# autonomousvision/volsurfs

Measured on AMD Instinct MI355X. Metric: Mrays/s (fwd+bwd) at 800x800, K=5 shells, higher is better.
Workload: dtype f16 (hash features, MLP on MFMA, composite: as the reference), f32 accumulate and I/O

## Files before the change

### include/volsurfs_hip.h

```cpp
#ifndef VOLSURFS_HIP_H
#define VOLSURFS_HIP_H

#include <stdint.h>

#ifdef __cplusplus
extern "C" {
#endif

#define VSA_OK 0
#define VSA_ERR_ARG (-1)
#define VSA_ERR_UNSUPPORTED (-2)

#define VSA_MAX_SHELLS 16

int vsa_version(void);

int vsa_composite_dense_fwd(const float* surfs_rgb, const float* surfs_alpha,
                            const float* rgb_bg, int bg_is_broadcast, float* out_rgb,
                            float* out_rgb_fg, float* out_bg_transmittance, float* out_weights,
                            float* out_surfs_rgb_h, float* out_surfs_alpha_h, int nr_rays,
                            int nr_shells, int carry_f16, void* stream);

int vsa_composite_dense_bwd(const float* surfs_rgb, const float* surfs_alpha,
                            const float* rgb_bg, int bg_is_broadcast, const float* g_rgb,
                            float* g_surfs_rgb, float* g_surfs_alpha, float* g_rgb_bg,
                            int nr_rays, int nr_shells, int carry_f16, void* stream);

int vsa_composite_dense_bwd_l1(const float* surfs_rgb, const float* surfs_alpha,
                               const float* rgb_bg, int bg_is_broadcast, const float* pred_rgb,
                               const float* gt_rgb, float loss_scale, float* g_surfs_rgb,
                               float* g_surfs_alpha, int nr_rays, int nr_shells, int carry_f16,
                               void* stream);

int vsa_composite_dense_fwd_bwd_l1(const float* surfs_rgb, const float* surfs_alpha,
                                   const float* rgb_bg, int bg_is_broadcast, const float* gt_rgb,
                                   float loss_scale, float* out_rgb, float* g_surfs_rgb,
                                   float* g_surfs_alpha, int nr_rays, int nr_shells, int carry_f16,
                                   void* stream);

long long vsa_reduce_scratch_bytes(void);
int vsa_count_hits(const int32_t* hit_slot, long long n, void* scratch, int64_t* out, void* stream);
int vsa_l1_mean(const float* pred, const float* gt, long long n, void* scratch, float* out, void* stream);

typedef struct vsa_bvh vsa_bvh;
int vsa_bvh_build(const float* verts, const int32_t* faces, int nr_verts, int nr_faces,
                  int leaf_size, vsa_bvh** out_bvh);
int vsa_bvh_sizes(const vsa_bvh* bvh, int* nr_nodes, int* nr_tris, int* max_depth);
int vsa_bvh_export(const vsa_bvh* bvh, float* nodes_out, float* tris_out, int node_base,
                   int tri_base);
int vsa_bvh_export_q(const vsa_bvh* bvh, uint32_t* qnodes_out, float* tris_out, int node_base,
                     int tri_base, float* frame_out);
int vsa_bvh_refit(vsa_bvh* bvh, const float* verts, int nr_verts);
int vsa_bvh_destroy(vsa_bvh* bvh);

typedef struct vsa_bvh_dev vsa_bvh_dev;
int vsa_bvh_dev_build(const float* verts, const int32_t* faces, int nr_verts, int nr_faces, int leaf_size,
                      void* stream, vsa_bvh_dev** out_bvh);
int vsa_bvh_dev_sizes(const vsa_bvh_dev* bvh, int* nr_nodes, int* nr_tris, int* max_depth);
int vsa_bvh_dev_export(const vsa_bvh_dev* bvh, float* nodes_out, uint32_t* qnodes_out, float* tris_out,
                       int node_base, int tri_base, float* frame_out, void* stream);
int vsa_bvh_dev_refit(vsa_bvh_dev* bvh, const float* verts, int nr_verts, void* stream);
int vsa_bvh_dev_destroy(vsa_bvh_dev* bvh);
int vsa_bvh_dev_build_ploc(const float* verts, const int32_t* faces, int nr_verts, int nr_faces, int leaf_size,
                           int radius, void* stream, vsa_bvh_dev** out_bvh);

int vsa_trace(const float* nodes, const float* tris, const int32_t* mesh_roots, int nr_meshes,
              int max_depth, const float* rays_o, const float* rays_d, int nr_rays, float t_min,
              float* hit_t, int32_t* hit_slot, float* hit_uv, void* stream);

int vsa_trace_q(const uint32_t* qnodes, const float* tris, const int32_t* mesh_roots,
                const float* mesh_frames, int nr_meshes, int max_depth, const float* rays_o,
                const float* rays_d, int nr_rays, float t_min, float* hit_t, int32_t* hit_slot,
                float* hit_uv, void* stream);
int vsa_trace_q_narrow(const uint32_t* qnodes, const float* tris, const int32_t* mesh_roots,
                       const float* mesh_frames, int nr_meshes, int max_depth, const float* rays_o,
                       const float* rays_d, int nr_rays, float t_min, float* hit_t, int32_t* hit_slot,
                       float* hit_uv, int rays_per_wave, void* stream);
long long vsa_trace_feedback_bytes(int nr_rays, int nr_meshes);
int vsa_trace_q_fb(const uint32_t* qnodes, const float* tris, const int32_t* mesh_roots,
                   const float* mesh_frames, int nr_meshes, int max_depth, const float* rays_o,
                   const float* rays_d, int nr_rays, float t_min, float* hit_t, int32_t* hit_slot,
                   float* hit_uv, void* feedback, long long feedback_bytes, int phase, void* stream);
int vsa_trace_coop_config(int chunk, int lanes, long long max_waves);
int vsa_trace_q_stats(const uint32_t* qnodes, const float* tris, const int32_t* mesh_roots,
                      const float* mesh_frames, int nr_meshes, int max_depth, const float* rays_o,
                      const float* rays_d, int nr_rays, float t_min, uint64_t* stats, void* stream);
int vsa_hit_attributes(const float* tris, const float* rays_o, const float* rays_d,
                       const float* hit_t, const int32_t* hit_slot, const float* hit_uv,
                       int nr_rays, uint8_t* is_hit, int32_t* tri_id, float* positions,
                       float* normals, float* barycentric, void* stream);

#define VSA_NT_MAX_LEVELS 16
#define VSA_NT_MAX_DEG 4
#define VSA_NT_WEIGHTS_PER_TEX 8192
#define VSA_NT_ROW_QUADS(d) ((d) == 0 ? 2 : ((d) == 1 ? 4 : 8))
#define VSA_NT_ALPHA_QUAD(d) ((d) == 0 ? 1 : ((d) == 1 ? 3 : ((d) == 2 ? 4 : 6)))

typedef struct vsa_nt_plan {
  int32_t nr_shells;
  int32_t rgb_degrees;
  int32_t alpha_degrees;
  int32_t inner_solid;
  int32_t with_alpha_decay;
  int32_t n_levels;
  int32_t tex_res[VSA_NT_MAX_DEG];
  float sh_lo[VSA_NT_MAX_DEG];
  float sh_span[VSA_NT_MAX_DEG];
  float level_scale[VSA_NT_MAX_LEVELS];
  int32_t level_res[VSA_NT_MAX_LEVELS];
  int32_t level_size[VSA_NT_MAX_LEVELS];
  int32_t level_offset[VSA_NT_MAX_LEVELS + 1];
  int64_t dom_off[VSA_MAX_SHELLS * VSA_NT_MAX_DEG + 1];
  int64_t slot_capacity;
  int32_t max_rays;
  int32_t anchor;
  int64_t row_base[VSA_MAX_SHELLS * VSA_NT_MAX_DEG + 1];
  void* balance;
  int32_t row_format;
  int32_t grads_zeroed;
  int32_t shared_rgb;
  int32_t shared_alpha;
} vsa_nt_plan;

long long vsa_nt_balance_bytes(void);
int vsa_nt_rebalance(const vsa_nt_plan* plan, void* stream);

int vsa_nt_mark(const vsa_nt_plan* plan, const int32_t* hit_slot, const float* hit_uv,
                const float* face_uvs, int nr_rays, float* tex_uv, uint8_t* marks, void* stream);

int vsa_nt_compact_frame(const vsa_nt_plan* plan, uint8_t* marks, int32_t* slot_of,
                         int32_t* texel_of_slot, float* slot_xy, int32_t* seg_start,
                         int32_t* block_scratch, void* stream);

int vsa_nt_encode_fwd(const vsa_nt_plan* plan, const void* tables_h, const float* slot_xy,
                      const int32_t* seg_start, void* features, void* stream);

int vsa_nt_mlp_fwd(const vsa_nt_plan* plan, const void* weights_h, const void* features,
                   const int32_t* seg_start, uint8_t* texels, void* pre_out, void* stream);

int vsa_nt_encode_mlp_fwd(const vsa_nt_plan* plan, const void* tables_h, const void* weights_h,
                          const float* slot_xy, const int32_t* seg_start, void* features,
                          uint8_t* texels, void* pre_out, void* stream);

int vsa_nt_mlp_bwd(const vsa_nt_plan* plan, const void* weights_h, void* features,
                   const int32_t* seg_start, uint16_t* grad_rows, float* grad_weights,
                   float* dfeat_abs_sum, float weight_grad_scale, void* stream);

int vsa_nt_shade_fwd(const vsa_nt_plan* plan, const int32_t* hit_slot, const float* tex_uv,
                     const float* rays_d, const float* tris, const int32_t* slot_of,
                     const int32_t* seg_start, const uint8_t* texels, int nr_rays,
                     float* surfs_rgb, float* surfs_alpha,
                     float* surfs_normals, float* coeffs_out, float* act_out, void* stream);

int vsa_nt_shade_bwd(const vsa_nt_plan* plan, const int32_t* hit_slot, const float* tex_uv,
                     const float* rays_d, const float* tris, const int32_t* slot_of,
                     const int32_t* seg_start, const uint8_t* texels, int nr_rays,
                     const float* g_surfs_rgb,
                     const float* g_surfs_alpha, float grad_scale, uint16_t* grad_rows,
                     const float* act_in, void* stream);

long long vsa_nt_planes_bytes(const vsa_nt_plan* plan);
int vsa_nt_export_planes(const vsa_nt_plan* plan, const int32_t* slot_of, const int32_t* seg_start,
                         const uint8_t* texels, uint8_t* planes, long long planes_bytes, void* stream);
int vsa_nt_import_planes(const vsa_nt_plan* plan, const uint8_t* planes, long long planes_bytes,
                         const int32_t* slot_of, const int32_t* seg_start, uint8_t* texels, void* stream);

int vsa_nt_encode_bwd(const vsa_nt_plan* plan, const void* dfeatures, const float* dfeat_abs_sum,
                      float grad_scale, const float* slot_xy, const int32_t* seg_start,
                      float* grad_tables, void* stream);

int vsa_nt_encode_bwd_range(const vsa_nt_plan* plan, const void* dfeatures,
                            const float* dfeat_abs_sum, float grad_scale, const float* slot_xy,
                            const int32_t* seg_start, float* grad_tables, int shell_begin,
                            int shell_end, void* stream);

typedef struct vsa_dp_flags vsa_dp_flags;
int vsa_dp_flags_create(int n, vsa_dp_flags** out);
int vsa_dp_flags_destroy(vsa_dp_flags* flags);
int vsa_dp_flags_read(const vsa_dp_flags* flags, uint32_t* host_out);

int vsa_nt_encode_bwd_phased(const vsa_nt_plan* plan, const void* dfeatures,
                             const float* dfeat_abs_sum, float grad_scale, const float* slot_xy,
                             const int32_t* seg_start, float* grad_tables, int n_phases,
                             const int32_t* phase_shell_end, vsa_dp_flags* flags, uint32_t* counters,
                             const uint32_t* epoch, int reserve_cus, void* stream);

int vsa_dp_signal(vsa_dp_flags* flags, int index, uint32_t* epoch, int advance_epoch, void* stream);

int vsa_dp_stream_wait(vsa_dp_flags* flags, int index, uint32_t value, int mode, void* stream);

#define VSA_GRID_MAX_LEVELS 32
typedef struct vsa_grid_plan {
  int32_t n_dims;
  int32_t n_levels;
  int32_t n_features;
  int32_t reserved0;
  float level_scale[VSA_GRID_MAX_LEVELS];
  int32_t level_res[VSA_GRID_MAX_LEVELS];
  int32_t level_size[VSA_GRID_MAX_LEVELS];
  int32_t level_offset[VSA_GRID_MAX_LEVELS + 1];
} vsa_grid_plan;

int vsa_grid_encode_fwd(const vsa_grid_plan* plan, const float* tables, const float* x,
                        int nr_points, float* out, void* stream);
int vsa_grid_encode_bwd(const vsa_grid_plan* plan, const float* x, const float* g_out,
                        int nr_points, float* grad_tables, void* stream);
int vsa_grid_encode_bwd_sliced(const vsa_grid_plan* plan, const float* x, const float* g_out,
                               int nr_points, float* grad_tables, float* workspace, void* stream);
int vsa_grid_encode_bwd_binned_workspace(const vsa_grid_plan* plan, int nr_points,
                                         long long* workspace_floats);
int vsa_grid_encode_bwd_binned(const vsa_grid_plan* plan, const float* x, const float* g_out,
                               int nr_points, float* grad_tables, float* workspace, void* stream);
int vsa_grid_encode_fwd_ld(const vsa_grid_plan* plan, const float* tables, const float* x,
                           int nr_points, float* out, int out_stride, int append_x, void* stream);
int vsa_grid_encode_bwd_ld(const vsa_grid_plan* plan, const float* x, const float* g_out,
                           int g_stride, int nr_points, float* grad_tables, void* stream);
int vsa_grid_encode_bwd_sliced_ld(const vsa_grid_plan* plan, const float* x, const float* g_out,
                                  int g_stride, int nr_points, float* grad_tables, float* workspace,
                                  void* stream);
int vsa_grid_encode_bwd_binned_ld(const vsa_grid_plan* plan, const float* x, const float* g_out,
                                  int g_stride, int nr_points, float* grad_tables, float* workspace,
                                  void* stream);
int vsa_sh_encode(const float* dirs, int nr_dirs, int degree, float* out, void* stream);

int vsa_field_head_fwd(const float* y1, int y1_stride, const float* dirs_enc, long long nr_points, int nr_feat,
                       int nr_dir, float* x2, float* density, void* stream);
int vsa_field_head_bwd(const float* y1, int y1_stride, const float* dx2, const float* d_density, long long nr_points,
                       int nr_feat, int nr_dir, float* dy1, void* stream);

#define VSA_MLP_MAX_LAYERS 6
typedef struct vsa_mlp_plan {
  int32_t n_layers;
  int32_t dims[VSA_MLP_MAX_LAYERS + 1];
  const float* w[VSA_MLP_MAX_LAYERS];
  const float* b[VSA_MLP_MAX_LAYERS];
// ... 106 lines not shown
                           const float* rgb, const float* rgb_bg, int bg_per_ray, const float* weights_sum,
                           const float* g_rgb, const float* g_weights_sum, float* g_density,
                           float* g_rgb_samples, float* g_rgb_bg, float* scratch, int nr_rays,
                           int bug_compat, void* stream);
int vsa_nerf_coarse_cdf(const int32_t* start_end, const float* density, const float* dt, float* cdf,
                        int nr_rays, void* stream);
int vsa_neus_composite_fwd(const int32_t* start_end, const float* sdf, const float* sdf_grad,
                           const float* dirs, const float* dt, const float* samples_z,
                           const float* normals, const float* rgb, const float* rgb_bg, int bg_per_ray,
                           double cos_anneal_ratio, double logistic_beta, float* rgb_fg, float* rgb_out,
                           float* weights_sum, float* depth, float* normals_out, float* weights,
                           float* alpha, int nr_rays, void* stream);
int vsa_neus_composite_bwd(const int32_t* start_end, const float* sdf, const float* sdf_grad,
                           const float* dirs, const float* dt, const float* rgb, const float* rgb_bg,
                           int bg_per_ray, double cos_anneal_ratio, double logistic_beta,
                           const float* weights_sum, const float* g_rgb, const float* g_weights_sum,
                           float* g_sdf, float* g_sdf_grad, float* g_rgb_samples, float* g_rgb_bg,
                           float* scratch, int nr_rays, int bug_compat, void* stream);
int vsa_sdf_coarse_cdf(const int32_t* start_end, const float* sdf, const float* dt, float logistic_beta,
                       float* cdf, int nr_rays, void* stream);
int vsa_offsets_composite_fwd(const int32_t* start_end, int nr_surfs, const float* sdfs, const float* sdfs_grad,
                              const float* normals, const float* rgb, const float* transparency, const float* dirs,
                              const float* dt, const float* samples_z, const float* rgb_bg, int bg_per_ray,
                              double cos_anneal_ratio, double logistic_beta, int with_alpha_decay,
                              double alpha_decay_factor, float* surfs_rgb, float* surfs_normals, float* surfs_depths,
                              float* surfs_weight_sum, float* surfs_alpha, float* surfs_transmittance,
                              float* surfs_blending_weights, float* rgb_fg, float* bg_transmittance, float* rgb_out,
                              float* alpha, int nr_rays, void* stream);
int vsa_offsets_composite_bwd(const int32_t* start_end, int nr_surfs, const float* sdfs, const float* sdfs_grad,
                              const float* normals, const float* rgb, const float* transparency, const float* dirs,
                              const float* dt, const float* rgb_bg, int bg_per_ray, double cos_anneal_ratio,
                              double logistic_beta, int with_alpha_decay, double alpha_decay_factor,
                              const float* surfs_rgb, const float* surfs_alpha, const float* surfs_transmittance,
                              const float* bg_transmittance, const float* g_rgb, float* g_sdfs, float* g_sdfs_grad,
                              float* g_rgb_samples, float* g_transparency, float* g_rgb_bg, float* scratch,
                              int nr_rays, int bug_compat, void* stream);
int vsa_sdfs_coarse_cdf(const int32_t* start_end, int nr_surfs, const float* sdfs, const float* dt,
                        float logistic_beta, float* cdf, int nr_rays, void* stream);
int vsa_packed_median_depth(const int32_t* start_end, const float* samples_z,
                            const float* weights, float threshold, float* out, int nr_rays,
                            int fallback_compat, void* stream);
int vsa_packed_update_dt(const int32_t* start_end, const float* ray_max_dt, const float* ray_exit,
                         const float* samples_z, int is_background, float* samples_dt,
                         int nr_rays, void* stream);
int vsa_sample_bg(const float* rays_o, const float* rays_d, const float* ray_t_start,
                  float ray_t_far, int nr_samples_per_ray, int jitter, uint64_t rng_state,
                  uint64_t rng_inc, float* ray_max_dt, float* samples_3d, float* samples_dirs,
                  float* samples_z, int32_t* ray_start_end_idx, int nr_rays, void* stream);
int vsa_contract_samples(const float* ray_o, const int32_t* start_end, const float* samples_3d,
                         const float* samples_z, float* out_samples_3d, float* out_samples_z,
                         int nr_rays, void* stream);

int vsa_packed_sum_over_rays(const int32_t* start_end, const float* values, float* sum_per_ray,
                             float* sum_per_sample, int nr_rays, int dim, void* stream);
int vsa_packed_sum_over_rays_bwd(const int32_t* start_end, const float* g_sum_per_ray,
                                 const float* g_sum_per_sample, float* g_values, int nr_rays,
                                 int dim, void* stream);
int vsa_packed_sdf2alpha(const int32_t* start_end, const float* samples_dt, const float* samples_sdf,
                         const float* logistic_beta, float* alpha, int nr_rays, void* stream);
int vsa_packed_compute_cdf(const int32_t* start_end, const float* weights, float* cdf, int nr_rays,
                           void* stream);

int vsa_sample_fg(const float* rays_o, const float* rays_d, const float* ray_t_entry,
                  const float* ray_t_exit, float min_dist_between_samples,
                  int min_nr_samples_per_ray, int max_nr_samples_per_ray, int jitter,
                  uint64_t rng_state, uint64_t rng_inc, float* ray_max_dt, int32_t* samples_idx,
                  float* samples_3d, float* samples_dirs, float* samples_z,
                  int32_t* ray_start_end_idx, int nr_rays, void* stream);
int vsa_pack_compact(const int32_t* start_end, const int32_t* out_start, const int32_t* samples_idx,
                     const float* samples_3d, const float* samples_dirs, const float* samples_z,
                     const float* samples_dt, const float* samples_values, int values_dim,
                     int32_t* out_idx, float* out_3d, float* out_dirs, float* out_z, float* out_dt,
                     float* out_values, int32_t* out_start_end, int nr_rays, void* stream);
int vsa_importance_sample(const float* rays_o, const float* rays_d, const int32_t* start_end,
                          const float* samples_z, const float* samples_cdf,
                          int nr_importance_samples, int jitter, uint64_t rng_state,
                          uint64_t rng_inc, float* out_3d, float* out_dirs, float* out_z,
                          int32_t* out_start_end, int nr_rays, void* stream);

int vsa_uncontract_samples(const float* ray_o, const int32_t* start_end, const float* samples_3d,
                           const float* samples_z, float* out_samples_3d, float* out_samples_z,
                           int nr_rays, void* stream);

int vsa_combine_packs(const int32_t* start_end_1, const int32_t* idx_1, const float* s3d_1,
                      const float* dirs_1, const float* z_1, const float* values_1,
                      const int32_t* start_end_2, const int32_t* idx_2, const float* s3d_2,
                      const float* dirs_2, const float* z_2, const float* values_2,
                      const int32_t* out_start, float min_dist_between_samples, int values_dim,
                      int32_t* out_idx, float* out_3d, float* out_dirs, float* out_z,
                      float* out_values, int32_t* out_start_end, int nr_rays, void* stream);

int vsa_intersect_primitive(const float* rays_o, const float* rays_d, int nr_rays, int kind,
                            float size, uint8_t* is_hit, float* t_near, float* t_far,
                            float* points_near, float* points_far, void* stream);

int vsa_camera_rays(const float* c2w, const float* intrinsics_inv, int height, int width,
                    int nr_rays_per_pixel, int jitter_pixels, uint64_t rng_state, uint64_t rng_inc,
                    float* rays_o, float* rays_d, float* points_2d, void* stream);

int vsa_reel_next_rays_batch(const float* c2w_all, const float* intrinsics_inv_all,
                             const float* rgb_all, const float* mask_all, int nr_cameras, int height,
                             int width, int batch_size, int nr_rays_per_pixel, int jitter_pixels,
                             uint64_t rng_state, uint64_t rng_inc, int32_t* camera_idx,
                             float* rays_o, float* rays_d, float* gt_rgb, float* gt_mask,
                             float* points_2d, void* stream);

typedef struct vsa_train_ctl {
  int32_t iter;
  int32_t nr_rays;
  int32_t capacity;
  int32_t adam_step;
  float loss_scale;
  float adam_lr;
  float loss;
  int32_t clamped;
  uint64_t rng_state, rng_inc;
  int64_t nr_hits;
  int32_t target_hits;
  int32_t nr_warmup;
  int32_t nr_milestones;
  int32_t milestone[8];
  float lr_stage[9];
  int32_t adam_pending;
  double lr_base;
  double loss_weight;
  int64_t sum_rays, sum_hits;
} vsa_train_ctl;

int vsa_train_ctl_tick(vsa_train_ctl* ctl, void* stream);

int vsa_reel_next_rays_batch_ctl(const float* c2w_all, const float* intrinsics_inv_all, const float* rgb_all,
                                 const float* mask_all, int nr_cameras, int height, int width, int capacity,
                                 int nr_rays_per_pixel, int jitter_pixels, const vsa_train_ctl* ctl,
                                 const float* dummy_o, const float* dummy_d, const float* dummy_rgb,
                                 int32_t* camera_idx, float* rays_o, float* rays_d, float* gt_rgb,
                                 float* gt_mask, float* points_2d, void* stream);

int vsa_composite_dense_fwd_bwd_l1_ctl(const float* surfs_rgb, const float* surfs_alpha, const float* rgb_bg,
                                       int bg_is_broadcast, const float* gt_rgb, const vsa_train_ctl* ctl,
                                       float* out_rgb, float* g_surfs_rgb, float* g_surfs_alpha, int capacity,
                                       int nr_shells, int carry_f16, void* stream);

int vsa_l1_mean_ctl(const float* pred, const float* gt, int capacity, void* scratch, vsa_train_ctl* ctl, void* stream);

int vsa_adam_step_ctl(const vsa_adam_tensor* tensors_dev, const int32_t* chunks_dev, int nr_chunks, float beta1,
                      float beta2, float eps, float grad_scale, int zero_grads, int max_workgroups,
                      const vsa_train_ctl* ctl, void* stream);

int vsa_tile_order(const float* src, float* dst, int height, int width, int channels, int inverse,
                   void* stream);
int vsa_tile_order_rays(const float* rays_o, const float* rays_d, const float* gt_rgb,
                        float* rays_o_tiled, float* rays_d_tiled, float* gt_rgb_tiled, int height,
                        int width, void* stream);


int vsa_occ_grid_points(const int32_t* point_indices, int nr_points, int nr_voxels_per_dim,
                        float extent_x, float extent_y, float extent_z, int centre_of_voxel, int jitter,
                        uint64_t rng_state, uint64_t rng_inc, float* out_points, void* stream);
int vsa_occ_update_values(const int32_t* point_indices, const float* values, int nr_points, float decay,
                          float* grid_values, void* stream);
int vsa_occ_update_occupancy_density(const int32_t* point_indices, int nr_points, int nr_voxels_per_dim,
                                     float extent_x, float extent_y, float extent_z,
                                     float occupancy_thresh, int check_neighbours,
                                     const float* grid_values, uint8_t* grid_occupancy, void* stream);
int vsa_occ_update_occupancy_sdf(const int32_t* point_indices, const float* logistic_beta, int nr_points,
                                 int nr_voxels_per_dim, float extent_x, float extent_y, float extent_z,
                                 float occupancy_thresh, const float* grid_values,
                                 uint8_t* grid_occupancy, void* stream);
int vsa_occ_check(const float* points, int nr_points, int nr_voxels_per_dim, float extent_x,
                  float extent_y, float extent_z, const float* grid_values,
                  const uint8_t* grid_occupancy, const uint8_t* grid_roi, uint8_t* out_occupancy,
                  float* out_values, void* stream);
int vsa_occ_rays_t_near_t_far(const float* rays_o, const float* rays_d, const float* ray_t_entry,
                              const float* ray_t_exit, int nr_rays, int nr_voxels_per_dim,
                              float extent_x, float extent_y, float extent_z,
                              const uint8_t* grid_occupancy, const uint8_t* grid_roi, float* out_t_near,
                              float* out_t_far, void* stream);
int vsa_occ_first_sample(const float* rays_o, const float* rays_d, const float* ray_t_entry,
                         const float* ray_t_exit, int nr_rays, int nr_voxels_per_dim, float extent_x,
                         float extent_y, float extent_z, const uint8_t* grid_occupancy,
                         const uint8_t* grid_roi, float* samples_3d, float* samples_dirs,
                         float* samples_z, float* samples_dt, int32_t* ray_start_end_idx, void* stream);
int vsa_occ_advance_samples(const float* samples_dirs, const float* samples_3d, int nr_points,
                            int nr_voxels_per_dim, float extent_x, float extent_y, float extent_z,
                            const uint8_t* grid_occupancy, const uint8_t* grid_roi,
                            float* new_samples_3d, uint8_t* is_within_bounds, void* stream);
int vsa_sample_fg_occupied(const float* rays_o, const float* rays_d, const float* ray_t_entry,
                           const float* ray_t_exit, float min_dist_between_samples,
                           int min_nr_samples_per_ray, int max_nr_samples_per_ray, int jitter_samples,
                           uint64_t rng_state, uint64_t rng_inc, int nr_voxels_per_dim, float extent_x,
                           float extent_y, float extent_z, const uint8_t* grid_occupancy,
                           const uint8_t* grid_roi, float* ray_max_dt, int32_t* samples_idx,
                           float* samples_3d, float* samples_dirs, float* samples_z,
                           int32_t* ray_start_end_idx, int nr_rays, void* stream);

long long vsa_image_metrics_workspace_bytes(int B, int H, int W, int pool, int pred_u8, int gt_u8);
int vsa_image_metrics(const void* pred, int pred_u8, const void* gt, int gt_u8, int B, int H, int W, int pool,
                      int quantize_pred, void* workspace, long long workspace_bytes, double* psnr_out,
                      double* ssim_out, void* stream);

long long vsa_isosurface_workspace_bytes(long long nx, long long ny, long long nz, int nr_levels);
int vsa_isosurface_count(const float* grid, long long nx, long long ny, long long nz, const float* levels,
                         int nr_levels, int inside_above, void* workspace, long long workspace_bytes,
                         long long* totals, void* stream);
int vsa_isosurface_emit(const float* grid, long long nx, long long ny, long long nz, const float* levels,
                        int nr_levels, int inside_above, const float* origin, const float* spacing, void* workspace,
                        long long workspace_bytes, const long long* totals, float* const* verts,
                        int32_t* const* faces, void* stream);
int vsa_mc_table(int8_t* out);

long long vsa_simplify_workspace_bytes(long long nr_verts, long long nr_faces);
int vsa_simplify(const float* verts, long long nr_verts, const int32_t* faces, long long nr_faces,
                 long long target_faces, void* workspace, long long workspace_bytes, float* out_verts,
                 int32_t* out_faces, long long* stats, float* stage_ms, void* stream);

#define VSA_ERR_ATLAS_FULL (-3)
long long vsa_atlas_workspace_bytes(long long nr_verts, long long nr_faces, int resolution);
int vsa_atlas(const float* verts, long long nr_verts, const int32_t* faces, long long nr_faces, int resolution,
              int padding, void* workspace, long long workspace_bytes, float* out_faces_uvs, int32_t* out_chart,
              long long* stats, float* scale, float* stage_ms, void* stream);
long long vsa_atlas_rasterize_workspace_bytes(long long nr_faces);
int vsa_atlas_rasterize(const float* faces_uvs, long long nr_faces, int resolution, void* workspace,
                        long long workspace_bytes, int32_t* out_face_id, int32_t* out_count, void* stream);

int vsa_st_begin(const float* points_near, int nr_rays, int nr_slots, float* pts, uint8_t* flags, int32_t* live,
                 float* dense, int32_t* count, void* stream);
int vsa_st_step(const int32_t* live_in, const int32_t* count_in, const float* sdf, int nr_columns,
                const int32_t* slot_cols, int nr_rays, const float* rays_d, float sdf_multiplier, float thresh,
                int kind, float size, float* pts, uint8_t* flags, uint8_t* keep, int32_t* block_counts,
                const float* dense_in, int32_t* live_out, float* dense_out, int32_t* count_out, int bound,
                void* stream);
int vsa_st_finish(const float* pts, const float* rays_o, int nr_rays, int nr_slots, const uint8_t* flags,
                  int unconverged_are_hits, float* z, uint8_t* hit, uint8_t* keep, int32_t* block_counts,
                  int32_t* hit_list, int32_t* hit_count, void* stream);
int vsa_st_scatter(const int32_t* ids, long long nr_ids, const float* src, int nr_channels, int nr_rays,
                   int nr_slots, float* dst, void* stream);
int vsa_st_blend(const float* surfs_rgb, const float* surfs_alpha, int nr_rays, int nr_surfs,
                 float* surfs_transmittance, float* surfs_blending_weights, float* rgb_fg, float* bg_transmittance,
                 void* stream);

long long vsa_tb_workspace_bytes(long long nr_faces, int resolution);
long long vsa_tb_max_chunks(int resolution, int nr_samples, long long chunk_rows);
int vsa_tb_samples(const float* faces_uvs, long long nr_faces, int resolution, int nr_samples,
                   unsigned long long seed, long long chunk_rows, void* workspace, long long workspace_bytes,
                   int32_t* owner, int32_t* ctl, int ctl_len, void* stream);
int vsa_tb_emit(const float* verts, const int32_t* faces, const float* faces_uvs, long long nr_faces, int resolution,
                int nr_samples, unsigned long long seed, const void* workspace, long long workspace_bytes,
                const int32_t* owner, int32_t* row_start, float* points, float* normals, void* stream);
int vsa_tb_resolve(const float* vals, int nr_channels, const int32_t* row_start, int texel_begin, int texel_end,
                   int resolution, float* texture, void* stream);
int vsa_tb_dilate(float* img, int height, int width, int nr_channels, int nr_iterations, int32_t* stamp,
                  int32_t* filled, void* stream);

int vsa_tsdf_fuse_lattice(const float* proj, const float* depth, int nr_views, int height, int width,
                          const float* axis, int n, float sdf_trunc, int uncontract, float* out_tsdf, void* stream);
int vsa_tsdf_fuse_points(const float* proj, const float* depth, const float* rgb_maps, int nr_views, int height,
                         int width, const float* points, long long nr_points, float sdf_trunc, int uncontract,
                         float* out_tsdf, float* out_rgb, void* stream);
int vsa_tsdf_uncontract_points(const float* points, long long nr_points, float max_range, float* out, void* stream);

long long vsa_mesh_clusters_workspace_bytes(long long nr_verts, long long nr_faces);
int vsa_mesh_clusters(const float* verts, long long nr_verts, const int32_t* faces, long long nr_faces,
                      void* workspace, long long workspace_bytes, int32_t* out_triangle_clusters,
                      int32_t* out_cluster_n_triangles, double* out_cluster_area, long long* out_nr_clusters,
                      float* stage_ms, void* stream);
int vsa_mesh_filter(const float* verts, long long nr_verts, const int32_t* faces, long long nr_faces, int mode,
                    const uint8_t* keep_mask, long long cluster_to_keep, long long min_cluster_faces,
                    int drop_unreferenced, int drop_degenerate, void* workspace, long long workspace_bytes,
                    float* out_verts, int32_t* out_faces, int32_t* out_vertex_map, int32_t* out_face_map,
                    long long* stats, float* stage_ms, void* stream);
int vsa_mesh_compact_rows(const void* rows, long long nr_rows, int row_words, const int32_t* map, void* out,
                          void* stream);

int vsa_face_view_counts(const uint32_t* qnodes, const float* tris, const int32_t* mesh_roots,
                         const float* mesh_frames, int nr_meshes, int max_depth,
                         const float* c2w_all, const float* intrinsics_inv_all,
                         int nr_views, int height, int width, int supersample, float t_min,
                         const long long* face_base, uint32_t* counts,
                         void* stream);
int vsa_face_view_counts_tile(int tile);
int vsa_face_ring_dilate(const int32_t* faces, long long nr_faces, long long nr_verts, uint8_t* keep,
                         int rings, uint8_t* vert_scratch, void* stream);

int vsa_closest_point_q(const uint32_t* qnodes, const float* tris, const int32_t* mesh_roots,
                        const float* mesh_frames, int nr_meshes, int max_depth, const float* points,
                        long long nr_points, float* dist, int32_t* slot, float* bary, void* stream);
int vsa_closest_point_q_stats(const uint32_t* qnodes, const float* tris, const int32_t* mesh_roots,
                              const float* mesh_frames, int nr_meshes, int max_depth, const float* points,
                              long long nr_points, long long* counters, void* stream);
int vsa_closest_walk_config(int keep_bounds);
long long vsa_surface_area_prefix_workspace_bytes(long long nr_slots);
int vsa_surface_area_prefix(const float* tris, long long first_slot, long long nr_slots, void* workspace,
                            long long workspace_bytes, long long* area_prefix, void* stream);
int vsa_surface_sample(const float* tris, long long first_slot, long long nr_slots, const long long* area_prefix,
                       long long nr_samples, unsigned long long seed, float* points, int32_t* slot, float* bary,
                       void* stream);
int vsa_surface_distance(const float* src_tris, long long src_first_slot, long long src_nr_slots,
                         const long long* src_area_prefix, const uint32_t* dst_qnodes, const float* dst_tris,
                         int dst_root, const float* dst_frame, int dst_max_depth, long long nr_samples,
                         unsigned long long seed, const float* thresholds, int nr_thresholds,
                         unsigned long long* stats, double* partials, void* stream);

long long vsa_mesh_pseudonormals_workspace_bytes(long long nr_verts, long long nr_faces);
int vsa_mesh_pseudonormals(const float* vertices, long long nr_verts, const int32_t* faces, long long nr_faces,
                           void* workspace, long long workspace_bytes, float* table, void* stream);
int vsa_signed_distance_q(const uint32_t* qnodes, const float* tris, const int32_t* mesh_roots,
// ... 40 lines not shown
```

### volsurfs_amd/composite.py

```python
import torch

from . import _lib


class _CompositeDense(torch.autograd.Function):
    @staticmethod
    def forward(ctx, surfs_rgb, surfs_alpha, rgb_bg, carry_f16):
        N, K, _ = surfs_rgb.shape
        surfs_rgb = _lib.check_f32(surfs_rgb.contiguous(), N, K, 3)
        surfs_alpha = _lib.check_f32(surfs_alpha.contiguous().view(N, K), N, K)
        rgb_bg = rgb_bg.contiguous()
        bcast = rgb_bg.shape[0] == 1 and N != 1
        _lib.check_f32(rgb_bg, 1 if bcast else N, 3)
        dev = surfs_rgb.device
        out_rgb = torch.empty(N, 3, device=dev)
        out_fg = torch.empty(N, 3, device=dev)
        out_bgT = torch.empty(N, 1, device=dev)
        out_w = torch.empty(N, K, 1, device=dev)
        out_rgb_h = torch.empty(N, K, 3, device=dev)
        out_alpha_h = torch.empty(N, K, 1, device=dev)
        _lib.call("vsa_composite_dense_fwd", surfs_rgb, surfs_alpha, rgb_bg, bcast, out_rgb,
                  out_fg, out_bgT, out_w, out_rgb_h, out_alpha_h, N, K, int(carry_f16),
                  _lib.stream_ptr())
        ctx.save_for_backward(surfs_rgb, surfs_alpha, rgb_bg)
        ctx.bcast = bcast
        ctx.carry_f16 = int(carry_f16)
        ctx.mark_non_differentiable(out_fg, out_bgT, out_w, out_rgb_h, out_alpha_h)
        return out_rgb, out_fg, out_bgT, out_w, out_rgb_h, out_alpha_h

    @staticmethod
    def backward(ctx, g_rgb, *unused):
        surfs_rgb, surfs_alpha, rgb_bg = ctx.saved_tensors
        N, K, _ = surfs_rgb.shape
        g_rgb = _lib.check_f32(g_rgb.contiguous(), N, 3)
        g_c = torch.empty_like(surfs_rgb)
        g_a = torch.empty_like(surfs_alpha)
        need_bg = ctx.needs_input_grad[2]
        g_bg = torch.empty(N, 3, device=g_rgb.device) if need_bg else None
        _lib.call("vsa_composite_dense_bwd", surfs_rgb, surfs_alpha, rgb_bg, ctx.bcast, g_rgb,
                  g_c, g_a, g_bg, N, K, ctx.carry_f16, _lib.stream_ptr())
        if need_bg and ctx.bcast:
            g_bg = g_bg.sum(0, keepdim=True)
        return g_c, g_a, g_bg, None


def composite_dense(surfs_rgb, surfs_alpha, rgb_bg, carry_f16=False):
    N, K = surfs_rgb.shape[:2]
    alpha2d = surfs_alpha.reshape(N, K)
    rgb, fg, bgT, w, rgb_h, alpha_h = _CompositeDense.apply(surfs_rgb, alpha2d, rgb_bg, carry_f16)
    return {
        "rgb": rgb,
        "rgb_fg": fg,
        "rgb_bg": rgb_bg.expand(N, 3).half().float(),
        "surfs_alpha": alpha_h,
        "surfs_rgb": rgb_h,
        "surfs_blending_weights": w,
        "bg_transmittance": bgT,
    }


class _CompositeL1(torch.autograd.Function):

    @staticmethod
    def forward(ctx, surfs_rgb, surfs_alpha, rgb_bg, gt_rgb):
        N, K = surfs_rgb.shape[:2]
        rgb, g_c, g_a = composite_fwd_bwd_l1_raw(surfs_rgb.contiguous(), surfs_alpha.reshape(N, K).contiguous(),
                                                 rgb_bg.contiguous(), gt_rgb.contiguous(), 1.0 / (3.0 * N))
        ctx.save_for_backward(g_c, g_a)
        ctx.alpha_shape = surfs_alpha.shape
        loss = l1_mean(rgb, gt_rgb)
        ctx.mark_non_differentiable(rgb)
        return loss, rgb

    @staticmethod
    def backward(ctx, g_loss, _g_rgb):
        g_c, g_a = ctx.saved_tensors
        return g_c * g_loss, (g_a * g_loss).reshape(ctx.alpha_shape), None, None


def composite_l1(surfs_rgb, surfs_alpha, rgb_bg, gt_rgb):
    return _CompositeL1.apply(surfs_rgb, surfs_alpha, rgb_bg, gt_rgb)


def composite_fwd_raw(surfs_rgb, surfs_alpha, rgb_bg, carry_f16=False):
    N, K, _ = surfs_rgb.shape
    out = torch.empty(N, 3, device=surfs_rgb.device)
    bcast = rgb_bg.shape[0] == 1 and N != 1
    _lib.call("vsa_composite_dense_fwd", surfs_rgb, surfs_alpha, rgb_bg, bcast, out, None, None,
              None, None, None, N, K, int(carry_f16), _lib.stream_ptr())
    return out


def composite_bwd_raw(surfs_rgb, surfs_alpha, rgb_bg, g_rgb, carry_f16=False):
    N, K, _ = surfs_rgb.shape
    g_c = torch.empty_like(surfs_rgb)
    g_a = torch.empty_like(surfs_alpha)
    bcast = rgb_bg.shape[0] == 1 and N != 1
    _lib.call("vsa_composite_dense_bwd", surfs_rgb, surfs_alpha, rgb_bg, bcast, g_rgb, g_c, g_a,
              None, N, K, int(carry_f16), _lib.stream_ptr())
    return g_c, g_a


def composite_bwd_l1_raw(surfs_rgb, surfs_alpha, rgb_bg, pred_rgb, gt_rgb, loss_scale, carry_f16=False):
    N, K, _ = surfs_rgb.shape
    g_c = torch.empty_like(surfs_rgb)
    g_a = torch.empty_like(surfs_alpha)
    bcast = rgb_bg.shape[0] == 1 and N != 1
    _lib.call("vsa_composite_dense_bwd_l1", surfs_rgb, surfs_alpha, rgb_bg, bcast, pred_rgb, gt_rgb,
              float(loss_scale), g_c, g_a, N, K, int(carry_f16), _lib.stream_ptr())
    return g_c, g_a


def composite_fwd_bwd_l1_raw(surfs_rgb, surfs_alpha, rgb_bg, gt_rgb, loss_scale, carry_f16=False):
    N, K, _ = surfs_rgb.shape
    rgb = torch.empty(N, 3, device=surfs_rgb.device)
    g_c = torch.empty_like(surfs_rgb)
    g_a = torch.empty_like(surfs_alpha)
    bcast = rgb_bg.shape[0] == 1 and N != 1
    _lib.call("vsa_composite_dense_fwd_bwd_l1", surfs_rgb, surfs_alpha, rgb_bg, bcast, gt_rgb,
              float(loss_scale), rgb, g_c, g_a, N, K, int(carry_f16), _lib.stream_ptr())
    return rgb, g_c, g_a


_reduce_scratch = {}


def reduce_scratch(device):
    import ctypes
    dev = torch.device(device)
    dev = torch.device("cuda", torch.cuda.current_device()) if dev.index is None else dev
    key = (dev, torch.cuda.current_stream(dev).cuda_stream)
    sc = _reduce_scratch.get(key)
    if sc is None:
        fn = _lib.lib().vsa_reduce_scratch_bytes
        fn.restype = ctypes.c_longlong
        sc = _reduce_scratch[key] = torch.zeros(int(fn()), dtype=torch.uint8, device=dev)
    return sc


def l1_mean(pred, gt):
    import ctypes
    pred, gt = _lib.check_f32(pred.contiguous()), _lib.check_f32(gt.contiguous(), *pred.shape)
    pred, gt = (x if x.data_ptr() % 16 == 0 else x.clone() for x in (pred, gt))
    out = torch.empty((), device=pred.device)
    _lib.call("vsa_l1_mean", pred, gt, ctypes.c_longlong(pred.numel()), reduce_scratch(pred.device), out,
              _lib.stream_ptr())
    return out


def count_hits(hit_slot):
    import ctypes
    if hit_slot.dtype != torch.int32 or not hit_slot.is_contiguous() or not hit_slot.is_cuda:
        raise _lib.VolsurfsHipError("count_hits: contiguous CUDA int32 tensor expected")
    out = torch.empty((), dtype=torch.int64, device=hit_slot.device)
    _lib.call("vsa_count_hits", hit_slot, ctypes.c_longlong(hit_slot.numel()), reduce_scratch(hit_slot.device), out,
              _lib.stream_ptr())
    return out
```

### volsurfs_amd/csrc/composite_dense.hip

```cpp
#include "common.h"

namespace {

#ifndef VSA_COMP_TILE
#define VSA_COMP_TILE 256
#endif
constexpr int TILE = VSA_COMP_TILE;

template <int K>
struct Lds {
  static constexpr int SC = (3 * K) | 1;
  static constexpr int SA = K | 1;
};

template <int W, int S>
__device__ __forceinline__ void slab_load(const float* __restrict__ g, float* __restrict__ s,
                                          int rows_valid) {
  const int total = rows_valid * W;
  const int nvec = total >> 2;
  const float4* g4 = reinterpret_cast<const float4*>(g);
  if constexpr (W == S) {
    if (rows_valid == TILE && (TILE * W) % 4 == 0) {
      typedef __attribute__((address_space(3))) void* lds_vp;
      typedef __attribute__((address_space(1))) const void* glb_vp;
      const int wave = __builtin_amdgcn_readfirstlane(threadIdx.x >> 6), lane = threadIdx.x & 63;
      constexpr int NV = TILE * W / 4, NC = (NV + 63) / 64;
      for (int c = wave; c < NC; c += TILE / 64)
        if (c * 64 + lane < NV)
          __builtin_amdgcn_global_load_lds((glb_vp)(g4 + c * 64 + lane), (lds_vp)(s + c * 256), 16, 0, 0);
      return;
    }
    float4* s4 = reinterpret_cast<float4*>(s);
    for (int v = threadIdx.x; v < nvec; v += TILE) s4[v] = g4[v];
  } else {
    for (int v = threadIdx.x; v < nvec; v += TILE) {
      float4 x = g4[v];
      int e = v << 2;
      float xs[4] = {x.x, x.y, x.z, x.w};
#pragma unroll
      for (int i = 0; i < 4; ++i) {
        int r = (e + i) / W;
        int j = (e + i) - r * W;
        s[r * S + j] = xs[i];
      }
    }
  }
  for (int e = (nvec << 2) + threadIdx.x; e < total; e += TILE) {
    int r = e / W;
    s[r * S + (e - r * W)] = g[e];
  }
}
__device__ __forceinline__ void slab_load_fence() {
  asm volatile("s_waitcnt vmcnt(0)" ::: "memory");
}

template <int W, int S>
__device__ __forceinline__ void slab_store(float* __restrict__ g, const float* __restrict__ s,
                                           int rows_valid) {
  const int total = rows_valid * W;
  const int nvec = total >> 2;
  float4* g4 = reinterpret_cast<float4*>(g);
  if constexpr (W == S) {
    const float4* s4 = reinterpret_cast<const float4*>(s);
    for (int v = threadIdx.x; v < nvec; v += TILE) g4[v] = s4[v];
  } else {
    for (int v = threadIdx.x; v < nvec; v += TILE) {
      int e = v << 2;
      float xs[4];
#pragma unroll
      for (int i = 0; i < 4; ++i) {
        int r = (e + i) / W;
        int j = (e + i) - r * W;
        xs[i] = s[r * S + j];
      }
      g4[v] = make_float4(xs[0], xs[1], xs[2], xs[3]);
    }
  }
  for (int e = (nvec << 2) + threadIdx.x; e < total; e += TILE) {
    int r = e / W;
    g[e] = s[r * S + (e - r * W)];
  }
}

template <int K, bool CARRY_F16>
struct RayFwd {
  float a[K], c[K][3], T[K], w[K], om[K];
  float bgT, fg[3];
  __device__ __forceinline__ void run(const float* sc, const float* sa) {
#pragma unroll
    for (int k = 0; k < K; ++k) {
      a[k] = vsa_round_f16(sa[k]);
#pragma unroll
      for (int ch = 0; ch < 3; ++ch) c[k][ch] = vsa_round_f16(sc[3 * k + ch]);
      om[k] = vsa_round_f16(1.0f - a[k]);
    }
    float acc = 1.0f, Tp = 1.0f;
    fg[0] = fg[1] = fg[2] = 0.f;
#pragma unroll
    for (int k = K - 1; k >= 0; --k) {
      T[k] = Tp;
      if (CARRY_F16) {
        Tp = vsa_round_f16(Tp * om[k]);
      } else {
        acc = vsa_pin_f32(acc * om[k]);
        Tp = vsa_round_f16(acc);
      }
      w[k] = vsa_round_f16(T[k] * a[k]);
#pragma unroll
      for (int ch = 0; ch < 3; ++ch) fg[ch] += vsa_round_f16(c[k][ch] * w[k]);
    }
    bgT = Tp;
#pragma unroll
    for (int ch = 0; ch < 3; ++ch) fg[ch] = vsa_round_f16(vsa_pin_f32(fg[ch]));
  }
};

template <int K, bool CARRY_F16>
__global__ __launch_bounds__(TILE) void composite_dense_fwd_kernel(
    const float* __restrict__ surfs_rgb, const float* __restrict__ surfs_alpha,
    const float* __restrict__ rgb_bg, int bg_bcast, float* __restrict__ out_rgb,
    float* __restrict__ out_rgb_fg, float* __restrict__ out_bgT, float* __restrict__ out_w,
    float* __restrict__ out_rgb_h, float* __restrict__ out_alpha_h, int N) {
  using L = Lds<K>;
  __shared__ __attribute__((aligned(16))) float s_c[TILE * L::SC];
  __shared__ __attribute__((aligned(16))) float s_a[TILE * L::SA];
  __shared__ __attribute__((aligned(16))) float s_o[TILE * 3];
  const long long ray0 = (long long)blockIdx.x * TILE;
  const int rows = min(TILE, (int)(N - ray0));
  slab_load<3 * K, L::SC>(surfs_rgb + ray0 * 3 * K, s_c, rows);
  slab_load<K, L::SA>(surfs_alpha + ray0 * K, s_a, rows);
  if (!bg_bcast) slab_load<3, 3>(rgb_bg + ray0 * 3, s_o, rows);
  slab_load_fence();
  __syncthreads();
  const int r = threadIdx.x;
  if (r < rows) {
    RayFwd<K, CARRY_F16> f;
    f.run(s_c + r * L::SC, s_a + r * L::SA);
    float bg[3];
#pragma unroll
    for (int ch = 0; ch < 3; ++ch)
      bg[ch] = vsa_round_f16(bg_bcast ? rgb_bg[ch] : s_o[r * 3 + ch]);
#pragma unroll
    for (int ch = 0; ch < 3; ++ch)
      s_o[r * 3 + ch] = vsa_round_f16(f.fg[ch] + vsa_round_f16(f.bgT * bg[ch]));
    const long long n = ray0 + r;
    if (out_rgb_fg) {
#pragma unroll
      for (int ch = 0; ch < 3; ++ch) out_rgb_fg[n * 3 + ch] = f.fg[ch];
    }
    if (out_bgT) out_bgT[n] = f.bgT;
    if (out_w) {
#pragma unroll
      for (int k = 0; k < K; ++k) out_w[n * K + k] = f.w[k];
    }
    if (out_alpha_h) {
#pragma unroll
      for (int k = 0; k < K; ++k) out_alpha_h[n * K + k] = f.a[k];
    }
    if (out_rgb_h) {
#pragma unroll
      for (int k = 0; k < K; ++k)
#pragma unroll
        for (int ch = 0; ch < 3; ++ch) out_rgb_h[(n * K + k) * 3 + ch] = f.c[k][ch];
    }
  }
  __syncthreads();
  slab_store<3, 3>(out_rgb + ray0 * 3, s_o, rows);
}

template <int K, bool CARRY_F16>
__global__ __launch_bounds__(TILE) void composite_dense_bwd_kernel(
    const float* __restrict__ surfs_rgb, const float* __restrict__ surfs_alpha,
    const float* __restrict__ rgb_bg, int bg_bcast, const float* __restrict__ g_rgb,
    float* __restrict__ g_surfs_rgb, float* __restrict__ g_surfs_alpha,
    float* __restrict__ g_rgb_bg, int N, const float* __restrict__ l1_gt, float l1_scale,
    float* __restrict__ pred_out, const vsa_train_ctl* __restrict__ ctl) {
  using L = Lds<K>;
  int n_active = N;
  if (ctl) {
    l1_scale = ctl->loss_scale;
    n_active = ctl->nr_rays;
  }
  __shared__ __attribute__((aligned(16))) float s_c[TILE * L::SC];
  __shared__ __attribute__((aligned(16))) float s_a[TILE * L::SA];
  __shared__ __attribute__((aligned(16))) float s_g[TILE * 3];
  __shared__ __attribute__((aligned(16))) float s_b[TILE * 3];
  __shared__ __attribute__((aligned(16))) float s_t[TILE * 3];
  const long long ray0 = (long long)blockIdx.x * TILE;
  const int rows = min(TILE, (int)(N - ray0));
  slab_load<3 * K, L::SC>(surfs_rgb + ray0 * 3 * K, s_c, rows);
  slab_load<K, L::SA>(surfs_alpha + ray0 * K, s_a, rows);
  if (!pred_out) slab_load<3, 3>(g_rgb + ray0 * 3, s_g, rows);
  if (!bg_bcast) slab_load<3, 3>(rgb_bg + ray0 * 3, s_b, rows);
  if (l1_gt) slab_load<3, 3>(l1_gt + ray0 * 3, s_t, rows);
  slab_load_fence();
  __syncthreads();
  const int r = threadIdx.x;
  if (r < rows) {
    RayFwd<K, CARRY_F16> f;
    float* sc = s_c + r * L::SC;
    float* sa = s_a + r * L::SA;
    f.run(sc, sa);
    float g[3], bg[3];
#pragma unroll
    for (int ch = 0; ch < 3; ++ch) {
      bg[ch] = vsa_round_f16(bg_bcast ? rgb_bg[ch] : s_b[r * 3 + ch]);
      if (pred_out) {
        g[ch] = vsa_round_f16(f.fg[ch] + vsa_round_f16(f.bgT * bg[ch]));
        s_g[r * 3 + ch] = g[ch];
      } else {
        g[ch] = s_g[r * 3 + ch];
      }
      if (l1_gt) {
        const float d = g[ch] - s_t[r * 3 + ch];
        g[ch] = ray0 + r >= n_active ? 0.f : (d > 0.f ? l1_scale : (d < 0.f ? -l1_scale : 0.f));
      }
    }
    float S = g[0] * bg[0] + g[1] * bg[1] + g[2] * bg[2];
#pragma unroll
    for (int k = 0; k < K; ++k) {
      float rk = g[0] * f.c[k][0] + g[1] * f.c[k][1] + g[2] * f.c[k][2];
      sa[k] = f.T[k] * (rk - S);
      S = f.a[k] * rk + f.om[k] * S;
#pragma unroll
      for (int ch = 0; ch < 3; ++ch) sc[3 * k + ch] = g[ch] * f.w[k];
    }
    if (g_rgb_bg) {
#pragma unroll
      for (int ch = 0; ch < 3; ++ch) s_b[r * 3 + ch] = g[ch] * f.bgT;
    }
  }
  __syncthreads();
  slab_store<3 * K, L::SC>(g_surfs_rgb + ray0 * 3 * K, s_c, rows);
  slab_store<K, L::SA>(g_surfs_alpha + ray0 * K, s_a, rows);
  if (g_rgb_bg) slab_store<3, 3>(g_rgb_bg + ray0 * 3, s_b, rows);
  if (pred_out) slab_store<3, 3>(pred_out + ray0 * 3, s_g, rows);
}

}

#define VSA_K_DISPATCH(K_, BODY)              \
  switch (K_) {                               \
    case 1: { constexpr int KK = 1; BODY; } break;   \
    case 2: { constexpr int KK = 2; BODY; } break;   \
    case 3: { constexpr int KK = 3; BODY; } break;   \
    case 4: { constexpr int KK = 4; BODY; } break;   \
    case 5: { constexpr int KK = 5; BODY; } break;   \
    case 6: { constexpr int KK = 6; BODY; } break;   \
    case 7: { constexpr int KK = 7; BODY; } break;   \
    case 8: { constexpr int KK = 8; BODY; } break;   \
    case 9: { constexpr int KK = 9; BODY; } break;   \
    default: return VSA_ERR_UNSUPPORTED;      \
  }

extern "C" int vsa_composite_dense_fwd(const float* surfs_rgb, const float* surfs_alpha,
                                       const float* rgb_bg, int bg_is_broadcast, float* out_rgb,
                                       float* out_rgb_fg, float* out_bg_transmittance,
                                       float* out_weights, float* out_surfs_rgb_h,
                                       float* out_surfs_alpha_h, int nr_rays, int nr_shells,
                                       int carry_f16, void* stream) {
  if (nr_rays < 0 || !out_rgb) return VSA_ERR_ARG;
  if (nr_rays == 0) return VSA_OK;
  if (!surfs_rgb || !surfs_alpha || !rgb_bg) return VSA_ERR_ARG;
  dim3 grid(vsa_div_up(nr_rays, TILE)), block(TILE);
  hipStream_t st = (hipStream_t)stream;
  VSA_K_DISPATCH(nr_shells, {
    if (carry_f16)
      hipLaunchKernelGGL((composite_dense_fwd_kernel<KK, true>), grid, block, 0, st, surfs_rgb,
                         surfs_alpha, rgb_bg, bg_is_broadcast, out_rgb, out_rgb_fg,
                         out_bg_transmittance, out_weights, out_surfs_rgb_h, out_surfs_alpha_h,
                         nr_rays);
    else
      hipLaunchKernelGGL((composite_dense_fwd_kernel<KK, false>), grid, block, 0, st, surfs_rgb,
                         surfs_alpha, rgb_bg, bg_is_broadcast, out_rgb, out_rgb_fg,
                         out_bg_transmittance, out_weights, out_surfs_rgb_h, out_surfs_alpha_h,
                         nr_rays);
  });
  VSA_RETURN_LAUNCH_STATUS();
}

static int composite_bwd_launch(const float* surfs_rgb, const float* surfs_alpha,
                                const float* rgb_bg, int bg_is_broadcast, const float* g_rgb,
                                float* g_surfs_rgb, float* g_surfs_alpha, float* g_rgb_bg,
                                int nr_rays, int nr_shells, int carry_f16, const float* l1_gt,
                                float l1_scale, void* stream, float* pred_out = nullptr,
                                const vsa_train_ctl* ctl = nullptr) {
  if (nr_rays < 0) return VSA_ERR_ARG;
  if (nr_rays == 0) return VSA_OK;
  if (!surfs_rgb || !surfs_alpha || !rgb_bg || (!g_rgb && !pred_out) || !g_surfs_rgb || !g_surfs_alpha)
    return VSA_ERR_ARG;
  dim3 grid(vsa_div_up(nr_rays, TILE)), block(TILE);
  hipStream_t st = (hipStream_t)stream;
  VSA_K_DISPATCH(nr_shells, {
    if (carry_f16)
      hipLaunchKernelGGL((composite_dense_bwd_kernel<KK, true>), grid, block, 0, st, surfs_rgb,
                         surfs_alpha, rgb_bg, bg_is_broadcast, g_rgb, g_surfs_rgb, g_surfs_alpha,
                         g_rgb_bg, nr_rays, l1_gt, l1_scale, pred_out, ctl);
    else
      hipLaunchKernelGGL((composite_dense_bwd_kernel<KK, false>), grid, block, 0, st, surfs_rgb,
                         surfs_alpha, rgb_bg, bg_is_broadcast, g_rgb, g_surfs_rgb, g_surfs_alpha,
                         g_rgb_bg, nr_rays, l1_gt, l1_scale, pred_out, ctl);
  });
  VSA_RETURN_LAUNCH_STATUS();
}

extern "C" int vsa_composite_dense_bwd(const float* surfs_rgb, const float* surfs_alpha,
                                       const float* rgb_bg, int bg_is_broadcast,
                                       const float* g_rgb, float* g_surfs_rgb,
                                       float* g_surfs_alpha, float* g_rgb_bg, int nr_rays,
                                       int nr_shells, int carry_f16, void* stream) {
  return composite_bwd_launch(surfs_rgb, surfs_alpha, rgb_bg, bg_is_broadcast, g_rgb, g_surfs_rgb,
                              g_surfs_alpha, g_rgb_bg, nr_rays, nr_shells, carry_f16, nullptr, 0.f,
                              stream);
}

extern "C" int vsa_composite_dense_bwd_l1(const float* surfs_rgb, const float* surfs_alpha,
                                          const float* rgb_bg, int bg_is_broadcast,
                                          const float* pred_rgb, const float* gt_rgb,
                                          float loss_scale, float* g_surfs_rgb,
                                          float* g_surfs_alpha, int nr_rays, int nr_shells,
                                          int carry_f16, void* stream) {
  if (!gt_rgb) return VSA_ERR_ARG;
  return composite_bwd_launch(surfs_rgb, surfs_alpha, rgb_bg, bg_is_broadcast, pred_rgb,
                              g_surfs_rgb, g_surfs_alpha, nullptr, nr_rays, nr_shells, carry_f16,
                              gt_rgb, loss_scale, stream);
}

extern "C" int vsa_composite_dense_fwd_bwd_l1(const float* surfs_rgb, const float* surfs_alpha,
                                              const float* rgb_bg, int bg_is_broadcast,
                                              const float* gt_rgb, float loss_scale, float* out_rgb,
                                              float* g_surfs_rgb, float* g_surfs_alpha, int nr_rays,
                                              int nr_shells, int carry_f16, void* stream) {
  if (!gt_rgb || (nr_rays > 0 && !out_rgb)) return VSA_ERR_ARG;
  return composite_bwd_launch(surfs_rgb, surfs_alpha, rgb_bg, bg_is_broadcast, nullptr, g_surfs_rgb,
                              g_surfs_alpha, nullptr, nr_rays, nr_shells, carry_f16, gt_rgb,
                              loss_scale, stream, out_rgb);
}

extern "C" int vsa_composite_dense_fwd_bwd_l1_ctl(const float* surfs_rgb, const float* surfs_alpha,
                                                  const float* rgb_bg, int bg_is_broadcast, const float* gt_rgb,
                                                  const vsa_train_ctl* ctl, float* out_rgb, float* g_surfs_rgb,
                                                  float* g_surfs_alpha, int capacity, int nr_shells, int carry_f16,
                                                  void* stream) {
  if (!gt_rgb || !ctl || capacity < 1 || !out_rgb) return VSA_ERR_ARG;
  return composite_bwd_launch(surfs_rgb, surfs_alpha, rgb_bg, bg_is_broadcast, nullptr, g_surfs_rgb, g_surfs_alpha,
                              nullptr, capacity, nr_shells, carry_f16, gt_rgb, 0.f, stream, out_rgb, ctl);
}
```

### volsurfs_amd/csrc/nt_shade.hip

```cpp
#include "nt_common.h"

struct ShadeIdx {
  long long tile;
  int shell;
  bool valid;
};
__device__ __forceinline__ ShadeIdx shade_idx(int K, int tiles) {
  const unsigned id = blockIdx.x, x = id & 7u, q = id >> 3;
  const unsigned s = q % (unsigned)K, tg = q / (unsigned)K;
  const long long t = (long long)tg * 8 + x;
  return {t, (int)s, t < tiles};
}
static inline dim3 shade_grid(int tiles, int shells) {
  return dim3((unsigned)(((tiles + 7) / 8) * 8 * shells));
}

namespace {

constexpr int SH_BLOCK = 256;

constexpr float C0 = 0.28209479177387814f;
constexpr float C1 = 0.4886025119029199f;
constexpr float C2_0 = 1.0925484305920792f, C2_1 = -1.0925484305920792f,
                C2_2 = 0.31539156525252005f, C2_3 = -1.0925484305920792f,
                C2_4 = 0.5462742152960396f;
constexpr float C3_0 = -0.5900435899266435f, C3_1 = 2.890611442640554f,
                C3_2 = -0.4570457994644658f, C3_3 = 0.3731763325901154f,
                C3_4 = -0.4570457994644658f, C3_5 = 1.445305721320277f,
                C3_6 = -0.5900435899266435f;

__device__ __forceinline__ void sh_basis(float x, float y, float z, float b[16]) {
  b[0] = C0;
  b[1] = -(C1 * y);
  b[2] = C1 * z;
  b[3] = -(C1 * x);
  const float xx = x * x, yy = y * y, zz = z * z, xy = x * y, yz = y * z, xz = x * z;
  b[4] = C2_0 * xy;
  b[5] = C2_1 * yz;
  b[6] = C2_2 * ((2.0f * zz - xx) - yy);
  b[7] = C2_3 * xz;
  b[8] = C2_4 * (xx - yy);
  b[9] = (C3_0 * y) * (3.0f * xx - yy);
  b[10] = (C3_1 * xy) * z;
  b[11] = (C3_2 * y) * ((4.0f * zz - xx) - yy);
  b[12] = (C3_3 * z) * ((2.0f * zz - 3.0f * xx) - 3.0f * yy);
  b[13] = (C3_4 * x) * ((4.0f * zz - xx) - yy);
  b[14] = (C3_5 * z) * (xx - yy);
  b[15] = (C3_6 * x) * (xx - 3.0f * yy);
}

struct HitCtx {
  bool hit;
  float dir[3];
  float decay;
  int row[VSA_NT_MAX_DEG][4];
  float w[VSA_NT_MAX_DEG][4];
  float fx[VSA_NT_MAX_DEG], fy[VSA_NT_MAX_DEG];
};

__device__ __forceinline__ float sigmoidf_(float x) { return 1.0f / (1.0f + __expf(-x)); }

__device__ __forceinline__ float sh_raw(const float b[16], const float* sh, int degrees) {
  float r = vsa_round_f16(C0 * sh[0]);
  if (degrees > 1) {
    r = r + b[1] * sh[1];
    r = r + b[2] * sh[2];
    r = r + b[3] * sh[3];
    if (degrees > 2) {
#pragma unroll
      for (int m = 4; m < 9; ++m) r = r + b[m] * sh[m];
      if (degrees > 3) {
#pragma unroll
        for (int m = 9; m < 16; ++m) r = r + b[m] * sh[m];
      }
    }
  }
  return r;
}

__device__ __forceinline__ void build_lut(const vsa_nt_plan& plan, float* s_lut) {
  for (int i = threadIdx.x; i < VSA_NT_MAX_DEG * 256; i += blockDim.x) {
    const int d = i >> 8, q = i & 255;
    const float o = vsa_round_f16((float)q / 255.0f);
    const float t = vsa_round_f16(plan.sh_span[d] * o);
    s_lut[i] = vsa_round_f16(plan.sh_lo[d] + t);
  }
}

template <bool FULL4>
__device__ __forceinline__ int rgb_degs(const vsa_nt_plan& p) { return FULL4 ? VSA_NT_MAX_DEG : p.rgb_degrees; }
template <bool FULL4>
__device__ __forceinline__ int alpha_degs(const vsa_nt_plan& p) { return FULL4 ? VSA_NT_MAX_DEG : p.alpha_degrees; }

template <bool FULL4 = false>
__device__ __forceinline__ bool load_ctx(const vsa_nt_plan& plan, int s, long long n, int N,
                                         const int* hit_slot, const float* tex_uv,
                                         const float* rays_d, const float4* tris,
                                         const int* slot_of, const int* seg_start, HitCtx& c,
                                         float nrm[3]) {
  const long long o = (long long)s * N + n;
  const int tslot = hit_slot[o];
  c.hit = tslot >= 0;
  nrm[0] = nrm[1] = nrm[2] = 0.f;
  if (!c.hit) return false;
  c.dir[0] = rays_d[3 * n];
  c.dir[1] = rays_d[3 * n + 1];
  c.dir[2] = rays_d[3 * n + 2];
  const float4 e1 = tris[3 * (long long)tslot + 1], e2 = tris[3 * (long long)tslot + 2];
  const float cx = e1.y * e2.z - e1.z * e2.y, cy = e1.z * e2.x - e1.x * e2.z,
              cz = e1.x * e2.y - e1.y * e2.x;
  const float len = sqrtf((cx * cx + cy * cy) + cz * cz);
  const float inv = len > 0.f ? 1.0f / len : 0.f;
  nrm[0] = cx * inv;
  nrm[1] = cy * inv;
  nrm[2] = cz * inv;
  c.decay = 1.0f;
  if (plan.with_alpha_decay) {
    float dot = ((-c.dir[0]) * nrm[0] + (-c.dir[1]) * nrm[1]) + (-c.dir[2]) * nrm[2];
    dot = fminf(fmaxf(dot, 0.0f), 1.0f);
    c.decay = sigmoidf_(10.0f * dot) * 2.0f - 1.0f;
  }
  const float u = tex_uv[2 * o], v = tex_uv[2 * o + 1];
  const int D = max(rgb_degs<FULL4>(plan), alpha_degs<FULL4>(plan));
#pragma unroll
  for (int d = 0; d < VSA_NT_MAX_DEG; ++d) {
    if (d >= D) {
#pragma unroll
      for (int k = 0; k < 4; ++k) c.row[d][k] = 0, c.w[d][k] = 0.f;
      c.fx[d] = c.fy[d] = 0.f;
      continue;
    }
    const int R = plan.tex_res[d], W = R + 2;
    const bool anchor = plan.anchor != 0;
    const NtFootprint f = nt_footprint(u, v, R, anchor);
    const long long base = plan.dom_off[s * VSA_NT_MAX_DEG + d] + (long long)(f.j0 + 1) * W + (f.i0 + 1);
    const int sd = s * VSA_NT_MAX_DEG + d;
    const int rb = (int)plan.row_base[sd] - seg_start[sd] * nt_row_quads(d);
    c.row[d][0] = rb + slot_of[base] * nt_row_quads(d);
    c.row[d][1] = anchor ? c.row[d][0] : rb + slot_of[base + 1] * nt_row_quads(d);
    c.row[d][2] = anchor ? c.row[d][0] : rb + slot_of[base + W] * nt_row_quads(d);
    c.row[d][3] = anchor ? c.row[d][0] : rb + slot_of[base + W + 1] * nt_row_quads(d);
    c.fx[d] = f.fx;
    c.fy[d] = f.fy;
    c.w[d][0] = (1.0f - f.fx) * (1.0f - f.fy);
    c.w[d][1] = f.fx * (1.0f - f.fy);
    c.w[d][2] = (1.0f - f.fx) * f.fy;
    c.w[d][3] = f.fx * f.fy;
  }
  return true;
}

template <bool F16ROWS>
__device__ __forceinline__ void add_corner_row(const vsa_nt_plan& plan, int d, const unsigned* __restrict__ texels,
                                               int row, float wk, const float* s_lut, float acc[28]) {
  const int n = 2 * d + 1;
  if constexpr (!F16ROWS) {
    unsigned wds[8] = {0, 0, 0, 0, 0, 0, 0, 0};
    const unsigned* rp = texels + row;
    if (d == 0) {
      const uint2 v = *reinterpret_cast<const uint2*>(rp);
      wds[0] = v.x, wds[1] = v.y;
    } else {
      const uint4 lo = *reinterpret_cast<const uint4*>(rp);
      wds[0] = lo.x, wds[1] = lo.y, wds[2] = lo.z, wds[3] = lo.w;
      if (d >= 2) {
        const uint4 hi = *reinterpret_cast<const uint4*>(rp + 4);
        wds[4] = hi.x, wds[5] = hi.y, wds[6] = hi.z, wds[7] = hi.w;
      }
    }
#pragma unroll
    for (int i = 0; i < 3 * n; ++i) {
      const unsigned q = (wds[i >> 2] >> (8 * (i & 3))) & 255u;
      acc[i] = acc[i] + s_lut[d * 256 + q] * wk;
    }
#pragma unroll
    for (int i = 0; i < n; ++i) {
      const unsigned q = (wds[nt_alpha_quad(d) + (i >> 2)] >> (8 * (i & 3))) & 255u;
      acc[21 + i] = acc[21 + i] + s_lut[d * 256 + q] * wk;
    }
  } else {
    unsigned wds[16];
    const uint4* rp = reinterpret_cast<const uint4*>(texels + 2 * (long long)row);
    const int nv = d == 0 ? 1 : d == 1 ? 2 : 4;
#pragma unroll
    for (int v = 0; v < 4; ++v) {
      const uint4 x = v < nv ? rp[v] : make_uint4(0, 0, 0, 0);
      wds[4 * v] = x.x, wds[4 * v + 1] = x.y, wds[4 * v + 2] = x.z, wds[4 * v + 3] = x.w;
    }
    const float lo = plan.sh_lo[d], span = plan.sh_span[d];
    const bool raw = plan.row_format == 2;
    auto expand = [&](int elem) {
      const unsigned short hb = (unsigned short)(wds[elem >> 1] >> (16 * (elem & 1)));
      const float o = (float)__builtin_bit_cast(_Float16, hb);
      return raw ? o : vsa_round_f16(lo + vsa_round_f16(vsa_pin_f32(span * o)));
    };
#pragma unroll
    for (int i = 0; i < 3 * n; ++i) acc[i] = acc[i] + expand(i) * wk;
#pragma unroll
    for (int i = 0; i < n; ++i) acc[21 + i] = acc[21 + i] + expand(4 * nt_alpha_quad(d) + i) * wk;
  }
}

template <bool F16ROWS = false>
__device__ __forceinline__ void gather_coeffs(const vsa_nt_plan& plan, const HitCtx& c,
                                              const unsigned* __restrict__ texels,
                                              const float* s_lut, bool has_alpha,
                                              float sh_rgb[3][16], float sh_a[16]) {
#pragma unroll
  for (int d = 0; d < VSA_NT_MAX_DEG; ++d) {
    const int n = 2 * d + 1, m0 = d * d;
    const bool do_rgb = d < plan.rgb_degrees, do_a = has_alpha && d < plan.alpha_degrees;
    if (!do_rgb && !do_a) continue;
    float acc[28];
#pragma unroll
    for (int i = 0; i < 28; ++i) acc[i] = 0.f;
#pragma unroll
    for (int k = 0; k < 4; ++k) add_corner_row<F16ROWS>(plan, d, texels, c.row[d][k], c.w[d][k], s_lut, acc);
#pragma unroll
    for (int ch = 0; ch < 3; ++ch)
#pragma unroll
      for (int i = 0; i < n; ++i) sh_rgb[ch][m0 + i] = do_rgb ? vsa_round_f16(acc[ch * n + i]) : 0.f;
#pragma unroll
    for (int i = 0; i < n; ++i) sh_a[m0 + i] = do_a ? vsa_round_f16(acc[21 + i]) : 0.f;
  }
}

template <bool FULL4 = false, bool F16ROWS = false>
__device__ __forceinline__ void shade_hit(const vsa_nt_plan& plan, const HitCtx& c,
                                          const unsigned* __restrict__ texels, const float* s_lut,
                                          bool has_alpha, const float b[16], float raw[4],
                                          float* __restrict__ coeffs_out) {
  raw[0] = raw[1] = raw[2] = raw[3] = 0.f;
#pragma unroll
  for (int d = 0; d < VSA_NT_MAX_DEG; ++d) {
    const int n = 2 * d + 1, m0 = d * d;
    const bool do_rgb = d < rgb_degs<FULL4>(plan), do_a = has_alpha && d < alpha_degs<FULL4>(plan);
    if (!do_rgb && !do_a) {
      if (coeffs_out) {
#pragma unroll
        for (int i = 0; i < n; ++i)
          coeffs_out[m0 + i] = coeffs_out[16 + m0 + i] = coeffs_out[32 + m0 + i] = coeffs_out[48 + m0 + i] = 0.f;
      }
      continue;
    }
    float acc[28];
#pragma unroll
    for (int i = 0; i < 28; ++i) acc[i] = 0.f;
#pragma unroll
    for (int k = 0; k < 4; ++k) add_corner_row<F16ROWS>(plan, d, texels, c.row[d][k], c.w[d][k], s_lut, acc);
#pragma unroll
    for (int ch = 0; ch < 4; ++ch) {
      const bool on = ch < 3 ? do_rgb : do_a;
#pragma unroll
      for (int i = 0; i < n; ++i) {
        const int m = m0 + i;
        const float shv = on ? vsa_round_f16(ch < 3 ? acc[ch * n + i] : acc[21 + i]) : 0.f;
        if (coeffs_out) coeffs_out[ch * 16 + m] = shv;
        if (on) raw[ch] = m == 0 ? vsa_round_f16(C0 * shv) : raw[ch] + b[m] * shv;
      }
    }
  }
}

#ifndef NT_SHADE_FWD_OCC
#define NT_SHADE_FWD_OCC 3
#endif
template <bool FULL4, bool F16ROWS = false>
__global__ __launch_bounds__(SH_BLOCK, NT_SHADE_FWD_OCC) void nt_shade_fwd_kernel(
    vsa_nt_plan plan, const int* __restrict__ hit_slot, const float* __restrict__ tex_uv,
    const float* __restrict__ rays_d, const float4* __restrict__ tris,
    const int* __restrict__ slot_of, const int* __restrict__ seg_start,
    const unsigned* __restrict__ texels, int N, float* __restrict__ surfs_rgb, float* __restrict__ surfs_alpha,
    float* __restrict__ surfs_normals, float* __restrict__ coeffs_out,
    float4* __restrict__ act_out) {
  __shared__ float s_lut[VSA_NT_MAX_DEG * 256];
  build_lut(plan, s_lut);
  __syncthreads();
  const int K = plan.nr_shells;
  const ShadeIdx wi = shade_idx(K, (N + SH_BLOCK - 1) / SH_BLOCK);
  const long long n = wi.tile * SH_BLOCK + threadIdx.x;
  const int s = wi.shell;
  if (!wi.valid) return;
  if (n >= N) return;
  HitCtx c;
  float nrm[3];
  float rgb[3] = {0.f, 0.f, 0.f}, alpha = 0.f;
  float4 act = make_float4(0.f, 0.f, 0.f, 0.f);
  if (load_ctx<FULL4>(plan, s, n, N, hit_slot, tex_uv, rays_d, tris, slot_of, seg_start, c, nrm)) {
    const bool has_alpha = nt_shell_has_alpha(plan, s);
    float b[16], raw[4];
    sh_basis(c.dir[0], c.dir[1], c.dir[2], b);
    shade_hit<FULL4, F16ROWS>(plan, c, texels, s_lut, has_alpha, b, raw,
              coeffs_out ? coeffs_out + ((long long)s * N + n) * 64 : nullptr);
#pragma unroll
    for (int ch = 0; ch < 3; ++ch) {
      const float sg = sigmoidf_(raw[ch]);
      (ch == 0 ? act.x : ch == 1 ? act.y : act.z) = sg;
      rgb[ch] = rgb_degs<FULL4>(plan) > 1 ? sg : vsa_round_f16(sg);
    }
    if (has_alpha) {
      const float sg = sigmoidf_(raw[3]);
      act.w = sg;
      const float a = alpha_degs<FULL4>(plan) > 1 ? sg : vsa_round_f16(sg);
      alpha = a * c.decay;
    } else {
      alpha = 1.0f;
    }
    if (act_out) act_out[(long long)s * N + n] = act;
  } else if (coeffs_out) {
    float* co = coeffs_out + ((long long)s * N + n) * 64;
    for (int i = 0; i < 64; ++i) co[i] = 0.f;
  }
  const long long o = n * K + s;
  surfs_rgb[3 * o] = rgb[0];
  surfs_rgb[3 * o + 1] = rgb[1];
  surfs_rgb[3 * o + 2] = rgb[2];
  surfs_alpha[o] = alpha;
  if (surfs_normals) {
    surfs_normals[3 * o] = nrm[0];
    surfs_normals[3 * o + 1] = nrm[1];
    surfs_normals[3 * o + 2] = nrm[2];
  }
}

#ifdef SHADE_SPAN
static __device__ unsigned long long g_sspan[1 << 16][2];
__device__ __forceinline__ unsigned long long shade_now() {
  unsigned long long t;
  asm volatile("s_memrealtime %0\n\ts_waitcnt lgkmcnt(0)" : "=s"(t)::"memory");
  return t;
}
#endif
constexpr int SHB_BLOCK = 128;

__device__ __forceinline__ void atomic_pk_add_f16(const _Float16* base, unsigned byte_off, float a, float b) {
  const half2_t v = {(_Float16)a, (_Float16)b};
  asm volatile("global_atomic_pk_add_f16 %0, %1, %2" ::"v"(byte_off), "v"(__builtin_bit_cast(unsigned, v)), "s"(base) : "memory");
}

template <bool RECOMPUTE, bool FULL4, bool F16ROWS = false>
#ifndef NT_SHADE_BWD_OCC
#define NT_SHADE_BWD_OCC 4
#endif
__global__ __launch_bounds__(SHB_BLOCK, RECOMPUTE ? 2 : NT_SHADE_BWD_OCC) void nt_shade_bwd_kernel(
    vsa_nt_plan plan, const int* __restrict__ hit_slot, const float* __restrict__ tex_uv,
    const float* __restrict__ rays_d, const float4* __restrict__ tris,
    const int* __restrict__ slot_of, const int* __restrict__ seg_start,
    const unsigned* __restrict__ texels, int N, const float* __restrict__ g_surfs_rgb,
    const float* __restrict__ g_surfs_alpha, float grad_scale, _Float16* __restrict__ grad_rows,
    const float4* __restrict__ act_in) {
  __shared__ float s_lut[RECOMPUTE ? VSA_NT_MAX_DEG * 256 : 1];
  __shared__ float s_graw[SHB_BLOCK][4];
  __shared__ float s_basis[SHB_BLOCK][17];
  __shared__ int s_row[SHB_BLOCK][9];
  __shared__ float s_f[SHB_BLOCK][9];
#ifdef SHADE_SPAN
  const unsigned long long span_t0 = shade_now();
#endif
  if (RECOMPUTE) {
    build_lut(plan, s_lut);
    __syncthreads();
  }
  const int K = plan.nr_shells;
  const ShadeIdx wi = shade_idx(K, (N + SHB_BLOCK - 1) / SHB_BLOCK);
  const long long n = wi.valid ? wi.tile * SHB_BLOCK + threadIdx.x : (long long)N;
  const int s = wi.shell;
  const int t = threadIdx.x;
  HitCtx c;
  c.hit = false;
  float nrm[3];
  const bool has_alpha = nt_shell_has_alpha(plan, s);
  if (n < N && load_ctx<FULL4>(plan, s, n, N, hit_slot, tex_uv, rays_d, tris, slot_of, seg_start, c, nrm)) {
    float b[16];
    sh_basis(c.dir[0], c.dir[1], c.dir[2], b);
    const long long o = n * K + s;
    float sg4[4];
    if (!RECOMPUTE) {
      const float4 a = act_in[(long long)s * N + n];
      sg4[0] = a.x, sg4[1] = a.y, sg4[2] = a.z, sg4[3] = a.w;
    } else {
      float sh_rgb[3][16], sh_a[16];
      gather_coeffs<F16ROWS>(plan, c, texels, s_lut, has_alpha, sh_rgb, sh_a);
#pragma unroll
      for (int ch = 0; ch < 3; ++ch) sg4[ch] = sigmoidf_(sh_raw(b, sh_rgb[ch], plan.rgb_degrees));
      sg4[3] = has_alpha ? sigmoidf_(sh_raw(b, sh_a, plan.alpha_degrees)) : 0.f;
    }
#pragma unroll
    for (int ch = 0; ch < 3; ++ch) {
      const float sg = sg4[ch];
      s_graw[t][ch] = g_surfs_rgb[3 * o + ch] * sg * (1.0f - sg) * grad_scale;
    }
    float ga = 0.f;
    if (has_alpha) {
      const float sg = sg4[3];
      ga = g_surfs_alpha[o] * c.decay * sg * (1.0f - sg) * grad_scale;
    }
    s_graw[t][3] = ga;
#pragma unroll
    for (int m = 0; m < 16; ++m) s_basis[t][m] = b[m];
#pragma unroll
    for (int d = 0; d < VSA_NT_MAX_DEG; ++d) {
      s_row[t][2 * d] = c.row[d][0];
      s_row[t][2 * d + 1] = c.row[d][2];
      s_f[t][2 * d] = c.fx[d];
      s_f[t][2 * d + 1] = c.fy[d];
    }
  }
  const int lane = t & 63, wbase = t & ~63;
  const unsigned long long hits = __ballot(c.hit);
  const int d = lane < 12 ? 0 : (lane < 26 ? 1 : (lane < 37 ? 2 : 3));
  const int lb = lane - (d == 0 ? 0 : (d == 1 ? 12 : (d == 2 ? 26 : 37)));
  const int nn = 2 * d + 1, n_rgb_pairs = (3 * nn + 1) >> 1, row_pairs = n_rgb_pairs + ((nn + 1) >> 1);
  const unsigned magic3 = 0x55555556u, magic5 = 0x33333334u, magic7 = 0x24924925u;
  const unsigned magic_nn = d == 1 ? magic3 : (d == 2 ? magic5 : magic7);
  auto div_nn = [&](int x) { return d == 0 ? x : (int)__umulhi((unsigned)x, magic_nn); };
  const int q = d == 0 ? (int)__umulhi((unsigned)lb, magic3) : (d == 1 ? (int)__umulhi((unsigned)lb, magic7) : 0);
  const int jb = lb - q * row_pairs;
  const bool is_alpha = jb >= n_rgb_pairs;
  const int e0 = is_alpha ? 2 * (jb - n_rgb_pairs) : 2 * jb;
  const int part = is_alpha ? nn : 3 * nn;
  const int qd = nt_row_quads(d), qsh = d == 0 ? 1 : (d == 1 ? 2 : 3);
  const int lofs = 4 * (q * qd + (is_alpha ? nt_alpha_quad(d) : 0)) + e0;
  const bool band_on = lane < 52 && (is_alpha ? (has_alpha && d < alpha_degs<FULL4>(plan)) : d < rgb_degs<FULL4>(plan));
  const bool on1 = band_on && e0 + 1 < part;
  const int c0 = div_nn(e0), c1 = div_nn(e0 + 1);
  const int ch0 = is_alpha ? 3 : c0, ch1 = is_alpha ? 3 : c1;
  const int m0 = d * d + (is_alpha ? e0 : e0 - c0 * nn), m1 = on1 ? d * d + (is_alpha ? e0 + 1 : e0 + 1 - c1 * nn) : 0;
  float span = plan.row_format == 2 ? 1.0f : plan.sh_span[d];
  asm volatile("" : "+v"(span));
  typedef float float2_t __attribute__((ext_vector_type(2)));
  int cur[4] = {-1, -1, -1, -1};
  float2_t acc[4] = {float2_t(0.f), float2_t(0.f), float2_t(0.f), float2_t(0.f)};
  const unsigned lofs_b = 2u * (unsigned)lofs;
  unsigned long long rem = hits;
  struct HitIn { float g0, g1, b0, b1, fx, fy; int r0, r1; };
  auto fetch = [&](int ht) {
    HitIn r;
    r.g0 = s_graw[ht][ch0], r.g1 = s_graw[ht][ch1], r.b0 = s_basis[ht][m0], r.b1 = s_basis[ht][m1];
    r.fx = s_f[ht][2 * d], r.fy = s_f[ht][2 * d + 1];
    r.r0 = s_row[ht][2 * d], r.r1 = s_row[ht][2 * d + 1];
    return r;
  };
  HitIn nx = fetch(wbase + (rem ? __ffsll((long long)rem) - 1 : 0));
  while (rem) {
    const int hl = __ffsll((long long)rem) - 1;
    rem &= rem - 1;
    const HitIn cu = nx;
    nx = fetch(wbase + (rem ? __ffsll((long long)rem) - 1 : hl));
    if (band_on) {
      float2_t gg;
      gg.x = cu.g0 * cu.b0;
      gg.y = on1 ? cu.g1 * cu.b1 : 0.f;
      const float fx = cu.fx, fy = cu.fy;
      const float w[4] = {(1.0f - fx) * (1.0f - fy), fx * (1.0f - fy), (1.0f - fx) * fy, fx * fy};
      int sl[4];
      float wl[4];
#pragma unroll
      for (int y = 0; y < 2; ++y) {
        const int ra = y ? cu.r1 : cu.r0, rb = ra + qd;
        const int la = ra >> 3, lbn = rb >> 3;
        const bool ma = q == ((ra & 7) >> qsh), mb = q == ((rb & 7) >> qsh), one = la == lbn;
        sl[2 * y] = la;
        wl[2 * y] = ma ? w[2 * y] : ((one && mb) ? w[2 * y + 1] : 0.f);
        sl[2 * y + 1] = one ? -1 : lbn;
        wl[2 * y + 1] = (!one && mb) ? w[2 * y + 1] : 0.f;
      }
      const bool dup = sl[2] == sl[0] || sl[2] == sl[1] || ((sl[3] == sl[0] || sl[3] == sl[1]) && sl[3] >= 0);
      if (__builtin_expect(__ballot(dup) != 0ull, 0)) {
#pragma unroll
        for (int k = 2; k < 4; ++k)
#pragma unroll
          for (int i = 0; i < 2; ++i)
            if (sl[k] == sl[i] && sl[k] >= 0) {
              wl[i] += wl[k];
              wl[k] = 0.f;
              sl[k] = -1;
            }
      }
      float2_t v[4];
#pragma unroll
      for (int k = 0; k < 4; ++k) v[k] = float2_t(wl[k] * span) * gg;
#pragma unroll
      for (int j = 0; j < 4; ++j) {
        bool kept = false;
#pragma unroll
        for (int k = 0; k < 4; ++k) {
          const bool same = cur[j] == sl[k];
          v[k] = __builtin_elementwise_fma(acc[j], float2_t(same ? 1.0f : 0.0f), v[k]);
          kept |= same;
        }
        if (!kept && cur[j] >= 0) atomic_pk_add_f16(grad_rows, (unsigned)cur[j] * 64u + lofs_b, acc[j].x, acc[j].y);
      }
#pragma unroll
      for (int k = 0; k < 4; ++k) {
        cur[k] = sl[k];
        acc[k] = v[k];
      }
    }
  }
  if (band_on) {
#pragma unroll
    for (int k = 0; k < 4; ++k)
      if (cur[k] >= 0) atomic_pk_add_f16(grad_rows, (unsigned)cur[k] * 64u + lofs_b, acc[k].x, acc[k].y);
  }
#ifdef SHADE_SPAN
  {
    const int w = blockIdx.y * gridDim.x + blockIdx.x;
    if (threadIdx.x == 0 && w < (1 << 16)) g_sspan[w][0] = span_t0, g_sspan[w][1] = shade_now();
  }
#endif
}

}

extern "C" int vsa_nt_shade_fwd(const vsa_nt_plan* plan, const int32_t* hit_slot,
                                const float* tex_uv, const float* rays_d, const float* tris,
                                const int32_t* slot_of, const int32_t* seg_start,
                                const uint8_t* texels, int nr_rays, float* surfs_rgb,
                                float* surfs_alpha, float* surfs_normals, float* coeffs_out,
                                float* act_out, void* stream) {
  if (!plan || nr_rays < 0) return VSA_ERR_ARG;
  if (nr_rays == 0) return VSA_OK;
  if (!hit_slot || !tex_uv || !rays_d || !tris || !slot_of || !seg_start || !texels || !surfs_rgb ||
      !surfs_alpha)
    return VSA_ERR_ARG;
  if (plan->row_format < 0 || plan->row_format > 2) return VSA_ERR_UNSUPPORTED;
  dim3 grid = shade_grid(vsa_div_up(nr_rays, SH_BLOCK), plan->nr_shells);
  if (plan->row_format != 0)
    hipLaunchKernelGGL((nt_shade_fwd_kernel<false, true>), grid, dim3(SH_BLOCK), 0, (hipStream_t)stream, *plan,
                       hit_slot, tex_uv, rays_d, reinterpret_cast<const float4*>(tris), slot_of,
                       seg_start, reinterpret_cast<const unsigned*>(texels), nr_rays, surfs_rgb,
                       surfs_alpha, surfs_normals, coeffs_out, reinterpret_cast<float4*>(act_out));
  else if (plan->rgb_degrees == VSA_NT_MAX_DEG && plan->alpha_degrees == VSA_NT_MAX_DEG)
    hipLaunchKernelGGL(nt_shade_fwd_kernel<true>, grid, dim3(SH_BLOCK), 0, (hipStream_t)stream, *plan,
                       hit_slot, tex_uv, rays_d, reinterpret_cast<const float4*>(tris), slot_of,
                       seg_start, reinterpret_cast<const unsigned*>(texels), nr_rays, surfs_rgb,
                       surfs_alpha, surfs_normals, coeffs_out, reinterpret_cast<float4*>(act_out));
  else
    hipLaunchKernelGGL(nt_shade_fwd_kernel<false>, grid, dim3(SH_BLOCK), 0, (hipStream_t)stream, *plan,
                       hit_slot, tex_uv, rays_d, reinterpret_cast<const float4*>(tris), slot_of,
                       seg_start, reinterpret_cast<const unsigned*>(texels), nr_rays, surfs_rgb,
                       surfs_alpha, surfs_normals, coeffs_out, reinterpret_cast<float4*>(act_out));
  VSA_RETURN_LAUNCH_STATUS();
}

extern "C" int vsa_nt_shade_bwd(const vsa_nt_plan* plan, const int32_t* hit_slot,
                                const float* tex_uv, const float* rays_d, const float* tris,
                                const int32_t* slot_of, const int32_t* seg_start,
                                const uint8_t* texels, int nr_rays, const float* g_surfs_rgb,
                                const float* g_surfs_alpha, float grad_scale, uint16_t* grad_rows,
                                const float* act_in, void* stream) {
  if (!plan || nr_rays < 0) return VSA_ERR_ARG;
  if (nr_rays == 0) return VSA_OK;
  if (!hit_slot || !tex_uv || !rays_d || !tris || !slot_of || !seg_start || !texels || !g_surfs_rgb ||
      !g_surfs_alpha || !grad_rows)
    return VSA_ERR_ARG;
  if (plan->row_base[VSA_MAX_SHELLS * VSA_NT_MAX_DEG] * 8 >= (1ll << 32)) return VSA_ERR_UNSUPPORTED;
  if (plan->row_format < 0 || plan->row_format > 2) return VSA_ERR_UNSUPPORTED;
  dim3 grid = shade_grid(vsa_div_up(nr_rays, SHB_BLOCK), plan->nr_shells);
  const bool full4 = plan->rgb_degrees == VSA_NT_MAX_DEG && plan->alpha_degrees == VSA_NT_MAX_DEG;
  if (act_in && full4)
    hipLaunchKernelGGL((nt_shade_bwd_kernel<false, true>), grid, dim3(SHB_BLOCK), 0, (hipStream_t)stream, *plan,
                       hit_slot, tex_uv, rays_d, reinterpret_cast<const float4*>(tris), slot_of,
                       seg_start, reinterpret_cast<const unsigned*>(texels), nr_rays, g_surfs_rgb,
                       g_surfs_alpha, grad_scale, reinterpret_cast<_Float16*>(grad_rows),
                       reinterpret_cast<const float4*>(act_in));
  else if (act_in)
    hipLaunchKernelGGL((nt_shade_bwd_kernel<false, false>), grid, dim3(SHB_BLOCK), 0, (hipStream_t)stream, *plan,
                       hit_slot, tex_uv, rays_d, reinterpret_cast<const float4*>(tris), slot_of,
                       seg_start, reinterpret_cast<const unsigned*>(texels), nr_rays, g_surfs_rgb,
                       g_surfs_alpha, grad_scale, reinterpret_cast<_Float16*>(grad_rows),
                       reinterpret_cast<const float4*>(act_in));
  else if (plan->row_format != 0)
    hipLaunchKernelGGL((nt_shade_bwd_kernel<true, false, true>), grid, dim3(SHB_BLOCK), 0, (hipStream_t)stream, *plan,
                       hit_slot, tex_uv, rays_d, reinterpret_cast<const float4*>(tris), slot_of,
                       seg_start, reinterpret_cast<const unsigned*>(texels), nr_rays, g_surfs_rgb,
                       g_surfs_alpha, grad_scale, reinterpret_cast<_Float16*>(grad_rows), nullptr);
  else
    hipLaunchKernelGGL((nt_shade_bwd_kernel<true, false>), grid, dim3(SHB_BLOCK), 0, (hipStream_t)stream, *plan,
                       hit_slot, tex_uv, rays_d, reinterpret_cast<const float4*>(tris), slot_of,
                       seg_start, reinterpret_cast<const unsigned*>(texels), nr_rays, g_surfs_rgb,
                       g_surfs_alpha, grad_scale, reinterpret_cast<_Float16*>(grad_rows), nullptr);
  VSA_RETURN_LAUNCH_STATUS();
}

#ifdef SHADE_SPAN
extern "C" int vsa_span_read_shade(void* dst) {
  VSA_HIP_TRY(hipDeviceSynchronize());
  VSA_HIP_TRY(hipMemcpyFromSymbol(dst, HIP_SYMBOL(g_sspan), sizeof(g_sspan)));
  return 0;
}
#endif
```

### volsurfs_amd/csrc/raygen.hip

```cpp
#include "common.h"
#include "pcg32.h"
#include "pinhole.h"

namespace {

__device__ __forceinline__ void store_ray(const RayOut& r, float x, float y, long long i,
                                          float* __restrict__ rays_o, float* __restrict__ rays_d,
                                          float* __restrict__ points_2d) {
  rays_o[3 * i] = r.ox, rays_o[3 * i + 1] = r.oy, rays_o[3 * i + 2] = r.oz;
  rays_d[3 * i] = r.dx, rays_d[3 * i + 1] = r.dy, rays_d[3 * i + 2] = r.dz;
  if (points_2d) points_2d[2 * i] = x, points_2d[2 * i + 1] = y;
}

__global__ __launch_bounds__(256) void camera_rays_kernel(
    const float* __restrict__ c2w, const float* __restrict__ kinv, int W, int R, int jitter,
    unsigned long long rng_state, unsigned long long rng_inc, long long n_rays,
    float* __restrict__ rays_o, float* __restrict__ rays_d, float* __restrict__ points_2d) {
  const long long i = (long long)blockIdx.x * 256 + threadIdx.x;
  if (i >= n_rays) return;
  const long long pixel = i / R;
  const int row = (int)(pixel / W), col = (int)(pixel % W);
  float jx = 0.5f, jy = 0.5f;
  if (jitter) {
    Pcg32 rng{rng_state, rng_inc};
    rng.advance(2ull * (unsigned long long)i);
    jx = rng.next_float();
    jy = rng.next_float();
  }
  const float x = (float)col + jx, y = (float)row + jy;
  store_ray(pinhole_ray(c2w, kinv, x, y), x, y, i, rays_o, rays_d, points_2d);
}

struct ReelDummy {
  float o[3], d[3], rgb[3];
};

__global__ __launch_bounds__(256) void reel_rays_kernel(
    const float* __restrict__ c2w_all, const float* __restrict__ kinv_all,
    const float* __restrict__ rgb_all, const float* __restrict__ mask_all, int C, int H, int W,
    int B, int R, int jitter, unsigned long long rng_state, unsigned long long rng_inc,
    int* __restrict__ camera_idx, float* __restrict__ rays_o, float* __restrict__ rays_d,
    float* __restrict__ gt_rgb, float* __restrict__ gt_mask, float* __restrict__ points_2d,
    const vsa_train_ctl* __restrict__ ctl, ReelDummy dummy) {
  const long long b = (long long)blockIdx.x * 256 + threadIdx.x;
  if (ctl) {
    rng_state = ctl->rng_state;
    rng_inc = ctl->rng_inc;
    if (b >= ctl->capacity) return;
    if (b >= ctl->nr_rays) {
      camera_idx[b] = 0;
      if (gt_rgb) {
#pragma unroll
        for (int c = 0; c < 3; ++c) gt_rgb[3 * b + c] = dummy.rgb[c];
      }
      if (gt_mask) gt_mask[b] = 0.f;
      for (int s = 0; s < R; ++s) {
        const long long i = b * R + s;
#pragma unroll
        for (int c = 0; c < 3; ++c) rays_o[3 * i + c] = dummy.o[c], rays_d[3 * i + c] = dummy.d[c];
        if (points_2d) points_2d[2 * i] = points_2d[2 * i + 1] = 0.f;
      }
      return;
    }
  } else if (b >= B) {
    return;
  }
  Pcg32 rng{rng_state, rng_inc};
  rng.advance((unsigned long long)b * (unsigned long long)(3 + (jitter ? 2 * R : 0)));
  const int cam = min((int)(rng.next_float() * (float)C), C - 1);
  const int col = min((int)(rng.next_float() * (float)W), W - 1);
  const int row = min((int)(rng.next_float() * (float)H), H - 1);
  camera_idx[b] = cam;
  const long long px = ((long long)cam * H + row) * W + col;
  if (gt_rgb) {
#pragma unroll
    for (int c = 0; c < 3; ++c) gt_rgb[3 * b + c] = rgb_all[3 * px + c];
  }
  if (gt_mask) gt_mask[b] = mask_all[px];
  const float* c2w = c2w_all + 12ll * cam;
  const float* kinv = kinv_all + 9ll * cam;
  for (int s = 0; s < R; ++s) {
    float jx = 0.5f, jy = 0.5f;
    if (jitter) {
      jx = rng.next_float();
      jy = rng.next_float();
    }
    const float x = (float)col + jx, y = (float)row + jy;
    store_ray(pinhole_ray(c2w, kinv, x, y), x, y, b * R + s, rays_o, rays_d, points_2d);
  }
}

__device__ __forceinline__ int tile_x_of(int j) { return (j & 8) ? 7 - (j & 7) : (j & 7); }

struct __attribute__((packed, aligned(4))) F3 {
  float x, y, z;
};

template <int C>
__global__ __launch_bounds__(256) void tile_order_kernel(const float* __restrict__ src,
                                                         float* __restrict__ dst, int W, long long n,
                                                         int inverse) {
  const long long i = (long long)blockIdx.x * 256 + threadIdx.x;
  if (i >= n) return;
  const int tiles_x = W >> 3;
  const long long t = i >> 6;
  const int j = (int)(i & 63);
  const long long row = (t / tiles_x) * 8 + (j >> 3), col = (t % tiles_x) * 8 + tile_x_of(j);
  const long long px = row * W + col;
  const long long from = inverse ? i : px, to = inverse ? px : i;
  if constexpr (C == 3) {
    *reinterpret_cast<F3*>(dst + to * 3) = *reinterpret_cast<const F3*>(src + from * 3);
  } else {
#pragma unroll
    for (int c = 0; c < C; ++c) dst[to * C + c] = src[from * C + c];
  }
}

__global__ __launch_bounds__(256) void tile_order_rays_kernel(
    const float* __restrict__ o, const float* __restrict__ d, const float* __restrict__ gt,
    float* __restrict__ o_t, float* __restrict__ d_t, float* __restrict__ gt_t, int W, long long n) {
  const long long i = (long long)blockIdx.x * 256 + threadIdx.x;
  if (i >= n) return;
  const int tiles_x = W >> 3;
  const long long t = i >> 6;
  const int j = (int)(i & 63);
  const long long px = ((t / tiles_x) * 8 + (j >> 3)) * W + (t % tiles_x) * 8 + tile_x_of(j);
  const F3 vo = *reinterpret_cast<const F3*>(o + 3 * px), vd = *reinterpret_cast<const F3*>(d + 3 * px);
  F3 vg = {0.f, 0.f, 0.f};
  if (gt) vg = *reinterpret_cast<const F3*>(gt + 3 * px);
  *reinterpret_cast<F3*>(o_t + 3 * i) = vo;
  *reinterpret_cast<F3*>(d_t + 3 * i) = vd;
  if (gt) *reinterpret_cast<F3*>(gt_t + 3 * i) = vg;
}

}

extern "C" int vsa_tile_order_rays(const float* rays_o, const float* rays_d, const float* gt_rgb,
                                   float* rays_o_tiled, float* rays_d_tiled, float* gt_rgb_tiled,
                                   int height, int width, void* stream) {
  if (height < 0 || width < 0 || (height & 7) || (width & 7)) return VSA_ERR_ARG;
  const long long n = (long long)height * width;
  if (n == 0) return VSA_OK;
  if (!rays_o || !rays_d || !rays_o_tiled || !rays_d_tiled || (gt_rgb && !gt_rgb_tiled)) return VSA_ERR_ARG;
  hipLaunchKernelGGL(tile_order_rays_kernel, dim3(vsa_div_up(n, 256)), dim3(256), 0, (hipStream_t)stream,
                     rays_o, rays_d, gt_rgb, rays_o_tiled, rays_d_tiled, gt_rgb_tiled, width, n);
  VSA_RETURN_LAUNCH_STATUS();
}

extern "C" int vsa_tile_order(const float* src, float* dst, int height, int width, int channels,
                              int inverse, void* stream) {
  if (height < 0 || width < 0 || (height & 7) || (width & 7)) return VSA_ERR_ARG;
  const long long n = (long long)height * width;
  if (n == 0) return VSA_OK;
  if (!src || !dst || src == dst) return VSA_ERR_ARG;
  const dim3 grid(vsa_div_up(n, 256)), block(256);
  switch (channels) {
    case 1: hipLaunchKernelGGL(tile_order_kernel<1>, grid, block, 0, (hipStream_t)stream, src, dst, width, n, inverse); break;
    case 2: hipLaunchKernelGGL(tile_order_kernel<2>, grid, block, 0, (hipStream_t)stream, src, dst, width, n, inverse); break;
    case 3: hipLaunchKernelGGL(tile_order_kernel<3>, grid, block, 0, (hipStream_t)stream, src, dst, width, n, inverse); break;
    case 4: hipLaunchKernelGGL(tile_order_kernel<4>, grid, block, 0, (hipStream_t)stream, src, dst, width, n, inverse); break;
    default: return VSA_ERR_UNSUPPORTED;
  }
  VSA_RETURN_LAUNCH_STATUS();
}

extern "C" int vsa_camera_rays(const float* c2w, const float* intrinsics_inv, int height, int width,
                               int nr_rays_per_pixel, int jitter_pixels, uint64_t rng_state,
                               uint64_t rng_inc, float* rays_o, float* rays_d, float* points_2d,
                               void* stream) {
  if (height < 0 || width < 0 || nr_rays_per_pixel < 1) return VSA_ERR_ARG;
  const long long n = (long long)height * width * nr_rays_per_pixel;
  if (n == 0) return VSA_OK;
  if (!c2w || !intrinsics_inv || !rays_o || !rays_d) return VSA_ERR_ARG;
  if (n > 0x7fffffffll * 256) return VSA_ERR_UNSUPPORTED;
  hipLaunchKernelGGL(camera_rays_kernel, dim3(vsa_div_up(n, 256)), dim3(256), 0, (hipStream_t)stream,
                     c2w, intrinsics_inv, width, nr_rays_per_pixel, jitter_pixels,
                     (unsigned long long)rng_state, (unsigned long long)rng_inc, n, rays_o, rays_d,
                     points_2d);
  VSA_RETURN_LAUNCH_STATUS();
}

extern "C" int vsa_reel_next_rays_batch(const float* c2w_all, const float* intrinsics_inv_all,
                                        const float* rgb_all, const float* mask_all, int nr_cameras,
                                        int height, int width, int batch_size, int nr_rays_per_pixel,
                                        int jitter_pixels, uint64_t rng_state, uint64_t rng_inc,
                                        int32_t* camera_idx, float* rays_o, float* rays_d,
                                        float* gt_rgb, float* gt_mask, float* points_2d,
                                        void* stream) {
  if (batch_size < 0 || nr_rays_per_pixel < 1) return VSA_ERR_ARG;
  if (batch_size == 0) return VSA_OK;
  if (nr_cameras < 1 || height < 1 || width < 1) return VSA_ERR_ARG;
  if (!c2w_all || !intrinsics_inv_all || !camera_idx || !rays_o || !rays_d) return VSA_ERR_ARG;
  if ((gt_rgb && !rgb_all) || (gt_mask && !mask_all)) return VSA_ERR_ARG;
  hipLaunchKernelGGL(reel_rays_kernel, dim3(vsa_div_up(batch_size, 256)), dim3(256), 0,
                     (hipStream_t)stream, c2w_all, intrinsics_inv_all, rgb_all, mask_all, nr_cameras,
                     height, width, batch_size, nr_rays_per_pixel, jitter_pixels,
                     (unsigned long long)rng_state, (unsigned long long)rng_inc, camera_idx, rays_o,
                     rays_d, gt_rgb, gt_mask, points_2d, (const vsa_train_ctl*)nullptr, ReelDummy{});
  VSA_RETURN_LAUNCH_STATUS();
}

extern "C" int vsa_reel_next_rays_batch_ctl(const float* c2w_all, const float* intrinsics_inv_all,
                                            const float* rgb_all, const float* mask_all, int nr_cameras, int height,
                                            int width, int capacity, int nr_rays_per_pixel, int jitter_pixels,
                                            const vsa_train_ctl* ctl, const float* dummy_o, const float* dummy_d,
                                            const float* dummy_rgb, int32_t* camera_idx, float* rays_o,
                                            float* rays_d, float* gt_rgb, float* gt_mask, float* points_2d,
                                            void* stream) {
  if (capacity < 1 || nr_rays_per_pixel < 1 || nr_cameras < 1 || height < 1 || width < 1) return VSA_ERR_ARG;
  if (!ctl || !dummy_o || !dummy_d || !dummy_rgb || !c2w_all || !intrinsics_inv_all || !camera_idx || !rays_o || !rays_d)
    return VSA_ERR_ARG;
  if ((gt_rgb && !rgb_all) || (gt_mask && !mask_all)) return VSA_ERR_ARG;
  ReelDummy dm;
  for (int c = 0; c < 3; ++c) dm.o[c] = dummy_o[c], dm.d[c] = dummy_d[c], dm.rgb[c] = dummy_rgb[c];
  hipLaunchKernelGGL(reel_rays_kernel, dim3(vsa_div_up(capacity, 256)), dim3(256), 0, (hipStream_t)stream, c2w_all,
                     intrinsics_inv_all, rgb_all, mask_all, nr_cameras, height, width, capacity, nr_rays_per_pixel,
                     jitter_pixels, 0ull, 0ull, camera_idx, rays_o, rays_d, gt_rgb, gt_mask, points_2d, ctl, dm);
  VSA_RETURN_LAUNCH_STATUS();
}

namespace {
__global__ void intersect_primitive_kernel(const float* __restrict__ rays_o,
                                           const float* __restrict__ rays_d, int N, int kind,
                                           float size, unsigned char* __restrict__ is_hit,
                                           float* __restrict__ t_near, float* __restrict__ t_far,
                                           float* __restrict__ p_near, float* __restrict__ p_far) {
  const long long n = (long long)blockIdx.x * blockDim.x + threadIdx.x;
  if (n >= N) return;
  const float o[3] = {rays_o[3 * n], rays_o[3 * n + 1], rays_o[3 * n + 2]};
  const float d[3] = {rays_d[3 * n], rays_d[3 * n + 1], rays_d[3 * n + 2]};
  float tn, tf;
  bool hit;
  if (kind == 0) {
    tn = -INFINITY;
    tf = INFINITY;
#pragma unroll
    for (int i = 0; i < 3; ++i) {
      const float inv = 1.0f / d[i];
      const float a = (-size - o[i]) * inv, b = (size - o[i]) * inv;
      tn = fmaxf(tn, fminf(a, b));
      tf = fminf(tf, fmaxf(a, b));
    }
    hit = tn <= tf && tf > 0.0f;
  } else {
    const float a = (d[0] * d[0] + d[1] * d[1]) + d[2] * d[2];
    const float b = 2.0f * ((o[0] * d[0] + o[1] * d[1]) + o[2] * d[2]);
    const float c = ((o[0] * o[0] + o[1] * o[1]) + o[2] * o[2]) - size * size;
    const float disc = b * b - (4.0f * a) * c;
    const float sq = sqrtf(fmaxf(disc, 0.0f));
    tn = (-b - sq) / (2.0f * a);
    tf = (-b + sq) / (2.0f * a);
    hit = disc >= 0.0f && tf > 0.0f;
  }
  tn = hit ? fmaxf(tn, 0.0f) : 0.0f;
  tf = hit ? tf : 0.0f;
  is_hit[n] = hit ? 1 : 0;
  t_near[n] = tn;
  t_far[n] = tf;
#pragma unroll
  for (int i = 0; i < 3; ++i) {
    if (p_near) p_near[3 * n + i] = o[i] + tn * d[i];
    if (p_far) p_far[3 * n + i] = o[i] + tf * d[i];
  }
}
}

extern "C" int vsa_intersect_primitive(const float* rays_o, const float* rays_d, int nr_rays,
                                       int kind, float size, uint8_t* is_hit, float* t_near,
                                       float* t_far, float* points_near, float* points_far,
                                       void* stream) {
  if (nr_rays < 0 || (kind != 0 && kind != 1) || !(size > 0.0f)) return VSA_ERR_ARG;
  if (nr_rays == 0) return VSA_OK;
  if (!rays_o || !rays_d || !is_hit || !t_near || !t_far) return VSA_ERR_ARG;
  hipLaunchKernelGGL(intersect_primitive_kernel, dim3(vsa_div_up(nr_rays, 256)), dim3(256), 0,
                     (hipStream_t)stream, rays_o, rays_d, nr_rays, kind, size, is_hit, t_near, t_far,
                     points_near, points_far);
  VSA_RETURN_LAUNCH_STATUS();
}
```

### volsurfs_amd/csrc/trace.hip

```cpp
#include "common.h"
#include "trace_walk.h"
#include <algorithm>
#include <cstdio>
#include <cstdlib>

namespace {

__device__ __forceinline__ bool box_test(float lx, float ly, float lz, float hx, float hy,
                                         float hz, float ox, float oy, float oz, float ix,
                                         float iy, float iz, float t_min, float t_max,
                                         float& t_near) {
  float a = (lx - ox) * ix, b = (hx - ox) * ix;
  float tn = fminf(a, b), tf = fmaxf(a, b);
  a = (ly - oy) * iy;
  b = (hy - oy) * iy;
  tn = fmaxf(tn, fminf(a, b));
  tf = fminf(tf, fmaxf(a, b));
  a = (lz - oz) * iz;
  b = (hz - oz) * iz;
  tn = fmaxf(tn, fminf(a, b));
  tf = fminf(tf, fmaxf(a, b));
  t_near = tn;
  return tn <= tf * 1.0000004f + 1e-30f && tf >= t_min && tn <= t_max;
}

#ifdef TRACE_SPAN
constexpr int TRACE_SPAN_WAVES = 1 << 17;
static __device__ unsigned long long g_tspan[TRACE_SPAN_WAVES][3];
static __device__ int g_torder[TRACE_SPAN_WAVES];
static __device__ int g_torder_on;
__device__ __forceinline__ unsigned long long trace_now() {
  unsigned long long t;
  asm volatile("s_memrealtime %0\n\ts_waitcnt lgkmcnt(0)" : "=s"(t)::"memory");
  return t;
}
enum { SP_ROUNDS, SP_VISITS, SP_OUTER };
#define SPAN_ADD(k, v)                                                                        \
  do {                                                                                        \
    const unsigned v__ = (unsigned)(v);                                                       \
    if ((int)threadIdx.x == __builtin_ctzll(__builtin_amdgcn_read_exec())) s_span[k] += v__;  \
  } while (0)
#endif

template <int STACK>
__global__ __launch_bounds__(TRACE_BLOCK) void trace_ww_kernel(
    const float4* __restrict__ nodes, const float4* __restrict__ tris, Roots roots,
    const float* __restrict__ rays_o, const float* __restrict__ rays_d, int N, float t_min,
    float* __restrict__ hit_t, int* __restrict__ hit_slot, float* __restrict__ hit_uv) {
  __shared__ int s_stack[STACK][TRACE_BLOCK];
  const int lane = threadIdx.x;
  const long long n = (long long)blockIdx.x * TRACE_BLOCK + lane;
  const int mesh = blockIdx.y;
  if (n >= N) return;
  const float ox = rays_o[3 * n], oy = rays_o[3 * n + 1], oz = rays_o[3 * n + 2];
  const float dx = rays_d[3 * n], dy = rays_d[3 * n + 1], dz = rays_d[3 * n + 2];
  const float ix = 1.0f / dx, iy = 1.0f / dy, iz = 1.0f / dz;

  Hit best = no_hit();
  int cur = roots.root[mesh];
  int sp = 0;
  while (cur != TRACE_EMPTY) {
    while ((unsigned)cur < (unsigned)TRACE_EMPTY) {
      const float4 q0 = nodes[4 * (long long)cur + 0];
      const float4 q1 = nodes[4 * (long long)cur + 1];
      const float4 q2 = nodes[4 * (long long)cur + 2];
      const float4 q3 = nodes[4 * (long long)cur + 3];
      const int ref0 = __float_as_int(q3.x), ref1 = __float_as_int(q3.y);
      const int cnt0 = __float_as_int(q3.z), cnt1 = __float_as_int(q3.w);
      float tn0, tn1;
      bool h0 = box_test(q0.x, q0.y, q0.z, q0.w, q1.x, q1.y, ox, oy, oz, ix, iy, iz, t_min, best.t, tn0);
      bool h1 = box_test(q1.z, q1.w, q2.x, q2.y, q2.z, q2.w, ox, oy, oz, ix, iy, iz, t_min, best.t, tn1);
      const int c0 = ref0 < 0 ? ~(((~ref0) << 4) | cnt0) : ref0;
      const int c1 = ref1 < 0 ? ~(((~ref1) << 4) | cnt1) : ref1;
      h0 = h0 && !(ref0 < 0 && cnt0 == 0);
      h1 = h1 && !(ref1 < 0 && cnt1 == 0);
      if (h0 && h1) {
        const bool swap = tn1 < tn0;
        s_stack[sp++][lane] = swap ? c0 : c1;
        cur = swap ? c1 : c0;
      } else if (h0) {
        cur = c0;
      } else if (h1) {
        cur = c1;
      } else {
        cur = sp ? s_stack[--sp][lane] : TRACE_EMPTY;
      }
    }
    if (cur != TRACE_EMPTY) {
      leaf_test(tris, cur, ox, oy, oz, dx, dy, dz, t_min, best);
      cur = sp ? s_stack[--sp][lane] : TRACE_EMPTY;
    }
  }
  write_hit(best, (long long)mesh * N + n, hit_t, hit_slot, hit_uv);
}

template <int STACK>
__global__ __launch_bounds__(TRACE_BLOCK) void trace_q_kernel(
    const uint4* __restrict__ qnodes, const float4* __restrict__ tris, Roots roots, Frames frames,
    const float* __restrict__ rays_o, const float* __restrict__ rays_d, int N, float t_min,
    float* __restrict__ hit_t, int* __restrict__ hit_slot, float* __restrict__ hit_uv, int rpw) {
  __shared__ int s_stack[STACK][TRACE_BLOCK];
  const int lane = threadIdx.x;
#ifndef TRACE_SPAN
  if (lane >= rpw) return;
  const long long n = (long long)blockIdx.x * rpw + lane;
  const int mesh = blockIdx.y;
#else
  int item = blockIdx.y * gridDim.x + blockIdx.x;
  if (g_torder_on) item = g_torder[item];
  const int mesh = item / (int)gridDim.x;
  const long long n = (long long)(item - mesh * (int)gridDim.x) * TRACE_BLOCK + lane;
  const unsigned long long span_t0 = trace_now();
  __shared__ unsigned s_span[8];
  if (threadIdx.x < 8) s_span[threadIdx.x] = 0;
#endif
  if (n >= N) return;
  const float ox = rays_o[3 * n], oy = rays_o[3 * n + 1], oz = rays_o[3 * n + 2];
  const float dx = rays_d[3 * n], dy = rays_d[3 * n + 1], dz = rays_d[3 * n + 2];
  const QRay qr = make_qray(frames.f[mesh], ox, oy, oz, dx, dy, dz);
  Hit best = no_hit();
  int cur = roots.root[mesh];
  int sp = 0;
  while (cur != TRACE_EMPTY) {
#ifdef TRACE_SPAN
    SPAN_ADD(SP_OUTER, 1);
#endif
    while ((unsigned)cur < (unsigned)TRACE_EMPTY) {
#ifdef TRACE_SPAN
      SPAN_ADD(SP_ROUNDS, 1);
      SPAN_ADD(SP_VISITS, __builtin_popcountll(__builtin_amdgcn_read_exec()));
#endif
      const uint4 a = qnodes[2 * (long long)cur], b = qnodes[2 * (long long)cur + 1];
      float tn0, tn1;
      const bool h0 = qbox_test(a.x, a.y, a.z, qr, t_min, best.t, tn0);
      const bool h1 = qbox_test(a.w, b.x, b.y, qr, t_min, best.t, tn1);
      const int c0 = (int)b.z, c1 = (int)b.w;
      if (h0 && h1) {
        const bool swap = tn1 < tn0;
        s_stack[sp++][lane] = swap ? c0 : c1;
        cur = swap ? c1 : c0;
      } else if (h0) {
        cur = c0;
      } else if (h1) {
        cur = c1;
      } else {
        cur = sp ? s_stack[--sp][lane] : TRACE_EMPTY;
      }
    }
    if (cur != TRACE_EMPTY) {
      leaf_test(tris, cur, ox, oy, oz, dx, dy, dz, t_min, best);
      cur = sp ? s_stack[--sp][lane] : TRACE_EMPTY;
    }
  }
// ... 26 lines not shown
  const unsigned b = __float_as_uint(t);
  const unsigned o = b ^ ((b >> 31) ? 0xffffffffu : 0x80000000u);
  return ((unsigned long long)o << 32) | (unsigned)id;
}
__device__ __forceinline__ float coop_key_t(unsigned long long k) {
  const unsigned o = (unsigned)(k >> 32);
  return __uint_as_float(o ^ ((o >> 31) ? 0x80000000u : 0xffffffffu));
}

template <int STACK>
__device__ __forceinline__ int q_finish_coop(const uint4* __restrict__ qnodes, const float4* __restrict__ tris,
                                          const QRay& qr, float ox, float oy, float oz, float dx, float dy,
                                          float dz, float t_min, int& cur, int& sp, Hit& best,
                                          int (*s_stack)[TRACE_BLOCK], TraceCoop& L, int lane) {
  constexpr int QCAP = STACK * TRACE_BLOCK < TRACE_COOP_Q ? STACK * TRACE_BLOCK : TRACE_COOP_Q;
  int* const qn = &s_stack[0][0];
  const bool strag = cur != TRACE_EMPTY;
  const int mine = strag ? sp + 1 : 0;
  int incl = mine, top = strag ? sp : 0;
#pragma unroll
  for (int off = 1; off < 64; off <<= 1) {
    const int o = __shfl_up(incl, off, 64);
    if (lane >= off) incl += o;
    top = max(top, __shfl_xor(top, off, 64));
  }
  int count = __shfl(incl, 63, 64);
  const int F = top * TRACE_BLOCK;
  if (count > QCAP / 2 || F + count > STACK * TRACE_BLOCK) return -1;
  if (strag) {
    const int base = incl - mine;
    L.key[lane] = coop_key(best.t, best.id);
    L.slot[lane] = best.slot;
    qn[F + base] = cur;
    L.qr[base] = (unsigned char)lane;
    for (int k = 0; k < sp; ++k) {
      qn[F + base + 1 + k] = s_stack[k][lane];
      L.qr[base + 1 + k] = (unsigned char)lane;
    }
  }
  if (F)
    for (int i = lane; i < count; i += TRACE_BLOCK) {
      const int e = qn[F + i];
      qn[i] = e;
    }
  const unsigned long long lt = lane ? (~0ull >> (64 - lane)) : 0ull;
  int rounds = 0;
  while (count > 0) {
    ++rounds;
    const int P = count > QCAP - 128 - STACK ? 1 : min(64, count);
    const int start = count - P;
    const bool have = lane < P;
    const int e = have ? qn[start + lane] : TRACE_EMPTY;
    const int r = have ? (int)L.qr[start + lane] : lane;
    count = start;
    const unsigned long long k0 = L.key[r];
    bool h0 = false, h1 = false;
    int c0 = 0, c1 = 0;
    {
      QRay q;
      const float ix = __shfl(qr.ix.x, r, 64), iy = __shfl(qr.iy.x, r, 64), iz = __shfl(qr.iz.x, r, 64);
      const float cx = __shfl(qr.cx.x, r, 64), cy = __shfl(qr.cy.x, r, 64), cz = __shfl(qr.cz.x, r, 64);
      q.ix = f32x2_t{ix, ix}, q.iy = f32x2_t{iy, iy}, q.iz = f32x2_t{iz, iz};
      q.cx = f32x2_t{cx, cx}, q.cy = f32x2_t{cy, cy}, q.cz = f32x2_t{cz, cz};
      if (have && e >= 0) {
        const uint4 a = qnodes[2 * (long long)e], b = qnodes[2 * (long long)e + 1];
        float tn0, tn1;
        const float tb = coop_key_t(k0);
        h0 = qbox_test(a.x, a.y, a.z, q, t_min, tb, tn0);
        h1 = qbox_test(a.w, b.x, b.y, q, t_min, tb, tn1);
        c0 = (int)b.z, c1 = (int)b.w;
      }
    }
    __builtin_amdgcn_sched_barrier(0);
    Hit hb;
    hb.t = coop_key_t(k0), hb.id = (int)(unsigned)k0, hb.u = hb.v = 0.f, hb.slot = -1;
    {
      const float rox = __shfl(ox, r, 64), roy = __shfl(oy, r, 64), roz = __shfl(oz, r, 64);
      const float rdx = __shfl(dx, r, 64), rdy = __shfl(dy, r, 64), rdz = __shfl(dz, r, 64);
      if (have && e < 0) {
        const int code = ~e;
        const int first = code >> 4, cnt = code & 15;
#pragma nounroll
        for (int i = 0; i < cnt; ++i) {
          const long long s = first + i;
          tri_test(tris[3 * s], tris[3 * s + 1], tris[3 * s + 2], rox, roy, roz, rdx, rdy, rdz, t_min, first + i, hb);
        }
      }
    }
    __builtin_amdgcn_sched_barrier(0);
    const bool better = hb.slot >= 0;
    const unsigned long long mykey = coop_key(hb.t, hb.id);
    if (better) atomicMin(&L.key[r], mykey);
    const unsigned long long m0 = __builtin_amdgcn_ballot_w64(h0), m1 = __builtin_amdgcn_ballot_w64(h1);
    const int n0 = __builtin_popcountll(m0);
    if (h0) {
      const int p = count + __builtin_popcountll(m0 & lt);
      qn[p] = c0;
      L.qr[p] = (unsigned char)r;
    }
    if (h1) {
      const int p = count + n0 + __builtin_popcountll(m1 & lt);
      qn[p] = c1;
      L.qr[p] = (unsigned char)r;
    }
    count += n0 + __builtin_popcountll(m1);
    if (better && L.key[r] == mykey) L.slot[r] = hb.slot;
  }
  if (strag) {
    const unsigned long long k = L.key[lane];
    const int slot = L.slot[lane];
    if (slot != best.slot) {
      Hit w = no_hit();
      tri_test(tris[3 * (long long)slot], tris[3 * (long long)slot + 1], tris[3 * (long long)slot + 2], ox, oy, oz, dx, dy,
               dz, t_min, slot, w);
      best = w;
    }
    (void)k;
  }
  cur = TRACE_EMPTY;
  sp = 0;
  return rounds;
}

struct TraceFeedback {
  const int* prev;
  const unsigned char* prev_flag;
  const int* prev_lists;
  int* next;
  unsigned char* next_flag;
  int* next_lists;
  int cap;
};
struct TraceFeedbackBuf {
  char* half[2];
  long long flags_bytes;
  const int* phase_word;
  int phase, cap;
};
__device__ __forceinline__ TraceFeedback trace_fb_select(const TraceFeedbackBuf& b) {
  const int ph = (b.phase_word ? __builtin_amdgcn_readfirstlane(*b.phase_word) : b.phase) & 1;
  char* prev = b.half[ph];
  char* next = b.half[ph ^ 1];
  TraceFeedback fb;
  fb.prev = reinterpret_cast<const int*>(prev);
  fb.prev_flag = reinterpret_cast<const unsigned char*>(prev + 16);
  fb.prev_lists = reinterpret_cast<const int*>(prev + 16 + b.flags_bytes);
  fb.next = reinterpret_cast<int*>(next);
  fb.next_flag = reinterpret_cast<unsigned char*>(next + 16);
  fb.next_lists = reinterpret_cast<int*>(next + 16 + b.flags_bytes);
  fb.cap = b.cap;
  return fb;
}
__global__ void trace_fb_flip_kernel(int* phase_word, char* half0, char* half1) {
  const int ph = (*phase_word ^ 1) & 1;
  if (threadIdx.x == 0) *phase_word = ph;
  if (threadIdx.x < 4) reinterpret_cast<int*>(ph ? half0 : half1)[threadIdx.x] = 0;
}
#ifndef TRACE_FB_T
#define TRACE_FB_T 160, 128, 64
#endif
constexpr int TRACE_FB_TS[3] = {TRACE_FB_T};
constexpr int TRACE_FB_T0 = TRACE_FB_TS[0], TRACE_FB_T1 = TRACE_FB_TS[1], TRACE_FB_T2 = TRACE_FB_TS[2];

template <int STACK, bool COOP>
__global__ __launch_bounds__(TRACE_BLOCK) void trace_qf_kernel(
    const uint4* __restrict__ qnodes, const float4* __restrict__ tris, Roots roots, Frames frames,
    const float* __restrict__ rays_o, const float* __restrict__ rays_d, int N, int G, int nr_items, float t_min,
    TraceFeedbackBuf fbb, float* __restrict__ hit_t, int* __restrict__ hit_slot, float* __restrict__ hit_uv,
    int coop_chunk, int coop_lanes) {
  __shared__ int s_stack[STACK][TRACE_BLOCK];
  const int lane = threadIdx.x;
  const TraceFeedback fb = trace_fb_select(fbb);
  int item = blockIdx.x;
  {
    int n0 = 0, n1 = 0, n2 = 0;
    if (fb.prev[0] == nr_items) n0 = min(fb.prev[1], fb.cap), n1 = min(fb.prev[2], fb.cap), n2 = min(fb.prev[3], fb.cap);
    const int heavy = n0 + n1 + n2;
    if (item < heavy) {
      const int l = item < n0 ? 0 : item < n0 + n1 ? 1 : 2;
      item = fb.prev_lists[l * fb.cap + (item - (l == 0 ? 0 : l == 1 ? n0 : n0 + n1))];
    } else {
      item -= heavy;
      if (item >= nr_items) return;
      if (heavy && fb.prev_flag[item]) return;
    }
  }
  const int mesh = item / G;
  const long long n_raw = (long long)(item - mesh * G) * TRACE_BLOCK + lane;
  const bool alive = n_raw < N;
  const long long n = alive ? n_raw : N - 1;
  const float ox = rays_o[3 * n], oy = rays_o[3 * n + 1], oz = rays_o[3 * n + 2];
  const float dx = rays_d[3 * n], dy = rays_d[3 * n + 1], dz = rays_d[3 * n + 2];
  const QRay qr = make_qray(frames.f[mesh], ox, oy, oz, dx, dy, dz);
  Hit best = no_hit();
  int cur = alive ? roots.root[mesh] : TRACE_EMPTY;
  int sp = 0;
  int trips = 0;
  if constexpr (COOP) {
    __shared__ TraceCoop s_coop;
    for (int chunk = coop_chunk;;) {
      trips += q_walk<STACK, true>(qnodes, tris, qr, ox, oy, oz, dx, dy, dz, t_min, cur, sp, best, s_stack, lane, chunk);
      const unsigned long long left = __builtin_amdgcn_ballot_w64(cur != TRACE_EMPTY);
      if (left == 0) break;
      if (__builtin_popcountll(left) > coop_lanes) continue;
      const int rounds = q_finish_coop<STACK>(qnodes, tris, qr, ox, oy, oz, dx, dy, dz, t_min, cur, sp, best, s_stack,
                                              s_coop, lane);
      if (rounds >= 0) {
        trips += rounds;
        break;
      }
    }
  } else {
    trips = q_walk<STACK, true>(qnodes, tris, qr, ox, oy, oz, dx, dy, dz, t_min, cur, sp, best, s_stack, lane, 0x7fffffff);
  }
  if (alive) write_hit(best, (long long)mesh * N + n, hit_t, hit_slot, hit_uv);
  if (lane == 0) {
    const int l = trips >= TRACE_FB_T0 ? 0 : trips >= TRACE_FB_T1 ? 1 : trips >= TRACE_FB_T2 ? 2 : 3;
    bool listed = false;
    if (l < 3) {
      const int idx = atomicAdd(&fb.next[1 + l], 1);
      listed = idx < fb.cap;
      if (listed) fb.next_lists[l * fb.cap + idx] = item;
    }
    fb.next_flag[item] = listed ? 1 : 0;
    if (item == 0) fb.next[0] = nr_items;
  }
}

template <int STACK>
__global__ __launch_bounds__(TRACE_BLOCK) void trace_q_count_kernel(
    const uint4* __restrict__ qnodes, const float4* __restrict__ tris, Roots roots, Frames frames,
    const float* __restrict__ rays_o, const float* __restrict__ rays_d, int N, float t_min,
    unsigned long long* __restrict__ stats) {
  __shared__ int s_stack[STACK][TRACE_BLOCK];
  const int lane = threadIdx.x;
  const long long n = (long long)blockIdx.x * TRACE_BLOCK + lane;
  const int mesh = blockIdx.y;
  WalkCounts wc = {};
  int trips = 0, max_trips = 0;
  if (n < N) {
    const float ox = rays_o[3 * n], oy = rays_o[3 * n + 1], oz = rays_o[3 * n + 2];
    const float dx = rays_d[3 * n], dy = rays_d[3 * n + 1], dz = rays_d[3 * n + 2];
    const QRay qr = make_qray(frames.f[mesh], ox, oy, oz, dx, dy, dz);
    Hit best = no_hit();
    int cur = roots.root[mesh], sp = 0;
    trips = q_walk<STACK, false, true>(qnodes, tris, qr, ox, oy, oz, dx, dy, dz, t_min, cur, sp, best, s_stack, lane, 0,
                                       &wc);
  }
  int visits = wc.visits, tests = wc.tests;
  for (int o = 32; o > 0; o >>= 1) {
    visits += __shfl_down(visits, o);
    tests += __shfl_down(tests, o);
  }
  max_trips = trips;
  if (lane == 0) {
    atomicAdd(&stats[0], (unsigned long long)visits);
    atomicAdd(&stats[1], (unsigned long long)tests);
    atomicAdd(&stats[2], (unsigned long long)trips);
    atomicAdd(&stats[3], 1ull);
    atomicMax(&stats[4], (unsigned long long)max_trips);
  }
}

extern "C" int vsa_trace_q_stats(const uint32_t* qnodes, const float* tris, const int32_t* mesh_roots,
                                 const float* mesh_frames, int nr_meshes, int max_depth,
                                 const float* rays_o, const float* rays_d, int nr_rays, float t_min,
                                 uint64_t* stats, void* stream) {
  if (nr_rays < 1) return VSA_ERR_ARG;
  if (const int rc = check_qtree(qnodes, tris, mesh_roots, mesh_frames, nr_meshes, max_depth, VSA_ERR_UNSUPPORTED)) return rc;
  if (!rays_o || !rays_d || !stats) return VSA_ERR_ARG;
  const QTree t = make_qtree(qnodes, tris, mesh_roots, mesh_frames, nr_meshes);
  VSA_HIP_TRY(hipMemsetAsync(stats, 0, 5 * sizeof(uint64_t), (hipStream_t)stream));
  dim3 grid(vsa_div_up(nr_rays, TRACE_BLOCK), nr_meshes), block(TRACE_BLOCK);
  with_stack(max_depth, [&](auto st) {
    hipLaunchKernelGGL(trace_q_count_kernel<decltype(st)::value>, grid, block, 0, (hipStream_t)stream, t.qnodes, t.tris,
                       t.roots, t.frames, rays_o, rays_d, nr_rays, t_min, reinterpret_cast<unsigned long long*>(stats));
  });
  VSA_RETURN_LAUNCH_STATUS();
}

__global__ void hit_attributes_kernel(const float4* __restrict__ tris,
                                      const float* __restrict__ rays_o,
                                      const float* __restrict__ rays_d,
                                      const float* __restrict__ hit_t,
                                      const int* __restrict__ hit_slot,
                                      const float* __restrict__ hit_uv, int N,
                                      unsigned char* __restrict__ is_hit,
                                      int* __restrict__ tri_id, float* __restrict__ positions,
                                      float* __restrict__ normals, float* __restrict__ bary) {
  const long long n = (long long)blockIdx.x * blockDim.x + threadIdx.x;
  if (n >= N) return;
  const int slot = hit_slot[n];
  float p[3] = {0, 0, 0}, nn[3] = {0, 0, 0}, b[3] = {0, 0, 0};
  int id = -1;
  if (slot >= 0) {
    const float t = hit_t[n];
    for (int c = 0; c < 3; ++c) p[c] = rays_o[3 * n + c] + t * rays_d[3 * n + c];
    const float4 v0 = tris[3 * (long long)slot], e1 = tris[3 * (long long)slot + 1],
                 e2 = tris[3 * (long long)slot + 2];
    id = __float_as_int(v0.w);
    float cx = e1.y * e2.z - e1.z * e2.y, cy = e1.z * e2.x - e1.x * e2.z,
          cz = e1.x * e2.y - e1.y * e2.x;
    float len = sqrtf(dot3(cx, cy, cz, cx, cy, cz));
    float inv = len > 0.f ? 1.0f / len : 0.f;
    nn[0] = cx * inv; nn[1] = cy * inv; nn[2] = cz * inv;
    const float u = hit_uv[2 * n], v = hit_uv[2 * n + 1];
    b[0] = (1.0f - u) - v; b[1] = u; b[2] = v;
  }
  if (is_hit) is_hit[n] = slot >= 0;
  if (tri_id) tri_id[n] = id;
  for (int c = 0; c < 3; ++c) {
    if (positions) positions[3 * n + c] = p[c];
    if (normals) normals[3 * n + c] = nn[c];
    if (bary) bary[3 * n + c] = b[c];
  }
}

}

extern "C" int vsa_trace(const float* nodes, const float* tris, const int32_t* mesh_roots,
                         int nr_meshes, int max_depth, const float* rays_o, const float* rays_d,
                         int nr_rays, float t_min, float* hit_t, int32_t* hit_slot, float* hit_uv,
                         void* stream) {
  if (nr_meshes < 1 || nr_meshes > VSA_MAX_SHELLS || nr_rays < 0 || !mesh_roots) return VSA_ERR_ARG;
  if (max_depth >= TRACE_STACK) return VSA_ERR_UNSUPPORTED;
  if (nr_rays == 0) return VSA_OK;
  if (!nodes || !tris || !rays_o || !rays_d || !hit_t || !hit_slot || !hit_uv) return VSA_ERR_ARG;
  const Roots r = make_roots(mesh_roots, nr_meshes);
  dim3 grid(vsa_div_up(nr_rays, TRACE_BLOCK), nr_meshes), block(TRACE_BLOCK);
  with_stack(max_depth, [&](auto st) {
    hipLaunchKernelGGL(trace_ww_kernel<decltype(st)::value>, grid, block, 0, (hipStream_t)stream,
                       reinterpret_cast<const float4*>(nodes), reinterpret_cast<const float4*>(tris), r, rays_o, rays_d,
                       nr_rays, t_min, hit_t, hit_slot, hit_uv);
  });
  VSA_RETURN_LAUNCH_STATUS();
}

extern "C" int vsa_trace_q_narrow(const uint32_t* qnodes, const float* tris, const int32_t* mesh_roots,
                                  const float* mesh_frames, int nr_meshes, int max_depth,
                                  const float* rays_o, const float* rays_d, int nr_rays, float t_min,
                                  float* hit_t, int32_t* hit_slot, float* hit_uv, int rays_per_wave,
                                  void* stream) {
  if (nr_rays < 0 || rays_per_wave < 1 || rays_per_wave > TRACE_BLOCK) return VSA_ERR_ARG;
  if (const int rc = check_qtree(qnodes, tris, mesh_roots, mesh_frames, nr_meshes, max_depth, VSA_ERR_UNSUPPORTED, nr_rays > 0))
    return rc;
  if (nr_rays == 0) return VSA_OK;
  if (!rays_o || !rays_d || !hit_t || !hit_slot || !hit_uv) return VSA_ERR_ARG;
  const QTree t = make_qtree(qnodes, tris, mesh_roots, mesh_frames, nr_meshes);
  dim3 grid(vsa_div_up(nr_rays, rays_per_wave), nr_meshes), block(TRACE_BLOCK);
  with_stack(max_depth, [&](auto st) {
    hipLaunchKernelGGL(trace_q_kernel<decltype(st)::value>, grid, block, 0, (hipStream_t)stream, t.qnodes, t.tris, t.roots,
                       t.frames, rays_o, rays_d, nr_rays, t_min, hit_t, hit_slot, hit_uv, rays_per_wave);
  });
  VSA_RETURN_LAUNCH_STATUS();
}

extern "C" int vsa_trace_q(const uint32_t* qnodes, const float* tris, const int32_t* mesh_roots,
                           const float* mesh_frames, int nr_meshes, int max_depth,
                           const float* rays_o, const float* rays_d, int nr_rays, float t_min,
                           float* hit_t, int32_t* hit_slot, float* hit_uv, void* stream) {
  return vsa_trace_q_narrow(qnodes, tris, mesh_roots, mesh_frames, nr_meshes, max_depth, rays_o, rays_d, nr_rays, t_min,
                            hit_t, hit_slot, hit_uv, TRACE_BLOCK, stream);
}

static long long trace_fb_half_bytes(long long items, int* cap_out) {
  const int cap = (int)std::min<long long>(items / 8 + 64, 1 << 27);
  if (cap_out) *cap_out = cap;
  return (16 + (items + 15) / 16 * 16 + 12ll * cap + 255) / 256 * 256;
}

extern "C" long long vsa_trace_feedback_bytes(int nr_rays, int nr_meshes) {
  if (nr_rays < 0 || nr_meshes < 1) return -1;
  return 2 * trace_fb_half_bytes((long long)vsa_div_up(nr_rays, TRACE_BLOCK) * nr_meshes, nullptr) + 256;
}

struct TraceCoopConfig {
  int chunk, lanes;
  long long max_waves;
};
static TraceCoopConfig& trace_coop_config() {
  static TraceCoopConfig cfg{TRACE_COOP_CHUNK, TRACE_COOP_LANES, TRACE_COOP_WAVES};
  return cfg;
}
extern "C" int vsa_trace_coop_config(int chunk, int lanes, long long max_waves) {
  if (chunk < 1 || lanes < 0 || lanes > TRACE_BLOCK || max_waves < 0) return VSA_ERR_ARG;
  trace_coop_config() = TraceCoopConfig{chunk, lanes, max_waves};
  return VSA_OK;
}

extern "C" int vsa_trace_q_fb(const uint32_t* qnodes, const float* tris, const int32_t* mesh_roots,
                              const float* mesh_frames, int nr_meshes, int max_depth, const float* rays_o,
                              const float* rays_d, int nr_rays, float t_min, float* hit_t, int32_t* hit_slot,
                              float* hit_uv, void* feedback, long long feedback_bytes, int phase, void* stream) {
  if (nr_rays < 0 || phase < 0 || phase > 2) return VSA_ERR_ARG;
  if (const int rc = check_qtree(qnodes, tris, mesh_roots, mesh_frames, nr_meshes, max_depth, VSA_ERR_UNSUPPORTED, nr_rays > 0))
    return rc;
  if (nr_rays == 0) return VSA_OK;
  if (!rays_o || !rays_d || !hit_t || !hit_slot || !hit_uv || !feedback) return VSA_ERR_ARG;
  const int G = vsa_div_up(nr_rays, TRACE_BLOCK);
  const long long items = (long long)G * nr_meshes;
  int cap = 0;
  if (items > 0x7fffffff / 2 || feedback_bytes < 2 * trace_fb_half_bytes(items, &cap) + 256 || ((uintptr_t)feedback & 15))
    return VSA_ERR_ARG;
  const long long half = ((feedback_bytes - 256) / 2) & ~255ll;
  const QTree t = make_qtree(qnodes, tris, mesh_roots, mesh_frames, nr_meshes);
  char* b = static_cast<char*>(feedback);
  TraceFeedbackBuf fb;
  fb.half[0] = b, fb.half[1] = b + half;
  fb.flags_bytes = (items + 15) / 16 * 16;
  fb.phase_word = phase == 2 ? reinterpret_cast<const int*>(b + 2 * half) : nullptr;
  fb.phase = phase & 1;
  fb.cap = cap;
  hipStream_t s = (hipStream_t)stream;
  if (phase == 2)
    hipLaunchKernelGGL(trace_fb_flip_kernel, dim3(1), dim3(64), 0, s, reinterpret_cast<int*>(b + 2 * half),
                       fb.half[0], fb.half[1]);
  else
    VSA_HIP_TRY(hipMemsetAsync(fb.half[phase ^ 1], 0, 16, s));
  dim3 grid((unsigned)(items + 3ll * cap)), block(TRACE_BLOCK);
  const TraceCoopConfig& cfg = trace_coop_config();
  const int coop_chunk = cfg.chunk, coop_lanes = cfg.lanes;
  const bool coop = coop_lanes > 0 && items <= cfg.max_waves;
  with_stack(max_depth, [&](auto st) {
    with_flag(coop, [&](auto co) {
      hipLaunchKernelGGL((trace_qf_kernel<decltype(st)::value, decltype(co)::value>), grid, block, 0, s, t.qnodes, t.tris,
                         t.roots, t.frames, rays_o, rays_d, nr_rays, G, (int)items, t_min, fb, hit_t, hit_slot, hit_uv,
                         coop_chunk, coop_lanes);
    });
  });
  VSA_RETURN_LAUNCH_STATUS();
}

extern "C" int vsa_hit_attributes(const float* tris, const float* rays_o, const float* rays_d,
                                  const float* hit_t, const int32_t* hit_slot,
                                  const float* hit_uv, int nr_rays, uint8_t* is_hit,
                                  int32_t* tri_id, float* positions, float* normals,
                                  float* barycentric, void* stream) {
  if (nr_rays < 0) return VSA_ERR_ARG;
  if (nr_rays == 0) return VSA_OK;
  if (!tris || !rays_o || !rays_d || !hit_t || !hit_slot || !hit_uv) return VSA_ERR_ARG;
  hipLaunchKernelGGL(hit_attributes_kernel, dim3(vsa_div_up(nr_rays, 256)), dim3(256), 0,
                     (hipStream_t)stream, reinterpret_cast<const float4*>(tris), rays_o, rays_d,
                     hit_t, hit_slot, hit_uv, nr_rays, is_hit, tri_id, positions, normals,
                     barycentric);
  VSA_RETURN_LAUNCH_STATUS();
}

#ifdef TRACE_SPAN
extern "C" int vsa_span_set_order(const void* order, int n) {
  VSA_HIP_TRY(hipDeviceSynchronize());
  const int on = order != nullptr;
  if (on) VSA_HIP_TRY(hipMemcpyToSymbol(HIP_SYMBOL(g_torder), order, sizeof(int) * n));
  VSA_HIP_TRY(hipMemcpyToSymbol(HIP_SYMBOL(g_torder_on), &on, sizeof(int)));
  return 0;
}
extern "C" int vsa_span_read_trace(void* dst) {
  VSA_HIP_TRY(hipDeviceSynchronize());
  VSA_HIP_TRY(hipMemcpyFromSymbol(dst, HIP_SYMBOL(g_tspan), sizeof(g_tspan)));
  return 0;
}
#endif
```

### volsurfs_amd/pipeline.py

```python
import torch

from . import _lib
from .camera import pinhole_rays
from .mesh import nested_shells, stress_shells
from .raytrace import RayTracer


GRAD_CHAIN_GAIN = 16.0

_CAPTURE_MODE = "thread_local"


class _no_gc:

    def __enter__(self):
        import gc
        gc.collect()
        self.was = gc.isenabled()
        gc.disable()

    def __exit__(self, *exc):
        import gc
        if self.was:
            gc.enable()
# ... 90 lines not shown
            rows = rows.to(device)
            o, d, gt = (x.view(H, W, 3)[rows].reshape(-1, 3).contiguous() for x in (o, d, gt))
            h_local = int(rows.numel())
        p = cls(meshes, o, d, gt, seed=seed, image_hw=(h_local, W), **kw)
        p.loss_rays = n_frame
        p.grad_scale = GRAD_CHAIN_GAIN * float(n_frame)
        p.res = res
        p.subdiv = subdiv
        p.scene_desc = ("stress shells: 4 lobes of depth 0.3 r across the view axis (non-convex, up to 6 crossings per "
                        "ray), triangle areas spread 12x, 256 randomly packed uv charts per shell, noise 0.05, "
                        f"parameters {kw.get('init', 'tcnn')}-initialised") if stress else \
            (f"noise {noise}, {atlas_charts}x{atlas_charts} randomly packed uv charts per shell, "
             f"parameters {kw.get('init', 'tcnn')}-initialised") if (noise or atlas_charts) else \
            "perfect spheres, one continuous octahedral uv chart, tcnn-initialised parameters"
        return p

    def reset_stage_timers(self):
        self.timer = StageTimer()

    def stage_report(self):
        return self.timer.report()

    @staticmethod
    def stage_roofline(st, hbm_peak, mfma_peak):
        sec = st["ms"] * 1e-3
        out = {}
        if st.get("bytes"):
            out["GB/s"] = round(st["bytes"] / sec / 1e9, 1)
            out["hbm_frac"] = round(st["bytes"] / sec / 1e9 / hbm_peak, 4)
        if st.get("flops"):
            out["TFLOP/s"] = round(st["flops"] / sec / 1e12, 2)
            out["mfma_frac"] = round(st["flops"] / sec / 1e12 / mfma_peak, 4)
        return out

    def config_desc(self, world):
        return {
            "workload": f"synthetic kitten-like: {self.res if isinstance(self.res, int) else self.res[1]}x"
                        f"{self.res if isinstance(self.res, int) else self.res[0]} rays, K={self.K} nested "
                        f"icospheres subdiv {self.subdiv} ({self.tracer.mesh_nr_tris[0]} tris each), "
                        "SH-degree-3 neural textures (rgb + alpha per shell, res 2048/1024/512/256, "
                        "16-level 2-D hash grid + 32-64-64-C MLP, 8-bit quantised, lerp), alpha decay, "
                        "white bg, L1 loss, gradients to all hash tables and MLP weights",
            "rays_per_gpu": self.nr_rays,
            "global_rays": self.loss_rays if self.loss_rays != self.nr_rays else self.nr_rays * world,
            "parallelism": f"tile-parallel x{world}",
            "hits_per_frame": getattr(self, "last_hits", None),
            "unique_texels_per_frame": getattr(self, "last_slots", None),
            "trace_launch_order": "cost feedback from the previous frame (static camera: the previous frame has "
                                  "the same rays; value_cold is the figure without any inter-frame feedback)"
                                  if self.tracer.cost_feedback and
                                  self.tracer.node_format == "q16" else "natural",
        }

    def stats(self):
        from .neural_textures import stage_accounting
        bank, N, K = self.bank, self.nr_rays, self.K
        self.last_hits = M = int((self._hit_slot >= 0).sum().item())
        nodes_b = self.tracer.nodes.numel() * 4 + self.tracer.tris.numel() * 4
        self.acct, self.mlp_flops_fwd, self.last_slots = stage_accounting(bank, N, M, nodes_b)
        return self.last_hits, self.last_slots

    def capture_graph_split(self, **step_kw):
        self._static_rgb = None
        self._graph_dp = dp = step_kw.get("dp")
        s = torch.cuda.Stream()
        s.wait_stream(torch.cuda.current_stream())
        hook, _ = (dp.on_weights_final, setattr(dp, "on_weights_final", None)) if dp is not None else (None, None)
        with torch.cuda.stream(s):
            for _ in range(2):
                self.step(**step_kw)
        if dp is not None:
            dp.on_weights_final = hook
        torch.cuda.current_stream().wait_stream(s)
        self._graph_prefix, self._graph_mid, self._graph_tail = (torch.cuda.CUDAGraph() for _ in range(3))
        with _no_gc():
            with torch.cuda.graph(self._graph_prefix, capture_error_mode=_CAPTURE_MODE):
                self.step(part="prefix", **step_kw)
            with torch.cuda.graph(self._graph_mid, pool=self._graph_prefix.pool(), capture_error_mode=_CAPTURE_MODE):
                self.step(part="mid", **step_kw)
            with torch.cuda.graph(self._graph_tail, pool=self._graph_prefix.pool(), capture_error_mode=_CAPTURE_MODE):
                self._static_rgb = self.step(part="tail", **step_kw)

    def replay_prefix(self):
        self._graph_prefix.replay()

    def _count_replay(self):
        dp = getattr(self, "_graph_dp", None)
        if dp is not None:
            dp.epoch_host += 1

    def replay_mid(self):
        self._graph_mid.replay()
        self._count_replay()

    def replay_tail(self):
        self._graph_tail.replay()
        return self._static_rgb

    def replay_rest(self):
        self._graph_mid.replay()
        self._count_replay()
        self._graph_tail.replay()
        return self._static_rgb

    def capture_graph(self, **step_kw):
        self._static_rgb = None
        self._graph_dp = dp = step_kw.get("dp")
        s = torch.cuda.Stream()
        s.wait_stream(torch.cuda.current_stream())
        hook, _ = (dp.on_weights_final, setattr(dp, "on_weights_final", None)) if dp is not None else (None, None)
        with torch.cuda.stream(s):
            for _ in range(2):
                self.step(**step_kw)
        if dp is not None:
            dp.on_weights_final = hook
        torch.cuda.current_stream().wait_stream(s)
        self._graph = torch.cuda.CUDAGraph()
        with _no_gc(), torch.cuda.graph(self._graph, capture_error_mode=_CAPTURE_MODE):
            self._static_rgb = self.step(**step_kw)
        return self._graph

    def replay(self):
        self._graph.replay()
        self._count_replay()
        return self._static_rgb

    def step(self, record=False, grad_ready=None, dp=None, part=None):
        from .composite import composite_fwd_raw, composite_bwd_raw
        N, K = self.nr_rays, self.K
        T, bank = self.timer, self.bank
        acct = getattr(self, "acct", None) or {}

        if part == "tail":
            return self._step_tail(record, acct, grad_ready, dp, self._mid_out)
        if part in ("rest", "mid"):
            rays_d, gt, hit_slot, tex_uv = self._prefix_out
        else:
            rays_d, gt, hit_slot, tex_uv = self._step_prefix(record, acct)
            if part == "prefix":
                self._prefix_out = (rays_d, gt, hit_slot, tex_uv)
                return None
        T.run("zero_grad", bank.zero_grads, record, bytes=(bank.tables.numel() + bank.weights.numel()) * 4)
        rgb = self._step_rest(record, acct, dp, rays_d, gt, hit_slot, tex_uv)
        if part == "mid":
            self._mid_out = rgb
            return None
        if dp is not None and dp.on_weights_final is not None and not torch.cuda.is_current_stream_capturing():
            dp.on_weights_final()
        return self._step_tail(record, acct, grad_ready, dp, rgb)

    def _step_prefix(self, record, acct):
        N, T, bank = self.nr_rays, self.timer, self.bank
        rays_o, rays_d, gt = self.rays_o, self.rays_d, self.gt
        if self.image_hw is not None:
            H, W = self.image_hw

            T.run("ray_tile_order",
                  lambda: _lib.call("vsa_tile_order_rays", self.rays_o, self.rays_d, self.gt, self._o_t,
                                    self._d_t, self._gt_t, H, W, _lib.stream_ptr()),
                  record, bytes=N * 72)
            rays_o, rays_d, gt = self._o_t, self._d_t, self._gt_t
        hit_t, hit_slot, hit_uv = T.run(
            "trace", lambda: self.tracer.trace_all(rays_o, rays_d), record,
            bytes=acct.get("trace", 0))
        self._hit_slot = hit_slot
        tex_uv = T.run("nt_mark_compact",
                       lambda: bank.mark_and_compact(hit_slot, hit_uv, self.face_uvs), record,
                       bytes=acct.get("nt_mark_compact", 0))
        return rays_d, gt, hit_slot, tex_uv

    def _step_rest(self, record, acct, dp, rays_d, gt, hit_slot, tex_uv):
        N, K = self.nr_rays, self.K
        T, bank = self.timer, self.bank
        mlp_flops = getattr(self, "mlp_flops_fwd", 0)
        from . import neural_textures as _nt
        if _nt.FUSED_FORWARD is True:
            T.run("nt_encode_mlp_fwd", bank.encode_mlp, record, bytes=acct.get("nt_encode_mlp_fwd", 0),
                  flops=mlp_flops, bound="mfma")
        else:
            T.run("nt_encode_fwd", bank.encode, record, bytes=acct.get("nt_encode_fwd", 0))
            T.run("nt_mlp_fwd", bank.mlp, record, bytes=acct.get("nt_mlp_fwd", 0), flops=mlp_flops,
                  bound="mfma")
        rgb_k, alpha_k, _, _ = T.run(
            "nt_shade_fwd", lambda: bank.shade(hit_slot, tex_uv, rays_d, self.tracer.tris,
                                               act_out=self._act),
            record, bytes=acct.get("nt_shade_fwd", 0))
        self.surfs_rgb, self.surfs_alpha = rgb_k, alpha_k
        from .composite import composite_fwd_bwd_l1_raw
        rgb, g_c, g_a = T.run("composite_fwd_bwd",
                              lambda: composite_fwd_bwd_l1_raw(rgb_k, alpha_k, self.bg, gt,
                                                               1.0 / (3.0 * self.loss_rays)),
                              record, bytes=N * (12 + 12 + 32 * K))
        if self.image_hw is not None:
            T.run("rgb_row_order", lambda: _lib.call("vsa_tile_order", rgb, self._rgb_out, self.image_hw[0],
                                                     self.image_hw[1], 3, 1, _lib.stream_ptr()),
                  record, bytes=N * 24)
            rgb = self._rgb_out
        tris = self.tracer.tris
        T.run("nt_shade_bwd", lambda: bank.backward_shade(hit_slot, tex_uv, rays_d, tris, g_c, g_a,
                                                           self.grad_scale, self._act), record,
              bytes=acct.get("nt_shade_bwd", 0), bound="atomic")
        T.run("nt_mlp_bwd", lambda: bank.backward_mlp(self.grad_scale), record,
              bytes=acct.get("nt_mlp_bwd", 0), flops=2 * mlp_flops, bound="mfma")
        if dp is not None:
            dp.signal_weights()
        return rgb

    def _step_tail(self, record, acct, grad_ready, dp, rgb):
        K, T, bank = self.K, self.timer, self.bank
        enc_bytes = acct.get("nt_encode_bwd", 0)
        if dp is not None:
            T.run("nt_encode_bwd", lambda: bank.backward_encode_phased(self.grad_scale, dp), record,
                  bytes=enc_bytes)
        elif grad_ready is None:
            T.run("nt_encode_bwd", lambda: bank.backward_encode(self.grad_scale), record,
                  bytes=enc_bytes)
        else:
            grad_ready(bank.weights.grad)

            def by_shell():
                for s in range(K):
                    bank.backward_encode(self.grad_scale, shells=(s, s + 1))
                    grad_ready(bank.tables.grad[s * 8:(s + 1) * 8])
            T.run("nt_encode_bwd", by_shell, record, bytes=enc_bytes)
        return rgb
```

### volsurfs_amd/raytrace.py

```python
import ctypes
import os

import numpy as np
import torch

from . import _lib


def _rays(rays_o, rays_d):
    N = rays_o.shape[0]
    return N, _lib.check_f32(rays_o.contiguous(), N, 3), _lib.check_f32(rays_d.contiguous(), N, 3)


class RayTracer:
    BUILDERS = ("host", "device", "ploc")
    DEVICE_BUILDERS = ("device", "ploc")
    PLOC_RADIUS = 8

    def __init__(self, tensor_meshes, leaf_size=4, node_format=None, builder="host", ploc_radius=None):
        if builder not in self.BUILDERS:
            raise _lib.VolsurfsHipError(f"unknown builder {builder!r} (expected one of {self.BUILDERS})")
        self.builder = builder
        self.node_format = node_format or os.environ.get("VSA_TRACE_NODES", "q16")
        if self.node_format not in ("q16", "f32"):
# ... 31 lines not shown
        else:
            built = [build_one(vf) for vf in arrays]
        for rc, h in built:
            if rc != 0:
                raise _lib.VolsurfsHipError(f"vsa_bvh_build failed with status {rc}")
        sizes = []
        for _, h in built:
            self._bvh.append(h)
            nn, nt, md = ctypes.c_int(), ctypes.c_int(), ctypes.c_int()
            L.vsa_bvh_sizes(h, ctypes.byref(nn), ctypes.byref(nt), ctypes.byref(md))
            sizes.append((nn.value, nt.value, md.value))
        self._record_shells(sizes)
        dev = tensor_meshes[0].vertices.device
        self.device = dev
        nodes, qnodes, tris, frames = self._export()
        self.nodes = torch.from_numpy(nodes).to(dev)
        self.qnodes = torch.from_numpy(qnodes.view(np.int32)).to(dev)
        self._frames = (ctypes.c_float * (6 * self.nr_meshes))(*frames.tolist())
        self.tris = torch.from_numpy(tris).to(dev)
        self.slot_face_id = torch.from_numpy(tris[:, 3].copy().view(np.int32)).to(dev)

    def _record_shells(self, sizes):
        node_base = tri_base = 0
        for nn, nt, md in sizes:
            self._layout.append((node_base, nn, tri_base, nt))
            self.mesh_tri_offset.append(tri_base)
            self.mesh_nr_tris.append(nt)
            self.max_depth = max(self.max_depth, md)
            node_base += nn
            tri_base += nt
        self.roots = [lay[0] for lay in self._layout]
        self._roots = (ctypes.c_int32 * self.nr_meshes)(*self.roots)
        return node_base, tri_base

    def _build_on_device(self, tensor_meshes, leaf_size, radius):
        L = _lib.lib()
        dev = tensor_meshes[0].vertices.device
        if dev.type != "cuda":
            raise _lib.VolsurfsHipError(f'builder="{self.builder}" needs the meshes on the GPU')
        st = _lib.stream_ptr()
        inputs = []
        try:
            for m in tensor_meshes:
                v = m.vertices.detach().to(dev, torch.float32).contiguous()
                f = m.faces.detach().to(dev, torch.int32).contiguous()
                inputs.append((v, f))
                h = ctypes.c_void_p()
                if self.builder == "ploc":
                    name = "vsa_bvh_dev_build_ploc"
                    rc = L.vsa_bvh_dev_build_ploc(v.data_ptr(), f.data_ptr(), v.shape[0], f.shape[0], leaf_size, radius,
                                                  st, ctypes.byref(h))
                else:
                    name = "vsa_bvh_dev_build"
                    rc = L.vsa_bvh_dev_build(v.data_ptr(), f.data_ptr(), v.shape[0], f.shape[0], leaf_size, st,
                                             ctypes.byref(h))
                if rc != 0:
                    raise _lib.VolsurfsHipError(f"{name} failed with status {rc}")
                self._bvh.append(h)
            sizes = []
            for h in self._bvh:
                nn, nt, md = ctypes.c_int(), ctypes.c_int(), ctypes.c_int()
                rc = L.vsa_bvh_dev_sizes(h, ctypes.byref(nn), ctypes.byref(nt), ctypes.byref(md))
                if rc == -2 and md.value >= 48:
                    raise _lib.VolsurfsHipError(
                        f'builder="{self.builder}": tree depth {md.value} >= 48, deeper than the traversal stack; '
                        'build this mesh with builder="host"')
                if rc != 0:
                    raise _lib.VolsurfsHipError(f"vsa_bvh_dev_sizes failed with status {rc}")
                sizes.append((nn.value, nt.value, md.value))
        except Exception:
            self._destroy()
            raise
        node_base, tri_base = self._record_shells(sizes)
        self.device = dev
        self.nodes = torch.empty(node_base, 16, dtype=torch.float32, device=dev)
        self.qnodes = torch.empty(node_base, 8, dtype=torch.int32, device=dev)
        self.tris = torch.empty(tri_base, 12, dtype=torch.float32, device=dev)
        self._export_device()
        self.slot_face_id = self.tris[:, 3].contiguous().view(torch.int32)

    def _export_device(self):
        L = _lib.lib()
        frames = (ctypes.c_float * (6 * self.nr_meshes))()
        st = _lib.stream_ptr()
        for i, (h, (nb, nn, tb, nt)) in enumerate(zip(self._bvh, self._layout)):
            rc = L.vsa_bvh_dev_export(h, self.nodes[nb].data_ptr(), self.qnodes[nb].data_ptr(), self.tris[tb].data_ptr(),
                                      nb, tb, ctypes.addressof(frames) + 24 * i, st)
            if rc != 0:
                raise _lib.VolsurfsHipError(f"vsa_bvh_dev_export failed with status {rc}")
        self._frames = frames

    def _destroy(self):
        L = _lib.lib()
        for h in self._bvh:
            (L.vsa_bvh_dev_destroy if self.builder in self.DEVICE_BUILDERS else L.vsa_bvh_destroy)(h)
        self._bvh = []

    def _export(self):
        L = _lib.lib()
        n_nodes = sum(lay[1] for lay in self._layout)
        n_tris = sum(lay[3] for lay in self._layout)
        nodes = np.empty((n_nodes, 16), np.float32)
        qnodes = np.empty((n_nodes, 8), np.uint32)
        tris = np.empty((n_tris, 12), np.float32)
        frames = np.empty(6 * self.nr_meshes, np.float32)
        for i, (h, (nb, nn, tb, nt)) in enumerate(zip(self._bvh, self._layout)):
            rc = L.vsa_bvh_export(h, nodes[nb:nb + nn].ctypes.data_as(ctypes.c_void_p),
                                  tris[tb:tb + nt].ctypes.data_as(ctypes.c_void_p), ctypes.c_int(nb),
                                  ctypes.c_int(tb))
            rc2 = L.vsa_bvh_export_q(h, qnodes[nb:nb + nn].ctypes.data_as(ctypes.c_void_p),
                                     tris[tb:tb + nt].ctypes.data_as(ctypes.c_void_p), ctypes.c_int(nb),
                                     ctypes.c_int(tb), frames[6 * i:6 * i + 6].ctypes.data_as(ctypes.c_void_p))
            if rc != 0 or rc2 != 0:
                raise _lib.VolsurfsHipError(f"vsa_bvh_export failed with status {rc} / {rc2}")
        return nodes, qnodes, tris, frames

    def refit(self, tensor_meshes):
        if len(tensor_meshes) != self.nr_meshes:
            raise _lib.VolsurfsHipError("refit needs the meshes the tracer was built on")
        L = _lib.lib()
        self._meshes, self._pn = list(tensor_meshes), None
        self._wm = self._census = None
        if self.builder in self.DEVICE_BUILDERS:
            st = _lib.stream_ptr()
            for h, m in zip(self._bvh, tensor_meshes):
                v = m.vertices.detach().to(self.device, torch.float32).contiguous()
                rc = L.vsa_bvh_dev_refit(h, v.data_ptr(), v.shape[0], st)
                if rc != 0:
                    raise _lib.VolsurfsHipError(f"vsa_bvh_dev_refit failed with status {rc} (vertex count changed?)")
            self._export_device()
            self._fb = None
            return self
        for h, m in zip(self._bvh, tensor_meshes):
            v = np.ascontiguousarray(m.vertices.detach().cpu().numpy(), np.float32)
            rc = L.vsa_bvh_refit(h, v.ctypes.data_as(ctypes.c_void_p), ctypes.c_int(v.shape[0]))
            if rc != 0:
                raise _lib.VolsurfsHipError(f"vsa_bvh_refit failed with status {rc} (vertex count changed?)")
        nodes, qnodes, tris, frames = self._export()
        self.nodes.copy_(torch.from_numpy(nodes))
        self.qnodes.copy_(torch.from_numpy(qnodes.view(np.int32)))
        self.tris.copy_(torch.from_numpy(tris))
        self._frames = (ctypes.c_float * (6 * self.nr_meshes))(*frames.tolist())
        self._fb = None
        return self

    def __del__(self):
        try:
            if getattr(self, "_bvh", None):
                self._destroy()
        except Exception:
            pass
        self._bvh = []

    def trace_all(self, rays_o, rays_d, t_min=0.0, out=None):
        N, rays_o, rays_d = _rays(rays_o, rays_d)
        K = self.nr_meshes
        if out is not None:
            hit_t, hit_slot, hit_uv = out
            _lib.check_f32(hit_t, K, N)
            _lib.check_f32(hit_uv, K, N, 2)
            if hit_slot.dtype != torch.int32 or tuple(hit_slot.shape) != (K, N) or not hit_slot.is_contiguous():
                raise _lib.VolsurfsHipError("trace_all: out[1] must be a contiguous int32 [K, N] tensor")
        else:
            hit_t = torch.empty(K, N, device=rays_o.device)
            hit_slot = torch.empty(K, N, dtype=torch.int32, device=rays_o.device)
            hit_uv = torch.empty(K, N, 2, device=rays_o.device)
        rpw = self.narrow_rays_per_wave(N, K) if self.node_format == "q16" else 64
        if rpw < 64:
            _lib.call("vsa_trace_q_narrow", *self.q16_tree_args(), rays_o, rays_d, N, float(t_min), hit_t, hit_slot,
                      hit_uv, int(rpw), _lib.stream_ptr())
        elif self.node_format == "q16" and self.cost_feedback and self.max_depth < 48:
            if self._fb is None or self._fb[1] < N or self._fb[0].device != rays_o.device:
                fn = _lib.lib().vsa_trace_feedback_bytes
                fn.restype = ctypes.c_longlong
                nbytes = int(fn(ctypes.c_int(N), ctypes.c_int(K)))
                if nbytes < 0:
                    raise _lib.VolsurfsHipError("vsa_trace_feedback_bytes failed")
                self._fb = [torch.zeros(nbytes, dtype=torch.uint8, device=rays_o.device), N, nbytes]
            _lib.call("vsa_trace_q_fb", *self.q16_tree_args(), rays_o, rays_d, N, float(t_min), hit_t, hit_slot, hit_uv,
                      self._fb[0], ctypes.c_longlong(self._fb[2]), 2, _lib.stream_ptr())
        elif self.node_format == "q16":
            _lib.call("vsa_trace_q", *self.q16_tree_args(), rays_o, rays_d, N, float(t_min), hit_t, hit_slot, hit_uv,
                      _lib.stream_ptr())
        else:
            _lib.call("vsa_trace", self.nodes, self.tris, self._roots, K, self.max_depth, rays_o,
                      rays_d, N, float(t_min), hit_t, hit_slot, hit_uv, _lib.stream_ptr())
        return hit_t, hit_slot, hit_uv

    NARROW_BELOW = int(os.environ.get("VSA_TRACE_NARROW_BELOW", "0"))
    NARROW_RPW = 16

    @staticmethod
    def coop_config(chunk=16, lanes=24, max_waves=4096):
        _lib.call("vsa_trace_coop_config", int(chunk), int(lanes), ctypes.c_longlong(int(max_waves)))

    def narrow_rays_per_wave(self, N, K):
        return self.NARROW_RPW if N * K < self.NARROW_BELOW else 64

    def walk_stats(self, rays_o, rays_d, t_min=0.0):
        N, rays_o, rays_d = _rays(rays_o, rays_d)
        st = torch.zeros(5, dtype=torch.int64, device=rays_o.device)
        _lib.call("vsa_trace_q_stats", *self.q16_tree_args(), rays_o, rays_d, N, float(t_min), st, _lib.stream_ptr())
        v = st.cpu().tolist()
        return dict(zip(("lane_visits", "tri_tests", "wave_trips", "waves", "max_wave_trips"), v))

    def face_view_counts(self, cameras, supersample=1, t_min=0.0):
        from .visibility import tracer_face_view_counts
        return tracer_face_view_counts(self, cameras, supersample, t_min)

    def q16_tree_args(self, mesh_id=None):
        if mesh_id is None:
            return self.qnodes, self.tris, self._roots, self._frames, self.nr_meshes, self.max_depth
        return (self.qnodes, self.tris, (ctypes.c_int32 * 1)(self.roots[mesh_id]), self._frame_ptr(mesh_id), 1,
                self.max_depth)

    def require_q16(self, what, walk=True):
        if self.node_format != "q16":
            raise _lib.VolsurfsHipError(
                f'{what} walks the quantised nodes: the tracer was built with node_format="{self.node_format}", '
                'build it with node_format="q16"')
        if walk and self.max_depth >= 48:
            raise _lib.VolsurfsHipError(f"tree depth {self.max_depth} >= 48, deeper than the traversal stack")

    def _closest_args(self, points, what):
        self.require_q16(what)
        if not isinstance(points, torch.Tensor) or points.dim() != 2 or points.shape[1] != 3 or points.shape[0] < 1:
            raise _lib.VolsurfsHipError(f"{what}: expected points [N, 3] with N >= 1, got "
                                        f"{tuple(points.shape) if isinstance(points, torch.Tensor) else type(points)}")
        return _lib.check_f32(points.contiguous(), points.shape[0], 3)

    def closest_all(self, points):
        points = self._closest_args(points, "closest_all")
        K, N = self.nr_meshes, points.shape[0]
        dist = torch.empty(K, N, device=points.device)
        slot = torch.empty(K, N, dtype=torch.int32, device=points.device)
        bary = torch.empty(K, N, 2, device=points.device)
        _lib.call("vsa_closest_point_q", *self.q16_tree_args(), points, N, dist, slot, bary, _lib.stream_ptr())
        return {"dist": dist, "face": self._slot_faces(slot), "slot": slot, "bary": bary}

    def closest(self, points, mesh_id=0):
        points = self._closest_args(points, "closest")
        if not 0 <= int(mesh_id) < self.nr_meshes:
            raise _lib.VolsurfsHipError(f"closest: mesh_id {mesh_id} outside 0..{self.nr_meshes - 1}")
        N = points.shape[0]
        dist = torch.empty(N, device=points.device)
        slot = torch.empty(N, dtype=torch.int32, device=points.device)
        bary = torch.empty(N, 2, device=points.device)
        _lib.call("vsa_closest_point_q", *self.q16_tree_args(mesh_id), points, N, dist, slot, bary, _lib.stream_ptr())
        return {"dist": dist, "face": self._slot_faces(slot), "slot": slot, "bary": bary}

    def pseudonormal_tables(self):
        if self._pn is None:
            from .mesh_sdf import pseudonormals
            tables = [pseudonormals(m, device=self.device) for m in self._meshes]
            base = np.cumsum([0] + [t.shape[0] for t in tables[:-1]])
            self._pn = (torch.cat(tables) if len(tables) > 1 else tables[0],
                        (ctypes.c_longlong * self.nr_meshes)(*[int(b) for b in base]))
        return self._pn

    SIGNS = ("pseudonormal", "winding", "auto")

    def winding_moments(self):
        if self._wm is None:
            self.require_q16("winding_moments")
            nn, nt, K = self.qnodes.shape[0], self.tris.shape[0], self.nr_meshes
            nbytes = _lib.workspace_bytes("vsa_mesh_winding_moments_workspace_bytes", nn, K)
            ws = torch.empty(nbytes, dtype=torch.uint8, device=self.device)
            table = torch.empty(2 * nn + K, 8, device=self.device)
            _lib.call("vsa_mesh_winding_moments", self.qnodes, self.tris, self._roots, K, nn, nt, ws, nbytes, table,
                      _lib.stream_ptr())
            self._wm = (table, (ctypes.c_longlong * K)(*[2 * nn + k for k in range(K)]))
        return self._wm

    def edge_census(self, mesh_id=0):
        if self._census is None:
            self._census = [None] * self.nr_meshes
        if self._census[mesh_id] is None:
            from .mesh_winding import edge_census
            self._census[mesh_id] = edge_census(self._meshes[mesh_id], device=self.device)
        return self._census[mesh_id]

    def sign_rule(self, sign, mesh_ids=None):
        if sign not in self.SIGNS:
            raise ValueError(f"sign must be one of {self.SIGNS}, got {sign!r}")
        if sign != "auto":
            return sign
        ids = range(self.nr_meshes) if mesh_ids is None else mesh_ids
        return "winding" if any(any(self.edge_census(k).values()) for k in ids) else "pseudonormal"

    @staticmethod
    def _check_beta(beta):
        beta = float(beta)
        if not beta > 1.0:
            raise ValueError(f"beta must be > 1 (math.inf: every leaf is summed exactly), got {beta}")
        return beta

    def _winding_roots(self, mesh_id):
        table, entries = self.winding_moments()
        if mesh_id is None:
            return table, self._roots, entries, self.nr_meshes
        return table, (ctypes.c_int32 * 1)(self.roots[mesh_id]), (ctypes.c_longlong * 1)(entries[mesh_id]), 1

    def _winding(self, points, mesh_id, beta, what):
        points = self._closest_args(points, what)
        beta = self._check_beta(beta)
        if mesh_id is not None and not 0 <= int(mesh_id) < self.nr_meshes:
            raise _lib.VolsurfsHipError(f"{what}: mesh_id {mesh_id} outside 0..{self.nr_meshes - 1}")
        table, roots, entries, K = self._winding_roots(mesh_id)
        N = points.shape[0]
        w = torch.empty((K, N) if mesh_id is None else (N,), device=points.device)
        _lib.call("vsa_winding_number_q", self.qnodes, self.tris, roots, K, self.max_depth, table, entries, beta, points,
                  N, w, _lib.stream_ptr())
        return w

    def winding_number_all(self, points, beta=2.0):
        return self._winding(points, None, beta, "winding_number_all")

    def winding_number(self, points, mesh_id=0, beta=2.0):
        return self._winding(points, int(mesh_id), beta, "winding_number")

    def winding_stats(self, points, beta=2.0):
        points = self._closest_args(points, "winding_stats")
        table, roots, entries, K = self._winding_roots(None)
        st = torch.zeros(3, dtype=torch.int64, device=points.device)
        _lib.call("vsa_winding_number_q_stats", self.qnodes, self.tris, roots, K, self.max_depth, table, entries,
                  self._check_beta(beta), points, points.shape[0], st, _lib.stream_ptr())
        v = st.cpu().tolist()
        return {"node_visits": v[0], "tri_terms": v[1], "queries": v[2]}

    def _signed_w(self, points, mesh_id, beta):
        beta = self._check_beta(beta)
        table, _, entries, K = self._winding_roots(mesh_id)
        N = points.shape[0]
# ... 103 lines not shown
```

Measured before the change: 266.1.

## Fuse step prologue with feedback flip, scatter composite output, pair texel corner loads

Several changes land at once. A new step prologue kernel does the feedback-buffer phase flip together with ray tile reordering, and the trace then runs in a flipped mode. The composite forward/backward writes predicted RGB straight to row order, which removes the separate inverse tile-order pass. Neural-texture shading now loads horizontally adjacent texel rows as one pair with wider loads, storing two row indices per degree instead of four. Together these aim to cut kernel launches and memory passes, at the cost of more code paths and new alignment assumptions on the paired loads.

```diff
diff --git a/include/volsurfs_hip.h b/include/volsurfs_hip.h
--- a/include/volsurfs_hip.h
+++ b/include/volsurfs_hip.h
@@ -37,6 +37,10 @@
                                    float loss_scale, float* out_rgb, float* g_surfs_rgb,
                                    float* g_surfs_alpha, int nr_rays, int nr_shells, int carry_f16,
                                    void* stream);
+int vsa_composite_dense_fwd_bwd_l1_rows(const float* surfs_rgb, const float* surfs_alpha, const float* rgb_bg,
+                                        int bg_is_broadcast, const float* gt_rgb, float loss_scale, float* out_rgb,
+                                        float* g_surfs_rgb, float* g_surfs_alpha, int height, int width,
+                                        int nr_shells, int carry_f16, void* stream);
 
 long long vsa_reduce_scratch_bytes(void);
 int vsa_count_hits(const int32_t* hit_slot, long long n, void* scratch, int64_t* out, void* stream);
@@ -81,6 +85,10 @@
                    const float* mesh_frames, int nr_meshes, int max_depth, const float* rays_o,
                    const float* rays_d, int nr_rays, float t_min, float* hit_t, int32_t* hit_slot,
                    float* hit_uv, void* feedback, long long feedback_bytes, int phase, void* stream);
+int vsa_trace_q_fb_flipped(const uint32_t* qnodes, const float* tris, const int32_t* mesh_roots,
+                           const float* mesh_frames, int nr_meshes, int max_depth, const float* rays_o,
+                           const float* rays_d, int nr_rays, float t_min, float* hit_t, int32_t* hit_slot,
+                           float* hit_uv, void* feedback, long long feedback_bytes, void* stream);
 int vsa_trace_coop_config(int chunk, int lanes, long long max_waves);
 int vsa_trace_q_stats(const uint32_t* qnodes, const float* tris, const int32_t* mesh_roots,
                       const float* mesh_frames, int nr_meshes, int max_depth, const float* rays_o,
@@ -493,6 +501,10 @@
 int vsa_tile_order_rays(const float* rays_o, const float* rays_d, const float* gt_rgb,
                         float* rays_o_tiled, float* rays_d_tiled, float* gt_rgb_tiled, int height,
                         int width, void* stream);
+int vsa_step_prologue(void* feedback, long long feedback_bytes, int nr_meshes, const float* rays_o,
+                      const float* rays_d, const float* gt_rgb, float* rays_o_tiled, float* rays_d_tiled,
+                      float* gt_rgb_tiled, int height, int width, float* clear, long long clear_floats,
+                      void* stream);
 
 
 int vsa_occ_grid_points(const int32_t* point_indices, int nr_points, int nr_voxels_per_dim,
diff --git a/volsurfs_amd/composite.py b/volsurfs_amd/composite.py
--- a/volsurfs_amd/composite.py
+++ b/volsurfs_amd/composite.py
@@ -111,14 +111,22 @@
     return g_c, g_a
 
 
-def composite_fwd_bwd_l1_raw(surfs_rgb, surfs_alpha, rgb_bg, gt_rgb, loss_scale, carry_f16=False):
+def composite_fwd_bwd_l1_raw(surfs_rgb, surfs_alpha, rgb_bg, gt_rgb, loss_scale, carry_f16=False, image_hw=None,
+                             rgb_out=None):
     N, K, _ = surfs_rgb.shape
-    rgb = torch.empty(N, 3, device=surfs_rgb.device)
+    rgb = torch.empty(N, 3, device=surfs_rgb.device) if rgb_out is None else _lib.check_f32(rgb_out, N, 3)
     g_c = torch.empty_like(surfs_rgb)
     g_a = torch.empty_like(surfs_alpha)
     bcast = rgb_bg.shape[0] == 1 and N != 1
-    _lib.call("vsa_composite_dense_fwd_bwd_l1", surfs_rgb, surfs_alpha, rgb_bg, bcast, gt_rgb,
-              float(loss_scale), rgb, g_c, g_a, N, K, int(carry_f16), _lib.stream_ptr())
+    if image_hw is not None:
+        H, W = image_hw
+        if H * W != N:
+            raise _lib.VolsurfsHipError(f"image_hw {image_hw} does not hold {N} rays")
+        _lib.call("vsa_composite_dense_fwd_bwd_l1_rows", surfs_rgb, surfs_alpha, rgb_bg, bcast, gt_rgb,
+                  float(loss_scale), rgb, g_c, g_a, int(H), int(W), K, int(carry_f16), _lib.stream_ptr())
+    else:
+        _lib.call("vsa_composite_dense_fwd_bwd_l1", surfs_rgb, surfs_alpha, rgb_bg, bcast, gt_rgb,
+                  float(loss_scale), rgb, g_c, g_a, N, K, int(carry_f16), _lib.stream_ptr())
     return rgb, g_c, g_a
 
 
diff --git a/volsurfs_amd/csrc/composite_dense.hip b/volsurfs_amd/csrc/composite_dense.hip
--- a/volsurfs_amd/csrc/composite_dense.hip
+++ b/volsurfs_amd/csrc/composite_dense.hip
@@ -1,4 +1,5 @@
 #include "common.h"
+#include "tile_order.h"
 
 namespace {
 
@@ -174,7 +175,7 @@
     const float* __restrict__ rgb_bg, int bg_bcast, const float* __restrict__ g_rgb,
     float* __restrict__ g_surfs_rgb, float* __restrict__ g_surfs_alpha,
     float* __restrict__ g_rgb_bg, int N, const float* __restrict__ l1_gt, float l1_scale,
-    float* __restrict__ pred_out, const vsa_train_ctl* __restrict__ ctl) {
+    float* __restrict__ pred_out, const vsa_train_ctl* __restrict__ ctl, int pred_img_w) {
   using L = Lds<K>;
   int n_active = N;
   if (ctl) {
@@ -234,7 +235,14 @@
   slab_store<3 * K, L::SC>(g_surfs_rgb + ray0 * 3 * K, s_c, rows);
   slab_store<K, L::SA>(g_surfs_alpha + ray0 * K, s_a, rows);
   if (g_rgb_bg) slab_store<3, 3>(g_rgb_bg + ray0 * 3, s_b, rows);
-  if (pred_out) slab_store<3, 3>(pred_out + ray0 * 3, s_g, rows);
+  if (pred_out) {
+    if (pred_img_w) {
+      if (r < rows)
+        *reinterpret_cast<F3*>(pred_out + 3 * tile_pixel_of(ray0 + r, pred_img_w)) = *reinterpret_cast<const F3*>(s_g + 3 * r);
+    } else {
+      slab_store<3, 3>(pred_out + ray0 * 3, s_g, rows);
+    }
+  }
 }
 
 }
@@ -284,7 +292,7 @@
                                 float* g_surfs_rgb, float* g_surfs_alpha, float* g_rgb_bg,
                                 int nr_rays, int nr_shells, int carry_f16, const float* l1_gt,
                                 float l1_scale, void* stream, float* pred_out = nullptr,
-                                const vsa_train_ctl* ctl = nullptr) {
+                                const vsa_train_ctl* ctl = nullptr, int pred_img_w = 0) {
   if (nr_rays < 0) return VSA_ERR_ARG;
   if (nr_rays == 0) return VSA_OK;
   if (!surfs_rgb || !surfs_alpha || !rgb_bg || (!g_rgb && !pred_out) || !g_surfs_rgb || !g_surfs_alpha)
@@ -295,11 +303,11 @@
     if (carry_f16)
       hipLaunchKernelGGL((composite_dense_bwd_kernel<KK, true>), grid, block, 0, st, surfs_rgb,
                          surfs_alpha, rgb_bg, bg_is_broadcast, g_rgb, g_surfs_rgb, g_surfs_alpha,
-                         g_rgb_bg, nr_rays, l1_gt, l1_scale, pred_out, ctl);
+                         g_rgb_bg, nr_rays, l1_gt, l1_scale, pred_out, ctl, pred_img_w);
     else
       hipLaunchKernelGGL((composite_dense_bwd_kernel<KK, false>), grid, block, 0, st, surfs_rgb,
                          surfs_alpha, rgb_bg, bg_is_broadcast, g_rgb, g_surfs_rgb, g_surfs_alpha,
-                         g_rgb_bg, nr_rays, l1_gt, l1_scale, pred_out, ctl);
+                         g_rgb_bg, nr_rays, l1_gt, l1_scale, pred_out, ctl, pred_img_w);
   });
   VSA_RETURN_LAUNCH_STATUS();
 }
@@ -337,6 +345,20 @@
                               loss_scale, stream, out_rgb);
 }
 
+extern "C" int vsa_composite_dense_fwd_bwd_l1_rows(const float* surfs_rgb, const float* surfs_alpha,
+                                                   const float* rgb_bg, int bg_is_broadcast, const float* gt_rgb,
+                                                   float loss_scale, float* out_rgb, float* g_surfs_rgb,
+                                                   float* g_surfs_alpha, int height, int width, int nr_shells,
+                                                   int carry_f16, void* stream) {
+  if (height < 0 || width < 0 || (height & 7) || (width & 7)) return VSA_ERR_ARG;
+  const long long n = (long long)height * width;
+  if (n > 0x7fffffff) return VSA_ERR_UNSUPPORTED;
+  if (!gt_rgb || (n > 0 && !out_rgb)) return VSA_ERR_ARG;
+  return composite_bwd_launch(surfs_rgb, surfs_alpha, rgb_bg, bg_is_broadcast, nullptr, g_surfs_rgb,
+                              g_surfs_alpha, nullptr, (int)n, nr_shells, carry_f16, gt_rgb, loss_scale, stream,
+                              out_rgb, nullptr, width);
+}
+
 extern "C" int vsa_composite_dense_fwd_bwd_l1_ctl(const float* surfs_rgb, const float* surfs_alpha,
                                                   const float* rgb_bg, int bg_is_broadcast, const float* gt_rgb,
                                                   const vsa_train_ctl* ctl, float* out_rgb, float* g_surfs_rgb,
diff --git a/volsurfs_amd/csrc/nt_shade.hip b/volsurfs_amd/csrc/nt_shade.hip
--- a/volsurfs_amd/csrc/nt_shade.hip
+++ b/volsurfs_amd/csrc/nt_shade.hip
@@ -53,7 +53,7 @@
   bool hit;
   float dir[3];
   float decay;
-  int row[VSA_NT_MAX_DEG][4];
+  int row[VSA_NT_MAX_DEG][2];
   float w[VSA_NT_MAX_DEG][4];
   float fx[VSA_NT_MAX_DEG], fy[VSA_NT_MAX_DEG];
 };
@@ -126,7 +126,8 @@
   for (int d = 0; d < VSA_NT_MAX_DEG; ++d) {
     if (d >= D) {
 #pragma unroll
-      for (int k = 0; k < 4; ++k) c.row[d][k] = 0, c.w[d][k] = 0.f;
+      for (int k = 0; k < 4; ++k) c.w[d][k] = 0.f;
+      c.row[d][0] = c.row[d][1] = 0;
       c.fx[d] = c.fy[d] = 0.f;
       continue;
     }
@@ -137,9 +138,7 @@
     const int sd = s * VSA_NT_MAX_DEG + d;
     const int rb = (int)plan.row_base[sd] - seg_start[sd] * nt_row_quads(d);
     c.row[d][0] = rb + slot_of[base] * nt_row_quads(d);
-    c.row[d][1] = anchor ? c.row[d][0] : rb + slot_of[base + 1] * nt_row_quads(d);
-    c.row[d][2] = anchor ? c.row[d][0] : rb + slot_of[base + W] * nt_row_quads(d);
-    c.row[d][3] = anchor ? c.row[d][0] : rb + slot_of[base + W + 1] * nt_row_quads(d);
+    c.row[d][1] = anchor ? c.row[d][0] : rb + slot_of[base + W] * nt_row_quads(d);
     c.fx[d] = f.fx;
     c.fy[d] = f.fy;
     c.w[d][0] = (1.0f - f.fx) * (1.0f - f.fy);
@@ -151,53 +150,73 @@
 }
 
 template <bool F16ROWS>
-__device__ __forceinline__ void add_corner_row(const vsa_nt_plan& plan, int d, const unsigned* __restrict__ texels,
-                                               int row, float wk, const float* s_lut, float acc[28]) {
+__device__ __forceinline__ void add_corner_pair(const vsa_nt_plan& plan, int d, const unsigned* __restrict__ texels,
+                                                int row, bool pair, float w0, float w1, const float* s_lut,
+                                                float acc[28]) {
   const int n = 2 * d + 1;
+  const int xq = pair ? nt_row_quads(d) : 0;
   if constexpr (!F16ROWS) {
-    unsigned wds[8] = {0, 0, 0, 0, 0, 0, 0, 0};
+    unsigned wds[2][8] = {{0, 0, 0, 0, 0, 0, 0, 0}, {0, 0, 0, 0, 0, 0, 0, 0}};
     const unsigned* rp = texels + row;
     if (d == 0) {
-      const uint2 v = *reinterpret_cast<const uint2*>(rp);
-      wds[0] = v.x, wds[1] = v.y;
+      if (pair) {
+        uint4 v;
+        __builtin_memcpy(&v, __builtin_assume_aligned(rp, 8), 16);
+        wds[0][0] = v.x, wds[0][1] = v.y, wds[1][0] = v.z, wds[1][1] = v.w;
+      } else {
+        const uint2 v = *reinterpret_cast<const uint2*>(rp);
+        wds[0][0] = wds[1][0] = v.x, wds[0][1] = wds[1][1] = v.y;
+      }
     } else {
-      const uint4 lo = *reinterpret_cast<const uint4*>(rp);
-      wds[0] = lo.x, wds[1] = lo.y, wds[2] = lo.z, wds[3] = lo.w;
-      if (d >= 2) {
-        const uint4 hi = *reinterpret_cast<const uint4*>(rp + 4);
-        wds[4] = hi.x, wds[5] = hi.y, wds[6] = hi.z, wds[7] = hi.w;
-      }
-    }
-#pragma unroll
-    for (int i = 0; i < 3 * n; ++i) {
-      const unsigned q = (wds[i >> 2] >> (8 * (i & 3))) & 255u;
-      acc[i] = acc[i] + s_lut[d * 256 + q] * wk;
-    }
-#pragma unroll
-    for (int i = 0; i < n; ++i) {
-      const unsigned q = (wds[nt_alpha_quad(d) + (i >> 2)] >> (8 * (i & 3))) & 255u;
-      acc[21 + i] = acc[21 + i] + s_lut[d * 256 + q] * wk;
+#pragma unroll
+      for (int x = 0; x < 2; ++x) {
+        const unsigned* rx = rp + x * xq;
+        const uint4 lo = *reinterpret_cast<const uint4*>(rx);
+        wds[x][0] = lo.x, wds[x][1] = lo.y, wds[x][2] = lo.z, wds[x][3] = lo.w;
+        if (d >= 2) {
+          const uint4 hi = *reinterpret_cast<const uint4*>(rx + 4);
+          wds[x][4] = hi.x, wds[x][5] = hi.y, wds[x][6] = hi.z, wds[x][7] = hi.w;
+        }
+      }
+    }
+#pragma unroll
+    for (int x = 0; x < 2; ++x) {
+      const float wk = x ? w1 : w0;
+#pragma unroll
+      for (int i = 0; i < 3 * n; ++i) {
+        const unsigned q = (wds[x][i >> 2] >> (8 * (i & 3))) & 255u;
+        acc[i] = acc[i] + s_lut[d * 256 + q] * wk;
+      }
+#pragma unroll
+      for (int i = 0; i < n; ++i) {
+        const unsigned q = (wds[x][nt_alpha_quad(d) + (i >> 2)] >> (8 * (i & 3))) & 255u;
+        acc[21 + i] = acc[21 + i] + s_lut[d * 256 + q] * wk;
+      }
     }
   } else {
-    unsigned wds[16];
-    const uint4* rp = reinterpret_cast<const uint4*>(texels + 2 * (long long)row);
-    const int nv = d == 0 ? 1 : d == 1 ? 2 : 4;
-#pragma unroll
-    for (int v = 0; v < 4; ++v) {
-      const uint4 x = v < nv ? rp[v] : make_uint4(0, 0, 0, 0);
-      wds[4 * v] = x.x, wds[4 * v + 1] = x.y, wds[4 * v + 2] = x.z, wds[4 * v + 3] = x.w;
-    }
     const float lo = plan.sh_lo[d], span = plan.sh_span[d];
     const bool raw = plan.row_format == 2;
-    auto expand = [&](int elem) {
-      const unsigned short hb = (unsigned short)(wds[elem >> 1] >> (16 * (elem & 1)));
-      const float o = (float)__builtin_bit_cast(_Float16, hb);
-      return raw ? o : vsa_round_f16(lo + vsa_round_f16(vsa_pin_f32(span * o)));
-    };
-#pragma unroll
-    for (int i = 0; i < 3 * n; ++i) acc[i] = acc[i] + expand(i) * wk;
-#pragma unroll
-    for (int i = 0; i < n; ++i) acc[21 + i] = acc[21 + i] + expand(4 * nt_alpha_quad(d) + i) * wk;
+#pragma unroll
+    for (int x = 0; x < 2; ++x) {
+      unsigned wds[16];
+      const uint4* rp = reinterpret_cast<const uint4*>(texels + 2 * (long long)(row + x * xq));
+      const int nv = d == 0 ? 1 : d == 1 ? 2 : 4;
+#pragma unroll
+      for (int v = 0; v < 4; ++v) {
+        const uint4 t = v < nv ? rp[v] : make_uint4(0, 0, 0, 0);
+        wds[4 * v] = t.x, wds[4 * v + 1] = t.y, wds[4 * v + 2] = t.z, wds[4 * v + 3] = t.w;
+      }
+      const float wk = x ? w1 : w0;
+      auto expand = [&](int elem) {
+        const unsigned short hb = (unsigned short)(wds[elem >> 1] >> (16 * (elem & 1)));
+        const float o = (float)__builtin_bit_cast(_Float16, hb);
+        return raw ? o : vsa_round_f16(lo + vsa_round_f16(vsa_pin_f32(span * o)));
+      };
+#pragma unroll
+      for (int i = 0; i < 3 * n; ++i) acc[i] = acc[i] + expand(i) * wk;
+#pragma unroll
+      for (int i = 0; i < n; ++i) acc[21 + i] = acc[21 + i] + expand(4 * nt_alpha_quad(d) + i) * wk;
+    }
   }
 }
 
@@ -215,7 +234,8 @@
 #pragma unroll
     for (int i = 0; i < 28; ++i) acc[i] = 0.f;
 #pragma unroll
-    for (int k = 0; k < 4; ++k) add_corner_row<F16ROWS>(plan, d, texels, c.row[d][k], c.w[d][k], s_lut, acc);
+    for (int y = 0; y < 2; ++y)
+      add_corner_pair<F16ROWS>(plan, d, texels, c.row[d][y], plan.anchor == 0, c.w[d][2 * y], c.w[d][2 * y + 1], s_lut, acc);
 #pragma unroll
     for (int ch = 0; ch < 3; ++ch)
 #pragma unroll
@@ -225,7 +245,7 @@
   }
 }
 
-template <bool FULL4 = false, bool F16ROWS = false>
+template <bool FULL4 = false, bool F16ROWS = false, bool PAIR = true>
 __device__ __forceinline__ void shade_hit(const vsa_nt_plan& plan, const HitCtx& c,
                                           const unsigned* __restrict__ texels, const float* s_lut,
                                           bool has_alpha, const float b[16], float raw[4],
@@ -247,7 +267,8 @@
 #pragma unroll
     for (int i = 0; i < 28; ++i) acc[i] = 0.f;
 #pragma unroll
-    for (int k = 0; k < 4; ++k) add_corner_row<F16ROWS>(plan, d, texels, c.row[d][k], c.w[d][k], s_lut, acc);
+    for (int y = 0; y < 2; ++y)
+      add_corner_pair<F16ROWS>(plan, d, texels, c.row[d][y], PAIR, c.w[d][2 * y], c.w[d][2 * y + 1], s_lut, acc);
 #pragma unroll
     for (int ch = 0; ch < 4; ++ch) {
       const bool on = ch < 3 ? do_rgb : do_a;
@@ -265,7 +286,7 @@
 #ifndef NT_SHADE_FWD_OCC
 #define NT_SHADE_FWD_OCC 3
 #endif
-template <bool FULL4, bool F16ROWS = false>
+template <bool FULL4, bool F16ROWS = false, bool ANCHOR = false>
 __global__ __launch_bounds__(SH_BLOCK, NT_SHADE_FWD_OCC) void nt_shade_fwd_kernel(
     vsa_nt_plan plan, const int* __restrict__ hit_slot, const float* __restrict__ tex_uv,
     const float* __restrict__ rays_d, const float4* __restrict__ tris,
@@ -290,7 +311,7 @@
     const bool has_alpha = nt_shell_has_alpha(plan, s);
     float b[16], raw[4];
     sh_basis(c.dir[0], c.dir[1], c.dir[2], b);
-    shade_hit<FULL4, F16ROWS>(plan, c, texels, s_lut, has_alpha, b, raw,
+    shade_hit<FULL4, F16ROWS, !ANCHOR>(plan, c, texels, s_lut, has_alpha, b, raw,
               coeffs_out ? coeffs_out + ((long long)s * N + n) * 64 : nullptr);
 #pragma unroll
     for (int ch = 0; ch < 3; ++ch) {
@@ -401,7 +422,7 @@
 #pragma unroll
     for (int d = 0; d < VSA_NT_MAX_DEG; ++d) {
       s_row[t][2 * d] = c.row[d][0];
-      s_row[t][2 * d + 1] = c.row[d][2];
+      s_row[t][2 * d + 1] = c.row[d][1];
       s_f[t][2 * d] = c.fx[d];
       s_f[t][2 * d + 1] = c.fy[d];
     }
@@ -526,21 +547,22 @@
     return VSA_ERR_ARG;
   if (plan->row_format < 0 || plan->row_format > 2) return VSA_ERR_UNSUPPORTED;
   dim3 grid = shade_grid(vsa_div_up(nr_rays, SH_BLOCK), plan->nr_shells);
-  if (plan->row_format != 0)
-    hipLaunchKernelGGL((nt_shade_fwd_kernel<false, true>), grid, dim3(SH_BLOCK), 0, (hipStream_t)stream, *plan,
-                       hit_slot, tex_uv, rays_d, reinterpret_cast<const float4*>(tris), slot_of,
-                       seg_start, reinterpret_cast<const unsigned*>(texels), nr_rays, surfs_rgb,
-                       surfs_alpha, surfs_normals, coeffs_out, reinterpret_cast<float4*>(act_out));
-  else if (plan->rgb_degrees == VSA_NT_MAX_DEG && plan->alpha_degrees == VSA_NT_MAX_DEG)
-    hipLaunchKernelGGL(nt_shade_fwd_kernel<true>, grid, dim3(SH_BLOCK), 0, (hipStream_t)stream, *plan,
-                       hit_slot, tex_uv, rays_d, reinterpret_cast<const float4*>(tris), slot_of,
-                       seg_start, reinterpret_cast<const unsigned*>(texels), nr_rays, surfs_rgb,
-                       surfs_alpha, surfs_normals, coeffs_out, reinterpret_cast<float4*>(act_out));
-  else
-    hipLaunchKernelGGL(nt_shade_fwd_kernel<false>, grid, dim3(SH_BLOCK), 0, (hipStream_t)stream, *plan,
-                       hit_slot, tex_uv, rays_d, reinterpret_cast<const float4*>(tris), slot_of,
-                       seg_start, reinterpret_cast<const unsigned*>(texels), nr_rays, surfs_rgb,
-                       surfs_alpha, surfs_normals, coeffs_out, reinterpret_cast<float4*>(act_out));
+  auto launch = [&](auto kernel) {
+    hipLaunchKernelGGL(kernel, grid, dim3(SH_BLOCK), 0, (hipStream_t)stream, *plan, hit_slot, tex_uv, rays_d,
+                       reinterpret_cast<const float4*>(tris), slot_of, seg_start, reinterpret_cast<const unsigned*>(texels),
+                       nr_rays, surfs_rgb, surfs_alpha, surfs_normals, coeffs_out, reinterpret_cast<float4*>(act_out));
+  };
+  const bool anchor = plan->anchor != 0;
+  if (plan->row_format != 0) {
+    if (anchor) launch(nt_shade_fwd_kernel<false, true, true>);
+    else launch(nt_shade_fwd_kernel<false, true, false>);
+  } else if (plan->rgb_degrees == VSA_NT_MAX_DEG && plan->alpha_degrees == VSA_NT_MAX_DEG) {
+    if (anchor) launch(nt_shade_fwd_kernel<true, false, true>);
+    else launch(nt_shade_fwd_kernel<true, false, false>);
+  } else {
+    if (anchor) launch(nt_shade_fwd_kernel<false, false, true>);
+    else launch(nt_shade_fwd_kernel<false, false, false>);
+  }
   VSA_RETURN_LAUNCH_STATUS();
 }
 
diff --git a/volsurfs_amd/csrc/raygen.hip b/volsurfs_amd/csrc/raygen.hip
--- a/volsurfs_amd/csrc/raygen.hip
+++ b/volsurfs_amd/csrc/raygen.hip
@@ -1,6 +1,7 @@
 #include "common.h"
 #include "pcg32.h"
 #include "pinhole.h"
+#include "tile_order.h"
 
 namespace {
 
@@ -90,23 +91,13 @@
   }
 }
 
-__device__ __forceinline__ int tile_x_of(int j) { return (j & 8) ? 7 - (j & 7) : (j & 7); }
-
-struct __attribute__((packed, aligned(4))) F3 {
-  float x, y, z;
-};
-
 template <int C>
 __global__ __launch_bounds__(256) void tile_order_kernel(const float* __restrict__ src,
                                                          float* __restrict__ dst, int W, long long n,
                                                          int inverse) {
   const long long i = (long long)blockIdx.x * 256 + threadIdx.x;
   if (i >= n) return;
-  const int tiles_x = W >> 3;
-  const long long t = i >> 6;
-  const int j = (int)(i & 63);
-  const long long row = (t / tiles_x) * 8 + (j >> 3), col = (t % tiles_x) * 8 + tile_x_of(j);
-  const long long px = row * W + col;
+  const long long px = tile_pixel_of(i, W);
   const long long from = inverse ? i : px, to = inverse ? px : i;
   if constexpr (C == 3) {
     *reinterpret_cast<F3*>(dst + to * 3) = *reinterpret_cast<const F3*>(src + from * 3);
@@ -121,16 +112,7 @@
     float* __restrict__ o_t, float* __restrict__ d_t, float* __restrict__ gt_t, int W, long long n) {
   const long long i = (long long)blockIdx.x * 256 + threadIdx.x;
   if (i >= n) return;
-  const int tiles_x = W >> 3;
-  const long long t = i >> 6;
-  const int j = (int)(i & 63);
-  const long long px = ((t / tiles_x) * 8 + (j >> 3)) * W + (t % tiles_x) * 8 + tile_x_of(j);
-  const F3 vo = *reinterpret_cast<const F3*>(o + 3 * px), vd = *reinterpret_cast<const F3*>(d + 3 * px);
-  F3 vg = {0.f, 0.f, 0.f};
-  if (gt) vg = *reinterpret_cast<const F3*>(gt + 3 * px);
-  *reinterpret_cast<F3*>(o_t + 3 * i) = vo;
-  *reinterpret_cast<F3*>(d_t + 3 * i) = vd;
-  if (gt) *reinterpret_cast<F3*>(gt_t + 3 * i) = vg;
+  tile_order_rays_at(o, d, gt, o_t, d_t, gt_t, W, i);
 }
 
 }
diff --git a/volsurfs_amd/csrc/step_prologue.hip b/volsurfs_amd/csrc/step_prologue.hip
--- /dev/null
+++ b/volsurfs_amd/csrc/step_prologue.hip
@@ -0,0 +1,64 @@
+#include "common.h"
+#include "tile_order.h"
+#include "trace_feedback.h"
+#include "trace_walk.h"
+
+namespace {
+
+constexpr int PRO_BLOCK = 256;
+constexpr int PRO_CLEAR_VECS = 4;
+
+__global__ __launch_bounds__(PRO_BLOCK) void step_prologue_kernel(
+    int* phase_word, char* half0, char* half1, const float* __restrict__ o, const float* __restrict__ d,
+    const float* __restrict__ gt, float* __restrict__ o_t, float* __restrict__ d_t, float* __restrict__ gt_t, int W,
+    long long n, int tile_wgs, float* __restrict__ clear, long long clear_n, int clear_wgs) {
+  const int b = (int)blockIdx.x;
+  if (b < tile_wgs) {
+    const long long i = (long long)b * PRO_BLOCK + threadIdx.x;
+    if (i < n) tile_order_rays_at(o, d, gt, o_t, d_t, gt_t, W, i);
+    return;
+  }
+  const int c = b - tile_wgs;
+  if (c < clear_wgs) {
+    float4* p4 = reinterpret_cast<float4*>(clear);
+    const long long n4 = clear_n >> 2;
+    const long long v0 = (long long)c * (PRO_BLOCK * PRO_CLEAR_VECS) + threadIdx.x;
+#pragma unroll
+    for (int k = 0; k < PRO_CLEAR_VECS; ++k) {
+      const long long v = v0 + (long long)k * PRO_BLOCK;
+      if (v < n4) p4[v] = make_float4(0.f, 0.f, 0.f, 0.f);
+    }
+    if (c == clear_wgs - 1 && (long long)threadIdx.x < (clear_n & 3)) clear[(n4 << 2) + threadIdx.x] = 0.f;
+    return;
+  }
+  if (threadIdx.x < 64) trace_fb_flip(phase_word, half0, half1, (int)threadIdx.x);
+}
+
+}
+
+extern "C" int vsa_step_prologue(void* feedback, long long feedback_bytes, int nr_meshes, const float* rays_o,
+                                 const float* rays_d, const float* gt_rgb, float* rays_o_tiled, float* rays_d_tiled,
+                                 float* gt_rgb_tiled, int height, int width, float* clear, long long clear_floats,
+                                 void* stream) {
+  if (height < 0 || width < 0 || (height & 7) || (width & 7) || clear_floats < 0) return VSA_ERR_ARG;
+  const long long n = (long long)height * width;
+  if (n > 0x7fffffff) return VSA_ERR_UNSUPPORTED;
+  if (n > 0 && (!rays_o || !rays_d || !rays_o_tiled || !rays_d_tiled || (gt_rgb && !gt_rgb_tiled))) return VSA_ERR_ARG;
+  if (clear_floats > 0 && (!clear || ((uintptr_t)clear & 15))) return VSA_ERR_ARG;
+  TraceFbLayout lay{{nullptr, nullptr}, nullptr, 0};
+  if (feedback) {
+    if (nr_meshes < 1 || n == 0) return VSA_ERR_ARG;
+    if (!trace_fb_layout(feedback, feedback_bytes, (long long)vsa_div_up(n, TRACE_BLOCK) * nr_meshes, &lay))
+      return VSA_ERR_ARG;
+  }
+  const int tile_wgs = vsa_div_up(n, PRO_BLOCK);
+  const long long clear_wgs_ll = clear_floats > 0 ? (clear_floats / 4 + PRO_BLOCK * PRO_CLEAR_VECS) / (PRO_BLOCK * PRO_CLEAR_VECS) : 0;
+  if (clear_wgs_ll > 0x3fffffff) return VSA_ERR_UNSUPPORTED;
+  const int clear_wgs = (int)clear_wgs_ll;
+  const unsigned wgs = (unsigned)tile_wgs + (unsigned)clear_wgs + (feedback ? 1u : 0u);
+  if (wgs == 0) return VSA_OK;
+  hipLaunchKernelGGL(step_prologue_kernel, dim3(wgs), dim3(PRO_BLOCK), 0, (hipStream_t)stream, lay.phase_word,
+                     lay.half[0], lay.half[1], rays_o, rays_d, gt_rgb, rays_o_tiled, rays_d_tiled, gt_rgb_tiled, width, n,
+                     tile_wgs, clear, clear_floats, clear_wgs);
+  VSA_RETURN_LAUNCH_STATUS();
+}
diff --git a/volsurfs_amd/csrc/tile_order.h b/volsurfs_amd/csrc/tile_order.h
--- /dev/null
+++ b/volsurfs_amd/csrc/tile_order.h
@@ -0,0 +1,28 @@
+#pragma once
+#include "common.h"
+
+__device__ __forceinline__ int tile_x_of(int j) { return (j & 8) ? 7 - (j & 7) : (j & 7); }
+
+__device__ __forceinline__ long long tile_pixel_of(long long i, int W) {
+  const int tiles_x = W >> 3;
+  const long long t = i >> 6;
+  const int j = (int)(i & 63);
+  return ((t / tiles_x) * 8 + (j >> 3)) * W + (t % tiles_x) * 8 + tile_x_of(j);
+}
+
+struct __attribute__((packed, aligned(4))) F3 {
+  float x, y, z;
+};
+
+__device__ __forceinline__ void tile_order_rays_at(const float* __restrict__ o, const float* __restrict__ d,
+                                                   const float* __restrict__ gt, float* __restrict__ o_t,
+                                                   float* __restrict__ d_t, float* __restrict__ gt_t, int W,
+                                                   long long i) {
+  const long long px = tile_pixel_of(i, W);
+  const F3 vo = *reinterpret_cast<const F3*>(o + 3 * px), vd = *reinterpret_cast<const F3*>(d + 3 * px);
+  F3 vg = {0.f, 0.f, 0.f};
+  if (gt) vg = *reinterpret_cast<const F3*>(gt + 3 * px);
+  *reinterpret_cast<F3*>(o_t + 3 * i) = vo;
+  *reinterpret_cast<F3*>(d_t + 3 * i) = vd;
+  if (gt) *reinterpret_cast<F3*>(gt_t + 3 * i) = vg;
+}
diff --git a/volsurfs_amd/csrc/trace.hip b/volsurfs_amd/csrc/trace.hip
--- a/volsurfs_amd/csrc/trace.hip
+++ b/volsurfs_amd/csrc/trace.hip
@@ -1,4 +1,5 @@
 #include "common.h"
+#include "trace_feedback.h"
 #include "trace_walk.h"
 #include <algorithm>
 #include <cstdio>
@@ -331,9 +332,7 @@
   return fb;
 }
 __global__ void trace_fb_flip_kernel(int* phase_word, char* half0, char* half1) {
-  const int ph = (*phase_word ^ 1) & 1;
-  if (threadIdx.x == 0) *phase_word = ph;
-  if (threadIdx.x < 4) reinterpret_cast<int*>(ph ? half0 : half1)[threadIdx.x] = 0;
+  trace_fb_flip(phase_word, half0, half1, (int)threadIdx.x);
 }
 #ifndef TRACE_FB_T
 #define TRACE_FB_T 160, 128, 64
@@ -542,12 +541,6 @@
                             hit_t, hit_slot, hit_uv, TRACE_BLOCK, stream);
 }
 
-static long long trace_fb_half_bytes(long long items, int* cap_out) {
-  const int cap = (int)std::min<long long>(items / 8 + 64, 1 << 27);
-  if (cap_out) *cap_out = cap;
-  return (16 + (items + 15) / 16 * 16 + 12ll * cap + 255) / 256 * 256;
-}
-
 extern "C" long long vsa_trace_feedback_bytes(int nr_rays, int nr_meshes) {
   if (nr_rays < 0 || nr_meshes < 1) return -1;
   return 2 * trace_fb_half_bytes((long long)vsa_div_up(nr_rays, TRACE_BLOCK) * nr_meshes, nullptr) + 256;
@@ -567,36 +560,32 @@
   return VSA_OK;
 }
 
-extern "C" int vsa_trace_q_fb(const uint32_t* qnodes, const float* tris, const int32_t* mesh_roots,
-                              const float* mesh_frames, int nr_meshes, int max_depth, const float* rays_o,
-                              const float* rays_d, int nr_rays, float t_min, float* hit_t, int32_t* hit_slot,
-                              float* hit_uv, void* feedback, long long feedback_bytes, int phase, void* stream) {
-  if (nr_rays < 0 || phase < 0 || phase > 2) return VSA_ERR_ARG;
+static int trace_q_fb_launch(const uint32_t* qnodes, const float* tris, const int32_t* mesh_roots,
+                             const float* mesh_frames, int nr_meshes, int max_depth, const float* rays_o,
+                             const float* rays_d, int nr_rays, float t_min, float* hit_t, int32_t* hit_slot,
+                             float* hit_uv, void* feedback, long long feedback_bytes, int phase, void* stream) {
+  if (nr_rays < 0 || phase < 0 || phase > 3) return VSA_ERR_ARG;
   if (const int rc = check_qtree(qnodes, tris, mesh_roots, mesh_frames, nr_meshes, max_depth, VSA_ERR_UNSUPPORTED, nr_rays > 0))
     return rc;
   if (nr_rays == 0) return VSA_OK;
   if (!rays_o || !rays_d || !hit_t || !hit_slot || !hit_uv || !feedback) return VSA_ERR_ARG;
   const int G = vsa_div_up(nr_rays, TRACE_BLOCK);
   const long long items = (long long)G * nr_meshes;
-  int cap = 0;
-  if (items > 0x7fffffff / 2 || feedback_bytes < 2 * trace_fb_half_bytes(items, &cap) + 256 || ((uintptr_t)feedback & 15))
-    return VSA_ERR_ARG;
-  const long long half = ((feedback_bytes - 256) / 2) & ~255ll;
+  TraceFbLayout lay;
+  if (!trace_fb_layout(feedback, feedback_bytes, items, &lay)) return VSA_ERR_ARG;
   const QTree t = make_qtree(qnodes, tris, mesh_roots, mesh_frames, nr_meshes);
-  char* b = static_cast<char*>(feedback);
   TraceFeedbackBuf fb;
-  fb.half[0] = b, fb.half[1] = b + half;
+  fb.half[0] = lay.half[0], fb.half[1] = lay.half[1];
   fb.flags_bytes = (items + 15) / 16 * 16;
-  fb.phase_word = phase == 2 ? reinterpret_cast<const int*>(b + 2 * half) : nullptr;
+  fb.phase_word = phase >= 2 ? lay.phase_word : nullptr;
   fb.phase = phase & 1;
-  fb.cap = cap;
+  fb.cap = lay.cap;
   hipStream_t s = (hipStream_t)stream;
   if (phase == 2)
-    hipLaunchKernelGGL(trace_fb_flip_kernel, dim3(1), dim3(64), 0, s, reinterpret_cast<int*>(b + 2 * half),
-                       fb.half[0], fb.half[1]);
-  else
+    hipLaunchKernelGGL(trace_fb_flip_kernel, dim3(1), dim3(64), 0, s, lay.phase_word, fb.half[0], fb.half[1]);
+  else if (phase < 2)
     VSA_HIP_TRY(hipMemsetAsync(fb.half[phase ^ 1], 0, 16, s));
-  dim3 grid((unsigned)(items + 3ll * cap)), block(TRACE_BLOCK);
+  dim3 grid((unsigned)(items + 3ll * lay.cap)), block(TRACE_BLOCK);
   const TraceCoopConfig& cfg = trace_coop_config();
   const int coop_chunk = cfg.chunk, coop_lanes = cfg.lanes;
   const bool coop = coop_lanes > 0 && items <= cfg.max_waves;
@@ -608,6 +597,23 @@
     });
   });
   VSA_RETURN_LAUNCH_STATUS();
+}
+
+extern "C" int vsa_trace_q_fb(const uint32_t* qnodes, const float* tris, const int32_t* mesh_roots,
+                              const float* mesh_frames, int nr_meshes, int max_depth, const float* rays_o,
+                              const float* rays_d, int nr_rays, float t_min, float* hit_t, int32_t* hit_slot,
+                              float* hit_uv, void* feedback, long long feedback_bytes, int phase, void* stream) {
+  if (phase > 2) return VSA_ERR_ARG;
+  return trace_q_fb_launch(qnodes, tris, mesh_roots, mesh_frames, nr_meshes, max_depth, rays_o, rays_d, nr_rays, t_min,
+                           hit_t, hit_slot, hit_uv, feedback, feedback_bytes, phase, stream);
+}
+
+extern "C" int vsa_trace_q_fb_flipped(const uint32_t* qnodes, const float* tris, const int32_t* mesh_roots,
+                                      const float* mesh_frames, int nr_meshes, int max_depth, const float* rays_o,
+                                      const float* rays_d, int nr_rays, float t_min, float* hit_t, int32_t* hit_slot,
+                                      float* hit_uv, void* feedback, long long feedback_bytes, void* stream) {
+  return trace_q_fb_launch(qnodes, tris, mesh_roots, mesh_frames, nr_meshes, max_depth, rays_o, rays_d, nr_rays, t_min,
+                           hit_t, hit_slot, hit_uv, feedback, feedback_bytes, 3, stream);
 }
 
 extern "C" int vsa_hit_attributes(const float* tris, const float* rays_o, const float* rays_d,
diff --git a/volsurfs_amd/csrc/trace_feedback.h b/volsurfs_amd/csrc/trace_feedback.h
--- /dev/null
+++ b/volsurfs_amd/csrc/trace_feedback.h
@@ -0,0 +1,32 @@
+#pragma once
+#include "common.h"
+#include <algorithm>
+
+static inline long long trace_fb_half_bytes(long long items, int* cap_out) {
+  const int cap = (int)std::min<long long>(items / 8 + 64, 1 << 27);
+  if (cap_out) *cap_out = cap;
+  return (16 + (items + 15) / 16 * 16 + 12ll * cap + 255) / 256 * 256;
+}
+
+struct TraceFbLayout {
+  char* half[2];
+  int* phase_word;
+  int cap;
+};
+static inline bool trace_fb_layout(void* feedback, long long feedback_bytes, long long items, TraceFbLayout* out) {
+  int cap = 0;
+  if (items > 0x7fffffff / 2 || feedback_bytes < 2 * trace_fb_half_bytes(items, &cap) + 256 || ((uintptr_t)feedback & 15))
+    return false;
+  const long long half = ((feedback_bytes - 256) / 2) & ~255ll;
+  char* b = static_cast<char*>(feedback);
+  out->half[0] = b, out->half[1] = b + half;
+  out->phase_word = reinterpret_cast<int*>(b + 2 * half);
+  out->cap = cap;
+  return true;
+}
+
+__device__ __forceinline__ void trace_fb_flip(int* phase_word, char* half0, char* half1, int lane) {
+  const int ph = (*phase_word ^ 1) & 1;
+  if (lane == 0) *phase_word = ph;
+  if (lane < 4) reinterpret_cast<int*>(ph ? half0 : half1)[lane] = 0;
+}
diff --git a/volsurfs_amd/pipeline.py b/volsurfs_amd/pipeline.py
--- a/volsurfs_amd/pipeline.py
+++ b/volsurfs_amd/pipeline.py
@@ -266,16 +266,19 @@
     def _step_prefix(self, record, acct):
         N, T, bank = self.nr_rays, self.timer, self.bank
         rays_o, rays_d, gt = self.rays_o, self.rays_d, self.gt
+        flipped = False
         if self.image_hw is not None:
             H, W = self.image_hw
-
+            fb = self.tracer.feedback_buffer(N, rays_o.device)
             T.run("ray_tile_order",
-                  lambda: _lib.call("vsa_tile_order_rays", self.rays_o, self.rays_d, self.gt, self._o_t,
-                                    self._d_t, self._gt_t, H, W, _lib.stream_ptr()),
+                  lambda: _lib.call("vsa_step_prologue", fb[0] if fb else None, fb[1] if fb else 0, self.K,
+                                    self.rays_o, self.rays_d, self.gt, self._o_t, self._d_t, self._gt_t, H, W,
+                                    None, 0, _lib.stream_ptr()),
                   record, bytes=N * 72)
+            flipped = fb is not None
             rays_o, rays_d, gt = self._o_t, self._d_t, self._gt_t
         hit_t, hit_slot, hit_uv = T.run(
-            "trace", lambda: self.tracer.trace_all(rays_o, rays_d), record,
+            "trace", lambda: self.tracer.trace_all(rays_o, rays_d, fb_flipped=flipped), record,
             bytes=acct.get("trace", 0))
         self._hit_slot = hit_slot
         tex_uv = T.run("nt_mark_compact",
@@ -303,13 +306,9 @@
         from .composite import composite_fwd_bwd_l1_raw
         rgb, g_c, g_a = T.run("composite_fwd_bwd",
                               lambda: composite_fwd_bwd_l1_raw(rgb_k, alpha_k, self.bg, gt,
-                                                               1.0 / (3.0 * self.loss_rays)),
+                                                               1.0 / (3.0 * self.loss_rays), image_hw=self.image_hw,
+                                                               rgb_out=self._rgb_out if self.image_hw else None),
                               record, bytes=N * (12 + 12 + 32 * K))
-        if self.image_hw is not None:
-            T.run("rgb_row_order", lambda: _lib.call("vsa_tile_order", rgb, self._rgb_out, self.image_hw[0],
-                                                     self.image_hw[1], 3, 1, _lib.stream_ptr()),
-                  record, bytes=N * 24)
-            rgb = self._rgb_out
         tris = self.tracer.tris
         T.run("nt_shade_bwd", lambda: bank.backward_shade(hit_slot, tex_uv, rays_d, tris, g_c, g_a,
                                                            self.grad_scale, self._act), record,
diff --git a/volsurfs_amd/raytrace.py b/volsurfs_amd/raytrace.py
--- a/volsurfs_amd/raytrace.py
+++ b/volsurfs_amd/raytrace.py
@@ -207,7 +207,21 @@
             pass
         self._bvh = []
 
-    def trace_all(self, rays_o, rays_d, t_min=0.0, out=None):
+    def feedback_buffer(self, N, device):
+        K = self.nr_meshes
+        if self.node_format != "q16" or self.narrow_rays_per_wave(N, K) < 64 or not self.cost_feedback or \
+                self.max_depth >= 48:
+            return None
+        if self._fb is None or self._fb[1] < N or self._fb[0].device != device:
+            fn = _lib.lib().vsa_trace_feedback_bytes
+            fn.restype = ctypes.c_longlong
+            nbytes = int(fn(ctypes.c_int(N), ctypes.c_int(K)))
+            if nbytes < 0:
+                raise _lib.VolsurfsHipError("vsa_trace_feedback_bytes failed")
+            self._fb = [torch.zeros(nbytes, dtype=torch.uint8, device=device), N, nbytes]
+        return self._fb[0], self._fb[2]
+
+    def trace_all(self, rays_o, rays_d, t_min=0.0, out=None, fb_flipped=False):
         N, rays_o, rays_d = _rays(rays_o, rays_d)
         K = self.nr_meshes
         if out is not None:
@@ -221,19 +235,18 @@
             hit_slot = torch.empty(K, N, dtype=torch.int32, device=rays_o.device)
             hit_uv = torch.empty(K, N, 2, device=rays_o.device)
         rpw = self.narrow_rays_per_wave(N, K) if self.node_format == "q16" else 64
+        fb = self.feedback_buffer(N, rays_o.device)
+        if fb_flipped and fb is None:
+            raise _lib.VolsurfsHipError("trace_all(fb_flipped=True): these rays do not use the feedback buffer")
         if rpw < 64:
             _lib.call("vsa_trace_q_narrow", *self.q16_tree_args(), rays_o, rays_d, N, float(t_min), hit_t, hit_slot,
                       hit_uv, int(rpw), _lib.stream_ptr())
-        elif self.node_format == "q16" and self.cost_feedback and self.max_depth < 48:
-            if self._fb is None or self._fb[1] < N or self._fb[0].device != rays_o.device:
-                fn = _lib.lib().vsa_trace_feedback_bytes
-                fn.restype = ctypes.c_longlong
-                nbytes = int(fn(ctypes.c_int(N), ctypes.c_int(K)))
-                if nbytes < 0:
-                    raise _lib.VolsurfsHipError("vsa_trace_feedback_bytes failed")
-                self._fb = [torch.zeros(nbytes, dtype=torch.uint8, device=rays_o.device), N, nbytes]
+        elif fb is not None and fb_flipped:
+            _lib.call("vsa_trace_q_fb_flipped", *self.q16_tree_args(), rays_o, rays_d, N, float(t_min), hit_t, hit_slot,
+                      hit_uv, fb[0], ctypes.c_longlong(fb[1]), _lib.stream_ptr())
+        elif fb is not None:
             _lib.call("vsa_trace_q_fb", *self.q16_tree_args(), rays_o, rays_d, N, float(t_min), hit_t, hit_slot, hit_uv,
-                      self._fb[0], ctypes.c_longlong(self._fb[2]), 2, _lib.stream_ptr())
+                      fb[0], ctypes.c_longlong(fb[1]), 2, _lib.stream_ptr())
         elif self.node_format == "q16":
             _lib.call("vsa_trace_q", *self.q16_tree_args(), rays_o, rays_d, N, float(t_min), hit_t, hit_slot, hit_uv,
                       _lib.stream_ptr())
```

After: 267.4 (median of 6 runs). About the same (+0.5%).
